# soedinglab/prosstt

Hardware: AMD Instinct MI355X
Metric: simulated cells*genes per second (count sampling: sample_density -> draw_counts) (higher is better)
Workload: dtype f32

## Files before the change

### prosstt_amd/_native.py

```python
import ctypes
import os
import threading
from collections import namedtuple

_HERE = os.path.dirname(os.path.abspath(__file__))

OK, EINVAL, EDOMAIN, EHIP, ENOMEM, ENODEV, ERCCL = 0, -1, -2, -3, -4, -5, -6
HOST_INPUTS, HOST_OUTPUT, CHECK_DOMAIN, TIME_KERNEL, CHECK_DEFERRED, MEANS_CACHED, PARAMS_NONNEG = 1, 2, 4, 8, 16, 32, 64
STATS_ACCUMULATE = 1

_Library = namedtuple("_Library", "path header hip symbols last_error")


def _path(env, filename):
    return os.environ.get(env) or os.path.join(_HERE, "lib", filename)


def _int(*argtypes):
    return ctypes.c_int, list(argtypes)


_ptr_to = ctypes.POINTER
_text = (ctypes.c_char_p, None)
vp, i32, i64, u32, u64, f64 = ctypes.c_void_p, ctypes.c_int32, ctypes.c_int64, ctypes.c_uint32, ctypes.c_uint64, ctypes.c_double
# ... 16 lines not shown
        "prosstt_amd_nb_params": _int(vp, vp, i64, i32, vp, vp, vp, vp, i64, vp, vp, vp, vp, u32),
        "prosstt_amd_hw_math": _int(vp, i32, u32, u64, vp, u32),
        "prosstt_amd_hw_math_at": _int(vp, i32, vp, u64, vp, u32),
        "prosstt_amd_comm_unique_id": _int(vp),
        "prosstt_amd_comm_init": _int(vp, vp, i32, i32, _ptr_to(vp)),
        "prosstt_amd_comm_destroy": _int(vp),
        "prosstt_amd_gather_counts": _int(vp, vp, vp, vp, i32, i32, vp),
        "prosstt_amd_comm_selftest": _int(vp, vp, u64),
        "prosstt_amd_domain_status": _int(vp, _ptr_to(i32)),
        "prosstt_amd_numpy_programs": _int(vp, vp, vp, vp, i32, i32, i32, vp, vp, vp, vp, vp, vp, vp, vp),
        "prosstt_amd_lineage_attempt": _int(vp, vp, i32, i32, vp, i64, i32, vp, vp, vp, vp),
        "prosstt_amd_lineage_attempt_batch": _int(vp, vp, i32, i32, i32, vp, i64, i32, vp, vp, vp, vp),
        "prosstt_amd_lineage_walk": _int(vp, u64, u64, i32, i32, vp),
        "prosstt_amd_lineage_walk_batch": _int(vp, u64, u64, i32, i32, i32, vp),
        "prosstt_amd_lineage_commit": _int(vp, vp, i32, i32, vp, i64, vp, vp),
        "prosstt_amd_gene_max": _int(vp, vp, i64, i64, vp),
        "prosstt_amd_means_from_rel": _int(vp, vp, vp, i64, i64, vp),
    }, "prosstt_amd_last_error"),
    "host": _Library(_path("PROSSTT_AMD_HOST_LIB", "libprosstt_amd_host.so"), "prosstt_amd_host.h", False, {
        "prosstt_amd_host_widen_i32_i64": _widen,
        "prosstt_amd_host_widen_u16_i64": _widen,
        "prosstt_amd_host_widen_u16_i32": _widen,
        "prosstt_amd_host_widen_u8_i64": _widen,
        "prosstt_amd_host_widen_u8_i32": _widen,
        "prosstt_amd_host_scatter_i32": _int(vp, i32, vp, vp, u64, i32),
        "prosstt_amd_host_has_avx2": (ctypes.c_int, None),
    }, None),
    "stats": _Library(_path("PROSSTT_AMD_STATS_LIB", "libprosstt_amd_stats.so"), "prosstt_amd_stats.h", True, {
        "prosstt_amd_stats_last_error": _text,
        "prosstt_amd_stats_workspace_bytes": _int(i64, i64, _ptr_to(u64)),
        "prosstt_amd_stats_count_summary": _int(vp, vp, i64, i64, i64, vp, u64, vp, vp, vp, vp, vp, vp, u32),
    }, "prosstt_amd_stats_last_error"),
    "embed": _Library(_path("PROSSTT_AMD_EMBED_LIB", "libprosstt_amd_embed.so"), "prosstt_amd_embed.h", True, {
        "prosstt_amd_embed_last_error": _text,
        "prosstt_amd_embed_workspace_bytes": _int(i64, i64, i64, _ptr_to(u64)),
        "prosstt_amd_embed_gene_moments": _int(vp, vp, i64, i64, i64, vp, vp, u64, vp, vp, vp),
        "prosstt_amd_embed_matmul": _int(vp, vp, i64, i64, i64, vp, vp, i64, vp, vp, u64, vp),
        "prosstt_amd_embed_rmatmul": _int(vp, vp, i64, i64, i64, vp, vp, i64, vp, vp, u64, vp),
    }, "prosstt_amd_embed_last_error"),
    "knn": _Library(_path("PROSSTT_AMD_KNN_LIB", "libprosstt_amd_knn.so"), "prosstt_amd_knn.h", True, {
        "prosstt_amd_knn_last_error": _text,
        "prosstt_amd_knn_workspace_bytes": _int(i64, i64, i64, i64, _ptr_to(u64)),
        "prosstt_amd_knn_search": _int(vp, vp, i64, i64, i64, i64, i64, vp, vp, vp, u64),
    }, "prosstt_amd_knn_last_error"),
    "graph": _Library(_path("PROSSTT_AMD_GRAPH_LIB", "libprosstt_amd_graph.so"), "prosstt_amd_graph.h", True, {
        "prosstt_amd_graph_last_error": _text,
        "prosstt_amd_graph_workspace_bytes": _int(i64, i64, _ptr_to(u64)),
        "prosstt_amd_graph_memberships": _int(vp, vp, vp, i64, i64, vp, vp, vp, vp),
        "prosstt_amd_graph_symmetrize_emit": _int(vp, vp, vp, i64, i64, vp, u64),
        "prosstt_amd_graph_symmetrize_fold": _int(vp, vp, vp, vp, i64, i64, i64, vp, u64, vp, vp, vp),
        "prosstt_amd_graph_normalize": _int(vp, vp, vp, vp, i64, i64, vp, vp, vp, vp),
        "prosstt_amd_graph_spmv": _int(vp, vp, vp, vp, i64, i64, vp, vp, i32),
    }, "prosstt_amd_graph_last_error"),
    "layout": _Library(_path("PROSSTT_AMD_LAYOUT_LIB", "libprosstt_amd_layout.so"), "prosstt_amd_layout.h", True, {
        "prosstt_amd_layout_last_error": _text,
        "prosstt_amd_layout_epochs": _int(vp, vp, vp, vp, i64, i64, i32, vp, vp, i32, i32, i32, f64, f64, f64, f64, i32, u64, i32),
        "prosstt_amd_layout_negatives": _int(vp, u64, i32, i64, i64, i32, i64, vp),
    }, "prosstt_amd_layout_last_error"),
}

ADDED_LIBRARIES = {
    "tsne": _Library(_path("PROSSTT_AMD_TSNE_LIB", "libprosstt_amd_tsne.so"), "prosstt_amd_tsne.h", True, {
        "prosstt_amd_tsne_last_error": _text,
        "prosstt_amd_tsne_workspace_bytes": _int(i64, i32, i32, _ptr_to(u64)),
        "prosstt_amd_tsne_affinities": _int(vp, vp, vp, i64, i64, f64, vp, vp, vp),
        "prosstt_amd_tsne_symmetrize_fold": _int(vp, vp, vp, vp, i64, i64, i64, vp, u64, vp, vp, vp),
        "prosstt_amd_tsne_gradient": _int(vp, vp, vp, vp, i64, i64, i32, vp, f64, i32, vp, u64, vp, vp, vp),
        "prosstt_amd_tsne_iterations": _int(vp, vp, vp, vp, i64, i64, i32, vp, vp, vp, vp, i32, i32, i32, f64, f64, i32, vp, u64),
        "prosstt_amd_tsne_objective": _int(vp, vp, vp, vp, i64, i64, i32, vp, vp),
    }, "prosstt_amd_tsne_last_error"),
}

LATER_LIBRARIES = {
    "dpt": _Library(_path("PROSSTT_AMD_DPT_LIB", "libprosstt_amd_dpt.so"), "prosstt_amd_dpt.h", True, {
        "prosstt_amd_dpt_last_error": _text,
        "prosstt_amd_dpt_workspace_bytes": _int(i64, i32, i32, _ptr_to(u64)),
        "prosstt_amd_dpt_rows": _int(vp, vp, i64, vp, i64, i64, vp, i64, vp),
        "prosstt_amd_dpt_concordance": _int(vp, vp, vp, i64, i32, i32, vp, u64, vp, vp),
    }, "prosstt_amd_dpt_last_error"),
    "markers": _Library(_path("PROSSTT_AMD_MARKERS_LIB", "libprosstt_amd_markers.so"), "prosstt_amd_markers.h", True, {
        "prosstt_amd_markers_last_error": _text,
        "prosstt_amd_markers_workspace_bytes": _int(i64, i64, i64, i64, _ptr_to(u64)),
        "prosstt_amd_markers_group_moments": _int(vp, vp, i64, i64, i64, vp, vp, i64, vp, i64, i64, vp, u64, vp, vp, vp, vp, vp),
    }, "prosstt_amd_markers_last_error"),
    "cluster": _Library(_path("PROSSTT_AMD_CLUSTER_LIB", "libprosstt_amd_cluster.so"), "prosstt_amd_cluster.h", True, {
        "prosstt_amd_cluster_last_error": _text,
        "prosstt_amd_cluster_workspace_bytes": _int(i64, i64, _ptr_to(u64)),
        "prosstt_amd_cluster_quantize": _int(vp, vp, vp, vp, i64, i64, vp, vp, vp),
        "prosstt_amd_cluster_sweep": _int(vp, vp, vp, vp, vp, i64, i64, vp, i64, i64, i64, vp, vp, i64, f64, i32, i32, vp, vp, vp),
        "prosstt_amd_cluster_totals": _int(vp, vp, vp, vp, vp, i64, i64, vp, vp, vp, vp),
        "prosstt_amd_cluster_aggregate_emit": _int(vp, vp, vp, i64, i64, vp, i64, vp, u64, vp),
        "prosstt_amd_cluster_aggregate_fold": _int(vp, vp, vp, vp, vp, i64, i64, i64, vp, vp, vp, vp),
    }, "prosstt_amd_cluster_last_error"),
    "ranks": _Library(_path("PROSSTT_AMD_RANKS_LIB", "libprosstt_amd_ranks.so"), "prosstt_amd_ranks.h", True, {
        "prosstt_amd_ranks_last_error": _text,
        "prosstt_amd_ranks_workspace_bytes": _int(i64, i64, i64, _ptr_to(u64)),
        "prosstt_amd_ranks_rank_sums": _int(vp, vp, i64, i64, i64, vp, vp, i64, vp, i64, i64, i64, vp, u64, vp, vp, vp),
    }, "prosstt_amd_ranks_last_error"),
    "hvg": _Library(_path("PROSSTT_AMD_HVG_LIB", "libprosstt_amd_hvg.so"), "prosstt_amd_hvg.h", True, {
        "prosstt_amd_hvg_last_error": _text,
        "prosstt_amd_hvg_workspace_bytes": _int(i64, i64, _ptr_to(u64)),
        "prosstt_amd_hvg_clipped_sums": _int(vp, vp, i64, i64, i64, vp, vp, u64, vp, vp, vp, vp),
        "prosstt_amd_hvg_normalized_moments": _int(vp, vp, i64, i64, i64, vp, vp, u64, vp, vp, vp),
        "prosstt_amd_hvg_gather_columns": _int(vp, vp, i64, i64, i64, vp, i64, vp, i64, vp),
    }, "prosstt_amd_hvg_last_error"),
    "autocorr": _Library(_path("PROSSTT_AMD_AUTOCORR_LIB", "libprosstt_amd_autocorr.so"), "prosstt_amd_autocorr.h", True, {
        "prosstt_amd_autocorr_last_error": _text,
        "prosstt_amd_autocorr_workspace_bytes": _int(i64, i64, i64, _ptr_to(u64)),
        "prosstt_amd_autocorr_gene_sums": _int(vp, vp, i64, i64, i64, vp, vp, vp, vp, vp, i64, vp, i64, i32, vp, u64, vp, vp, vp, vp, vp),
        "prosstt_amd_autocorr_smooth": _int(vp, vp, i64, i64, i64, vp, vp, vp, vp, vp, i64, i32, i32, vp, i64, vp),
    }, "prosstt_amd_autocorr_last_error"),
    "fit": _Library(_path("PROSSTT_AMD_FIT_LIB", "libprosstt_amd_fit.so"), "prosstt_amd_fit.h", True, {
        "prosstt_amd_fit_last_error": _text,
        "prosstt_amd_fit_workspace_bytes": _int(i64, i64, i64, _ptr_to(u64)),
        "prosstt_amd_fit_loglik": _int(vp, vp, i64, i64, i64, vp, vp, i64, vp, i64, vp, vp, i64, vp, u64, vp, vp, vp, vp),
    }, "prosstt_amd_fit_last_error"),
    "trends": _Library(_path("PROSSTT_AMD_TRENDS_LIB", "libprosstt_amd_trends.so"), "prosstt_amd_trends.h", True, {
        "prosstt_amd_trends_last_error": _text,
        "prosstt_amd_trends_workspace_bytes": _int(i64, i64, i64, i64, _ptr_to(u64)),
        "prosstt_amd_trends_node_sums": _int(vp, vp, i64, i64, i64, vp, vp, vp, i64, i64, i64, vp, u64, vp, vp, vp),
    }, "prosstt_amd_trends_last_error"),
    "mapping": _Library(_path("PROSSTT_AMD_MAPPING_LIB", "libprosstt_amd_mapping.so"), "prosstt_amd_mapping.h", True, {
        "prosstt_amd_mapping_last_error": _text,
        "prosstt_amd_mapping_workspace_bytes": _int(i64, i64, i64, i64, _ptr_to(u64)),
        "prosstt_amd_mapping_node_scores": _int(vp, vp, i64, i64, i64, vp, vp, i64, i64, vp, vp, vp, i64, i64, vp, u64, vp, vp,
                                                vp, vp, vp, vp),
        "prosstt_amd_mapping_node_scores_tiled": _int(vp, vp, i64, i64, i64, vp, vp, i64, i64, vp, vp, vp, i64, i64, i32, vp, u64,
                                                      vp, vp, vp, vp, vp, vp),
    }, "prosstt_amd_mapping_last_error"),
    "ptree": _Library(_path("PROSSTT_AMD_PTREE_LIB", "libprosstt_amd_ptree.so"), "prosstt_amd_ptree.h", True, {
        "prosstt_amd_ptree_last_error": _text,
        "prosstt_amd_ptree_workspace_bytes": _int(i64, i64, i64, i32, _ptr_to(u64)),
        "prosstt_amd_ptree_assign": _int(vp, vp, i64, i64, i64, vp, i64, i64, f64, vp, u64, vp, vp, vp, vp, vp, vp, vp),
        "prosstt_amd_ptree_project": _int(vp, vp, i64, i64, i64, vp, i64, i64, vp, i64, vp, vp, vp, vp),
    }, "prosstt_amd_ptree_last_error"),
}

NEWER_LIBRARIES = {
    "regress": _Library(_path("PROSSTT_AMD_REGRESS_LIB", "libprosstt_amd_regress.so"), "prosstt_amd_regress.h", True, {
        "prosstt_amd_regress_last_error": _text,
        "prosstt_amd_regress_workspace_bytes": _int(i64, i64, i64, _ptr_to(u64)),
        "prosstt_amd_regress_normal_equations": _int(vp, vp, i64, i64, i64, vp, vp, i64, vp, i64, i64, vp, vp, vp, i32, i32, vp,
                                                     u64, vp, vp, vp, vp, vp),
    }, "prosstt_amd_regress_last_error"),
}


SAMPLER_LATER = ("prosstt_amd_plan.h", {
    "prosstt_amd_strip_plan": _int(i64, i32, i32, i32, i32, vp, _ptr_to(i32), _ptr_to(i32), _ptr_to(i32)),
    "prosstt_amd_last_strip_plan": _int(vp, vp, _ptr_to(i32), _ptr_to(i32), _ptr_to(i32)),
})


def _library(name):
    for table in (LIBRARIES, ADDED_LIBRARIES, LATER_LIBRARIES):
        if name in table:
            return table[name]
    return NEWER_LIBRARIES[name]


class NativeError(RuntimeError):
    def __init__(self, code, message):
        super().__init__("prosstt_amd error %d: %s" % (code, message))
        self.code = code


_loaded = {}
_lock = threading.Lock()


def load(name="sampler"):
    lib = _library(name)
    with _lock:
        if name not in _loaded:
            if not os.path.exists(lib.path):
                raise RuntimeError("%s not found: build it with `make -C prosstt_amd/csrc %s` (or "
                                   "`python -c 'import __graft_entry__ as g; g.build()'`)%s"
                                   % (lib.path, name, ". prosstt_amd has no CPU fallback." if lib.hip else ""))
            if lib.hip:
                import torch
            L = ctypes.CDLL(lib.path)
            symbols = dict(lib.symbols, **SAMPLER_LATER[1]) if name == "sampler" else lib.symbols
            for symbol, (restype, argtypes) in symbols.items():
                fn = getattr(L, symbol)
                fn.restype = restype
                if argtypes is not None:
                    fn.argtypes = argtypes
            _loaded[name] = L
        return _loaded[name]


def check(code, name="sampler"):
    if code != OK:
        msg = getattr(load(name), _library(name).last_error)().decode("utf-8", "replace")
        if code == EDOMAIN:
            raise ValueError(msg)
        raise NativeError(code, msg)


def device_count():
    n = ctypes.c_int(0)
    rc = load().prosstt_amd_device_count(ctypes.byref(n))
    return n.value if rc == OK else 0
```

### prosstt_amd/csrc/k3_heavy.h

```cpp
#pragma once
#include "prnb_device.h"
#include "k3_stream.h"

namespace k3 {

constexpr int kHeavyBlock = 256;
constexpr int kHCap = 128;
constexpr uint32_t kWalkerBlocks = 6u;
constexpr int kWCap = 96;

struct HGEntry { int32_t n, g, attempt; float m; };
struct HPEntry { int32_t n, g; float lam; int32_t attempt; };
struct HWId { int32_t n, g; };

struct HeavyLds {
    HGEntry hg[kHCap];
    HPEntry hp[kHCap];
    f32x4_t wst[kWCap];
    HWId wid[kWCap];
    uint16_t wk[kWCap];
};

__global__ __launch_bounds__(kHeavyBlock) void sample_counts_heavy_kernel(
    const HeavyList* __restrict__ heavy_ptr, uint32_t regions, StripPlan plan,
    const float* __restrict__ means, int64_t rows,
    int32_t G, const int32_t* __restrict__ row_of_cell, const float* __restrict__ scal,
    const float* __restrict__ ga, const float* __restrict__ gbm1, int64_t N, uint32_t k0, uint32_t k1,
    uint64_t cell_offset, const int64_t* __restrict__ cell_index, int32_t* __restrict__ out, int64_t ld,
    int64_t* __restrict__ check_words, uint32_t check_request, uint32_t check_bad_row, uint32_t check_verdict)
{
    __shared__ __attribute__((aligned(16))) float inv_k_store[prnb::kTabShift + prnb::kKTab];
    float* const inv_k = inv_k_store + prnb::kTabShift;
    __shared__ HeavyLds lds_all[kHeavyBlock / 64];
    const HeavyList heavy = *heavy_ptr;
    const int tid = threadIdx.x, lane = tid & 63, wv = __builtin_amdgcn_readfirstlane(tid >> 6);
    HeavyLds& L = lds_all[wv];
    for (int k = tid - prnb::kTabShift; k < prnb::kKTab; k += kHeavyBlock) inv_k[k] = k > 0 ? 1.0f / (float)k : 0.0f;
    __shared__ uint32_t seg_n[kSegs], seg_first[kSegs + 1];
    if (wv == 0) {
        uint32_t n = heavy.seg_cnt[lane];
        n = n < heavy.ent_cap ? n : heavy.ent_cap;
        uint32_t x = (n + 63u) >> 6;
        const uint32_t mine = x;
#pragma unroll
        for (int d = 1; d < 64; d <<= 1) {
            const uint32_t t = (uint32_t)__shfl_up((int)x, d, 64);
            if (lane >= d) x += t;
        }
        seg_n[lane] = n;
        seg_first[lane] = x - mine;
        if (lane == 63) seg_first[kSegs] = x;
    }
    struct ClassRec { int32_t first_cell, end_cell; uint32_t first_block, groups, groups_rcp, log2_len, pad[2]; };
    __shared__ __attribute__((aligned(16))) ClassRec cls_tab[kPlanClasses];
    if (tid < kPlanClasses) {
        static_assert(kPlanClasses == 4, "spelled out below");
        const StripClass c0 = plan.c[0], c1 = plan.c[1], c2 = plan.c[2], c3 = plan.c[3];
        const int32_t end_all = plan.c[4].first_cell;
        const int32_t first = tid == 0 ? c0.first_cell : (tid == 1 ? c1.first_cell : (tid == 2 ? c2.first_cell : c3.first_cell));
        const int32_t end = tid == 0 ? c1.first_cell : (tid == 1 ? c2.first_cell : (tid == 2 ? c3.first_cell : end_all));
        const int32_t len = tid == 0 ? c0.strip_cells : (tid == 1 ? c1.strip_cells : (tid == 2 ? c2.strip_cells : c3.strip_cells));
        const int32_t fb = tid == 0 ? c0.first_block : (tid == 1 ? c1.first_block : (tid == 2 ? c2.first_block : c3.first_block));
        const uint32_t sh = (uint32_t)__builtin_ctz((uint32_t)len);
        const int32_t strips = (end - first + len - 1) >> sh;
        const uint32_t g = strips > 4 ? (uint32_t)(strips + 3) / 4u : 1u;
        ClassRec c;
        c.first_cell = first; c.end_cell = end; c.first_block = (uint32_t)fb;
        c.groups = g;
        c.groups_rcp = 0xffffffffu / g + ((g & (g - 1u)) == 0u ? 1u : 0u);
        c.log2_len = sh; c.pad[0] = c.pad[1] = 0u;
        cls_tab[tid] = c;
    }
    __syncthreads();
    const uint32_t waves = gridDim.x * (kHeavyBlock / 64);
    auto locate = [&](uint32_t chunk, uint32_t& seg, uint32_t& first) __attribute__((always_inline)) {
        uint32_t lo = 0u;
#pragma unroll
        for (uint32_t step = kSegs / 2; step != 0u; step >>= 1)
            if (seg_first[lo + step] <= chunk) lo += step;
        seg = lo;
        first = (chunk - seg_first[lo]) << 6;
    };
    const uint32_t fb1 = (uint32_t)plan.c[1].first_block, fb2 = (uint32_t)plan.c[2].first_block, fb3 = (uint32_t)plan.c[3].first_block;
    struct Origin { int32_t tile_g, n0, cells; };
    auto region_origin = [&](uint32_t r) __attribute__((always_inline)) -> Origin {
        const uint32_t blk = r >> 2;
        const uint32_t cls = (blk >= fb1 ? 1u : 0u) + (blk >= fb2 ? 1u : 0u) + (blk >= fb3 ? 1u : 0u);
        const ClassRec c = cls_tab[cls];
        const uint32_t local = blk - c.first_block;
        uint32_t q = __umulhi(local, c.groups_rcp);
        q += (local - q * c.groups >= c.groups) ? 1u : 0u;
        q = c.groups > 1u ? q : local;
        Origin o;
        o.tile_g = (int32_t)q;
        o.n0 = c.first_cell + (int32_t)(((local - q * c.groups) * 4u + (r & 3u)) << c.log2_len);
        o.cells = c.end_cell - o.n0 < (1 << c.log2_len) ? c.end_cell - o.n0 : (1 << c.log2_len);
        return o;
    };

    int hg_top = 0, hp_top = 0, hw_top = 0;

    auto cell_id = [&](int32_t n) __attribute__((always_inline)) -> uint64_t {
        return cell_index ? (uint64_t)cell_index[n] : cell_offset + (uint64_t)n;
    };

    auto poisson_pass = [&]() __attribute__((always_inline)) {
        const int cnt = hp_top < 64 ? hp_top : 64;
        bool again = false, small = false;
        HPEntry e;
        e.n = 0; e.g = 0; e.lam = 0.0f; e.attempt = 0;
        int32_t x = 0;
        if (lane < cnt) {
            e = L.hp[hp_top - 1 - lane];
            const uint64_t cell = cell_id(e.n);
            const uint32_t c0 = (uint32_t)cell, c1 = (uint32_t)(cell >> 32);
            const float lam = e.lam;
            if (!(lam > 0.0f)) {
                x = 0;
            } else if (lam < prnb::kPoisInv) {
                small = true;
            } else if (!(lam < prnb::kLamBig)) {
                const prnb::Words w = prnb::philox_count<0>(c0, c1, (uint32_t)e.g, 0x80000000u, k0, k1);
                const float z = prnb::hw_normal(w.w[0], w.w[1]);
                const float kf = __builtin_floorf(PRNB_FMA(prnb::hw_sqrt(lam), z, lam) + 0.5f);
                x = (int32_t)__builtin_fminf(__builtin_fmaxf(kf, 0.0f), 2147483520.0f);
            } else {
                const int j = e.attempt;
                const prnb::Words w =
                    prnb::philox_count<0>(c0, c1, (uint32_t)e.g, 0x80000000u + (uint32_t)(j >> 1), k0, k1);
                const float slam = prnb::hw_sqrt(lam);
                const float bb = PRNB_FMA(2.53f, slam, 0.931f);
                const float aa = PRNB_FMA(0.02483f, bb, -0.059f);
                const float U = prnb::unif((j & 1) ? w.w[2] : w.w[0]) - 0.5f;
                const float V = prnb::unif((j & 1) ? w.w[3] : w.w[1]);
                const float us = __builtin_fmaxf(0.5f - __builtin_fabsf(U), 5.8207661e-11f);
                const float rus = prnb::hw_rcp(us);
                float kf = __builtin_floorf(PRNB_FMA(PRNB_FMA(2.0f * aa, rus, bb), U, lam + 0.43f));
                const float vr = PRNB_FMA(-3.6224f, prnb::hw_rcp(bb - 2.0f), 0.9277f);
                bool accept = (us >= 0.07f) && (V <= vr);
                if (!accept && !(kf < 0.0f || (us < 0.013f && V > us))) {
                    const float invalpha = PRNB_FMA(1.1328f, prnb::hw_rcp(bb - 3.4f), 1.1239f);
                    const float lhs = prnb::kLn2 * prnb::hw_log2((V * invalpha) * prnb::hw_rcp(PRNB_FMA(aa * rus, rus, bb)));
                    float rhs;
                    if (kf < 10.0f) {
                        rhs = PRNB_FMA(kf, prnb::kLn2 * prnb::hw_log2(lam), -lam) - prnb::logfact_small((int)kf);
                    } else {
                        const float rk = prnb::hw_rcp(kf);
                        const float d = (lam - kf) * rk;
                        const float lp = prnb::hw_log1pmx(d, lam * rk);
                        const float st = rk * PRNB_FMA(-0.0027777778f, rk * rk, 0.083333336f);
                        rhs = PRNB_FMA(kf, lp, PRNB_FMA(-0.5f, prnb::kLn2 * prnb::hw_log2(6.2831855f * kf), -st));
                    }
                    accept = lhs <= rhs;
                }
                if (!accept) {
                    kf = __builtin_floorf(lam);
                    again = j + 1 < 2 * prnb::kMaxTries;
                }
                x = (int32_t)__builtin_fminf(__builtin_fmaxf(kf, 0.0f), 2147483520.0f);
            }
        }
        if (__builtin_amdgcn_ballot_w64(small) != 0ull) {
            const uint64_t cell = cell_id(e.n);
            const prnb::Words w = prnb::philox_count<0>((uint32_t)cell, (uint32_t)(cell >> 32), (uint32_t)e.g, 0x80000000u, k0, k1);
            const float lam = small ? e.lam : 1.0f;
            const int32_t xs = prnb::chop_down_wave(small, w.w[0], prnb::hw_exp2(-(lam * prnb::kLog2e)), lam, 0.0f, inv_k);
            if (small) x = xs;
        }
        if (lane < cnt && !again && x != 0) out[(int64_t)e.n * ld + e.g] = x;
        hp_top -= cnt;
        const unsigned long long m = __builtin_amdgcn_ballot_w64(again);
        if (again) {
            e.attempt += 1;
            L.hp[hp_top + lane_rank(m)] = e;
        }
        hp_top += __popcll(m);
    };

    auto gamma_pass = [&]() __attribute__((always_inline)) {
        const int cnt = hg_top < 64 ? hg_top : 64;
        bool again = false, accepted = false;
        HGEntry e;
        e.n = 0; e.g = 0; e.attempt = 0; e.m = 0.0f;
        float lam = 0.0f;
        if (lane < cnt) {
            e = L.hg[hg_top - 1 - lane];
            const prnb::Params P = prnb::make_params_m(e.m, ga[e.g], gbm1[e.g]);
            const float r = P.m * P.inv_th;
            if (P.valid && r >= prnb::kRMin) {
                const uint64_t cell = cell_id(e.n);
                const bool boost = r < 1.0f;
                const float rr = boost ? r + 1.0f : r;
                const float dd = rr - 0.33333334f;
                const float cc = prnb::hw_rsq(9.0f * dd);
                const int i = e.attempt;
                const bool last = (i == prnb::kMaxTries - 1);
                const prnb::Words w = prnb::philox_count<0>((uint32_t)cell, (uint32_t)(cell >> 32), (uint32_t)e.g,
                                                          1u + (uint32_t)i, k0, k1);
                const float x = prnb::hw_normal(w.w[0], w.w[1]);
                const float t = cc * x;
                const float v1 = 1.0f + t;
                float v = 1.0f;
                bool ok;
                if (!(v1 > 0.0f)) {
                    ok = last;
                } else {
                    v = (v1 * v1) * v1;
                    ok = last;
                    if (!ok) {
                        const float u = prnb::unif(w.w[2]);
                        const float x2 = x * x;
                        ok = u < PRNB_FMA(-0.0331f, x2 * x2, 1.0f);
                        if (!ok) {
                            const float t2 = t * t;
                            const float h = PRNB_FMA(3.0f, prnb::hw_log1pmx(t, v1), PRNB_FMA(-t2, t, -3.0f * t2));
                            ok = prnb::kLn2 * prnb::hw_log2(u) < PRNB_FMA(dd, h, 0.5f * x2);
                        }
                    }
                }
                if (ok) {
                    float g = dd * v;
                    if (boost) g = g * prnb::hw_exp2(prnb::hw_log2(prnb::unif(w.w[3])) * prnb::hw_rcp(r));
                    lam = P.theta * g;
                    accepted = true;
                } else {
                    again = true;
                }
            }
        }
        hg_top -= cnt;
        const unsigned long long ma = __builtin_amdgcn_ballot_w64(again);
        if (again) {
            e.attempt += 1;
            L.hg[hg_top + lane_rank(ma)] = e;
        }
        hg_top += __popcll(ma);
        const unsigned long long mp = __builtin_amdgcn_ballot_w64(accepted);
        if (accepted) {
            HPEntry p;
            p.n = e.n; p.g = e.g; p.lam = lam; p.attempt = 0;
            L.hp[hp_top + lane_rank(mp)] = p;
        }
        hp_top += __popcll(mp);
        while (hp_top >= 64) poisson_pass();
    };

    int32_t wk = -1;
    float wps = 0.0f, wrem = 0.0f, wd = 0.0f, wq = 0.0f;
    int32_t wn = 0, wg = 0;
    auto walk_take = [&]() __attribute__((always_inline)) {
        const unsigned long long idle_m = __builtin_amdgcn_ballot_w64(wk < 0);
        const int rank = lane_rank(idle_m);
        if (wk < 0 && rank < hw_top) {
            const int at = hw_top - 1 - rank;
            const f32x4_t s = L.wst[at];
            const HWId id = L.wid[at];
            wk = (int32_t)L.wk[at];
            wps = s.x; wd = s.y; wq = s.z; wrem = s.w;
            wn = id.n; wg = id.g;
        }
        const int idle = __popcll(idle_m);
        hw_top -= idle < hw_top ? idle : hw_top;
    };
    auto walk_pass = [&]() __attribute__((always_inline)) {
        const bool busy = wk >= 0;
        const float* tab = &inv_k[busy ? wk + 1 : 6];
        float4 iv[4];
#pragma unroll
        for (int j = 0; j < 4; ++j) iv[j] = *reinterpret_cast<const float4*>(__builtin_assume_aligned(tab + 4 * j, 16));
        float t = wps, r = wrem;
        float rg[4][4], tl[4];
#pragma unroll
        for (int j = 0; j < 4; ++j) {
            rg[j][0] = r - t;
            t = t * PRNB_FMA(wd, iv[j].x, wq);
            rg[j][1] = rg[j][0] - t;
            t = t * PRNB_FMA(wd, iv[j].y, wq);
            rg[j][2] = rg[j][1] - t;
            t = t * PRNB_FMA(wd, iv[j].z, wq);
            rg[j][3] = rg[j][2] - t;
            tl[j] = t;
            r = rg[j][3];
            t = t * PRNB_FMA(wd, iv[j].w, wq);
        }
        bool end[4];
#pragma unroll
        for (int j = 0; j < 4; ++j) end[j] = (rg[j][3] < 0.0f) || (tl[j] < 1.0f) || (wk + 4 * j + 3 >= prnb::kWalkEnd);
        const bool ended = busy && (end[0] || end[1] || end[2] || end[3]);
        if (__builtin_amdgcn_ballot_w64(ended) != 0ull) {
            int32_t at[4];
#pragma unroll
            for (int j = 0; j < 4; ++j)
                at[j] = ((wk + 4 * j + 3) + ((int32_t)prnb::f2u(rg[j][0]) >> 31)) + (((int32_t)prnb::f2u(rg[j][1]) >> 31) + ((int32_t)prnb::f2u(rg[j][2]) >> 31));
            if (ended) {
                out[(int64_t)wn * ld + wg] = end[0] ? at[0] : (end[1] ? at[1] : (end[2] ? at[2] : at[3]));
                wk = -1;
                wps = 0.0f;
            }
        }
        if (wk >= 0) {
            wps = t;
            wk += 16;
            wrem = r;
        }
    };
    auto walk_service = [&](bool drain) __attribute__((always_inline)) {
        for (;;) {
            const int busy = __popcll(__builtin_amdgcn_ballot_w64(wk >= 0));
            if (busy <= 32 && (drain ? hw_top > 0 : hw_top >= 32)) walk_take();
            else if (drain ? busy > 0 : busy > 32) walk_pass();
            else break;
        }
    };
    auto walk_push = [&](bool push, int32_t n, int32_t g, int32_t k, f32x4_t s) __attribute__((always_inline)) {
        const unsigned long long mw = __builtin_amdgcn_ballot_w64(push);
        if (push) {
            const int at = hw_top + lane_rank(mw);
            L.wst[at] = s;
            HWId id;
            id.n = n; id.g = g;
            L.wid[at] = id;
            L.wk[at] = (uint16_t)k;
        }
        hw_top += __popcll(mw);
        if (hw_top >= 32) walk_service(false);
    };

    auto from_start = [&](bool has, int32_t n, int32_t g) __attribute__((always_inline)) {
        bool heavy_c = false, light = false;
        prnb::Params P;
        P.m = 1.0f; P.theta = 1.0f; P.iu = 0.5f; P.t2 = 1.0f; P.inv_th = 1.0f; P.valid = false; P.light = false;
        if (has) {
            int32_t row = row_of_cell[n];
            row = row < 0 ? 0 : (row >= rows ? (int32_t)(rows - 1) : row);
            P = prnb::make_params(means[(int64_t)row * G + g], scal[n], ga[g], gbm1[g]);
            light = P.valid && P.light;
            heavy_c = P.valid && !P.light;
        }
        const unsigned long long mh = __builtin_amdgcn_ballot_w64(heavy_c);
        if (heavy_c) {
            HGEntry e;
            e.n = n; e.g = g; e.attempt = 0; e.m = P.m;
            L.hg[hg_top + lane_rank(mh)] = e;
        }
        hg_top += __popcll(mh);
        bool push = false;
        f32x4_t s = {0.0f, 0.0f, 0.0f, 0.0f};
        if (__builtin_amdgcn_ballot_w64(light) != 0ull) {
            const uint64_t cell = cell_id(has ? n : 0);
            const prnb::Words w = prnb::philox_count<0>((uint32_t)cell, (uint32_t)(cell >> 32), (uint32_t)g >> 2, 0u, k0, k1);
            const uint32_t sel = (uint32_t)g & 3u;
            const uint32_t wj = sel == 0u ? w.w[0] : (sel == 1u ? w.w[1] : (sel == 2u ? w.w[2] : w.w[3]));
            const float mp = P.m * P.iu, q = P.theta * P.iu, d = mp - q;
            const float ps = prnb::hw_exp2(-P.t2) * 4294967296.0f;
            const float r0 = (float)wj - ps;
            const float p1 = ps * mp;
            const float r1 = r0 - p1;
            const float p2 = p1 * PRNB_FMA(d, inv_k[2], q);
            const float r2 = r1 - p2;
            const float p3 = p2 * PRNB_FMA(d, inv_k[3], q);
            const float r3 = r2 - p3;
            const float p4 = p3 * PRNB_FMA(d, inv_k[4], q);
            const float r4 = r3 - p4;
            const bool done = (r0 < 0.0f) || (r1 < 0.0f) || (r2 < 0.0f) || (r3 < 0.0f) || (r4 < 0.0f) || (p4 < 1.0f);
            const int32_t x = (r0 < 0.0f) ? 0 : ((r1 < 0.0f) ? 1 : ((r2 < 0.0f) ? 2 : ((r3 < 0.0f) ? 3 : 4)));
            if (light && done && x != 0) out[(int64_t)n * ld + g] = x;
            push = light && !done;
            s.x = p4 * PRNB_FMA(d, inv_k[5], q);
            s.y = d; s.z = q; s.w = r4;
        }
        walk_push(push, n, g, 5, s);
        while (hg_top >= 64) gamma_pass();
    };

    const uint32_t wave_id = blockIdx.x * (kHeavyBlock / 64) + (uint32_t)wv;
    const bool walker = (blockIdx.x & 15u) < kWalkerBlocks;
    const uint32_t walker_blocks = (gridDim.x >> 4) * kWalkerBlocks + ((gridDim.x & 15u) < kWalkerBlocks ? (gridDim.x & 15u) : kWalkerBlocks);
    const uint32_t n_redo = heavy.seg_cnt[kSegs + 1] < (uint32_t)kRedoCap ? heavy.seg_cnt[kSegs + 1] : (uint32_t)kRedoCap;
    auto push_entries = [&](bool has, int32_t n, int32_t g, float m) __attribute__((always_inline)) {
        const unsigned long long mh = __builtin_amdgcn_ballot_w64(has);
        if (has) {
            HGEntry h;
            h.n = n; h.g = g; h.attempt = 0; h.m = m;
            L.hg[hg_top + lane_rank(mh)] = h;
        }
        hg_top += __popcll(mh);
        while (hg_top >= 64) gamma_pass();
    };
    if (!walker) {
        const uint32_t blk_rank = blockIdx.x - ((blockIdx.x >> 4) * kWalkerBlocks + ((blockIdx.x & 15u) < kWalkerBlocks ? (blockIdx.x & 15u) : kWalkerBlocks));
        const uint32_t rank = blk_rank * (kHeavyBlock / 64) + (uint32_t)wv;
        const uint32_t drawers = (gridDim.x - walker_blocks) * (kHeavyBlock / 64);
        {
            const int sub = lane >> 4, sl = lane & 15;
            const uint4* const dense4 = reinterpret_cast<const uint4*>(heavy.dense);
            struct Step { uint32_t cnt; uint4 d4; Origin o; };
            auto load_step = [&](uint64_t r0) __attribute__((always_inline)) -> Step {
                Step S;
                S.cnt = 0u; S.d4 = make_uint4(0u, 0u, 0u, 0u);
                const uint64_t r = r0 + (uint64_t)sub * drawers;
                S.o = region_origin((uint32_t)r);
                if (r < (uint64_t)regions) {
                    S.cnt = heavy.count[r] & 0xffffu;
                    S.d4 = dense4[r * (kDense / 2) + (uint32_t)sl];
                }
                return S;
            };
            Step nxt = load_step(rank);
            for (uint64_t r0 = rank; r0 < (uint64_t)regions; r0 += 4ull * drawers) {
                const Step cur = nxt;
                nxt = load_step(r0 + 4ull * drawers);
                const uint32_t cnt = cur.cnt > heavy.cap ? 0u : cur.cnt;
                const int32_t tile_g = cur.o.tile_g, n0 = cur.o.n0;
                push_entries(2u * (uint32_t)sl < cnt, n0 + (int32_t)(cur.d4.x >> 8), tile_g * kTileG + (int32_t)(cur.d4.x & 255u), __uint_as_float(cur.d4.y));
                push_entries(2u * (uint32_t)sl + 1u < cnt, n0 + (int32_t)(cur.d4.z >> 8), tile_g * kTileG + (int32_t)(cur.d4.z & 255u), __uint_as_float(cur.d4.w));
            }
        }
        {
            const uint32_t chunks = seg_first[kSegs];
            HeavyEntry nx;
            nx.n = 0; nx.g = 0; nx.m = 0.0f; nx.pad = 0u;
            bool nx_has = false;
            auto request = [&](uint32_t chunk) __attribute__((always_inline)) {
                uint32_t sg, first;
                locate(chunk, sg, first);
                nx_has = first + (uint32_t)lane < seg_n[sg];
                if (nx_has) nx = heavy.ent[(uint64_t)sg * heavy.ent_cap + first + (uint32_t)lane];
            };
            if (rank < chunks) request(rank);
            for (uint32_t chunk = rank; chunk < chunks; chunk += drawers) {
                const HeavyEntry e = nx;
                const bool has = nx_has;
                if (chunk + drawers < chunks) request(chunk + drawers);
                push_entries(has, e.n, e.g, e.m);
            }
        }
    } else {
        const uint32_t wrank = ((blockIdx.x >> 4) * kWalkerBlocks + (blockIdx.x & 15u)) * (kHeavyBlock / 64) + (uint32_t)wv;
        const uint32_t walkers = walker_blocks * (kHeavyBlock / 64);
        for (uint32_t i = wrank * 64u; i < n_redo; i += walkers * 64u) {
            const bool has = i + (uint32_t)lane < n_redo;
            const int2 ng = has ? heavy.redo[i + (uint32_t)lane] : make_int2(0, 0);
            from_start(has, ng.x, ng.y);
        }
        const uint32_t per_walker = ((regions + walkers - 1u) / walkers + 15u) & ~15u;
        const uint32_t r_end = (wrank + 1u) * per_walker < regions ? (wrank + 1u) * per_walker : regions;
        const uint32_t rl = (uint32_t)lane >> 2, s0 = (uint32_t)lane & 3u;
        static_assert(kWalkSlots <= 12, "three slots per lane");
        struct WStep { uint32_t n_walks; f32x4_t st[3]; uint32_t id[3]; Origin o; };
        auto load_wstep = [&](uint32_t rb) __attribute__((always_inline)) -> WStep {
            WStep S;
            S.n_walks = 0u;
            const uint32_t r = rb + rl;
            S.o = region_origin(r);
#pragma unroll
            for (int j = 0; j < 3; ++j) { S.st[j] = f32x4_t{0.0f, 0.0f, 0.0f, 0.0f}; S.id[j] = 0u; }
            if (r < r_end) {
                S.n_walks = heavy.count[r] >> 16;
#pragma unroll
                for (int j = 0; j < 3; ++j) {
                    const uint32_t slot = s0 + 4u * (uint32_t)j;
                    if (slot < (uint32_t)kWalkSlots) {
                        S.st[j] = heavy.wst[(uint64_t)r * kWalkSlots + slot];
                        S.id[j] = heavy.wid[(uint64_t)r * kWalkSlots + slot];
                    }
                }
            }
            return S;
        };
        WStep wn = load_wstep(wrank * per_walker);
        for (uint32_t rb = wrank * per_walker; rb < r_end; rb += 16u) {
            const WStep cur = wn;
            wn = load_wstep(rb + 16u);
            const int32_t tile_g = cur.o.tile_g, n0 = cur.o.n0;
#pragma unroll
            for (int j = 0; j < 3; ++j) {
                const uint32_t slot = s0 + 4u * (uint32_t)j;
                walk_push(slot < cur.n_walks, n0 + (int32_t)((cur.id[j] & 0xffffu) >> 8), tile_g * kTileG + (int32_t)(cur.id[j] & 255u),
                          (int32_t)(cur.id[j] >> 16) - 3, cur.st[j]);
            }
        }
    }
    {
        const uint32_t n_ovf = heavy.seg_cnt[kSegs];
        for (uint32_t i = wave_id; i < n_ovf; i += waves) {
            const uint32_t r = heavy.ovf_regions[i];
            const Origin o = region_origin(r);
            const int32_t tg = o.tile_g;
            const int64_t nb = o.n0;
            for (int32_t c = 0; c < o.cells; ++c)
                for (int j = 0; j < 4; ++j) {
                    const int32_t g = tg * kTileG + j * 64 + lane;
                    from_start(g < G, (int32_t)(nb + c), g);
                }
        }
    }
    walk_service(true);
    while (hg_top > 0) gamma_pass();
    while (hp_top > 0) poisson_pass();

    if (check_words && check_words[check_request] != 0 && check_words[check_bad_row] == 0) {
        bool bad = false;
        for (int64_t n = blockIdx.x; n < N; n += gridDim.x) {
            const float s = scal[n];
            const float* mrow = means + (int64_t)row_of_cell[n] * G;
            for (int32_t g = tid; g < G; g += kHeavyBlock) {
                const float M = mrow[g];
                const float m = M * s;
                bad = bad || !(M > 0.0f && M < __builtin_inff()) || (PRNB_FMA(ga[g], m, gbm1[g]) < 0.0f);
            }
        }
        if (bad) check_words[check_verdict] = 1;
    }
}

}
```

### prosstt_amd/csrc/k3_stream.h

```cpp
#pragma once
#include <type_traits>
#include "prnb_device.h"

namespace k3 {

constexpr int kBlock = 256;
constexpr int kTileG = 256;
constexpr int kStripCells = 128;
constexpr int kS1Cap = 192;
constexpr int kS2Cap = 104;
constexpr int kS2Run = 40;
static_assert(kS2Cap >= kS2Run - 1 + 64 && kS1Cap >= 63 + 128, "a stack must take one more round of pushes");
constexpr int kRing = 8;
constexpr int kBail = 6;

constexpr int kLateCap = 64;
constexpr int kRingMaxK3 = 248;
constexpr int kLongSlots = 4;
constexpr int kListTail = 16;
constexpr int kInvTab = 272;

struct CellInfo { uint64_t row_bytes; float s; uint32_t runs; uint32_t ph[4]; };
static_assert(sizeof(CellInfo) == 32, "one s_load_dwordx8");

constexpr int kRunMinCells = 8;

__host__ __device__ inline uint32_t run_word(const int32_t* row_of_cell, int64_t i, int64_t N, int64_t rows, int32_t strip_cells)
{
    if (i >= N) return 1u;
    auto row = [&](int64_t n) -> int64_t { const int64_t r = row_of_cell[n]; return r < 0 ? 0 : (r >= rows ? rows - 1 : r); };
    const int64_t first = i - i % strip_cells;
    const int64_t end = first + strip_cells < N ? first + strip_cells : N;
    const int64_t mine = row(i);
    if (i != first && row(i - 1) == mine) return 0u;
    int64_t j = i + 1;
    while (j < end && row(j) == mine) ++j;
    const uint32_t len = (uint32_t)(j - i);
    if (i != first) return len;
    uint32_t runs = 1u;
    for (int64_t prev = mine; j < end; ++j) {
        const int64_t r = row(j);
        runs += r != prev;
        prev = r;
    }
    return len | (runs << 16);
}

constexpr int kPlanClasses = 4;
constexpr int kPlanAlign = 64;
constexpr int kPlanMinStrip = 8;
struct StripClass { int32_t first_cell, strip_cells, first_block; };
struct StripPlan {
    int32_t classes, tiles_g;
    StripClass c[kPlanClasses + 1];
};

__host__ __device__ inline StripPlan strip_plan(int64_t N, int32_t G, int32_t resident, int32_t forced_cells, int32_t taper, int32_t max_classes)
{
    const int64_t n = N > 0 ? N : 0;
    const int64_t tiles = ((int64_t)(G > 0 ? G : 0) + kTileG - 1) / kTileG;
    int64_t L = 64;
    while (L > 8 && ((n + L - 1) / L) * tiles < 4 * 5 * 1024) L /= 2;
    if (forced_cells == 8 || forced_cells == 16 || forced_cells == 32 || forced_cells == 64) L = forced_cells;
    if (forced_cells == kStripCells) L = 64;
    const int64_t uniform_blocks = (((n + L - 1) / L + 3) / 4) * tiles;
    const int64_t R = taper > 0 ? taper : resident;
    const int most = max_classes >= 1 && max_classes <= kPlanClasses ? max_classes : kPlanClasses;
    int64_t size[kPlanClasses] = {n, 0, 0, 0};
    int K = 1;
    if (taper > 0 || (resident > 0 && uniform_blocks >= 4 * (int64_t)resident)) {
        const int64_t uniform_len = L;
        if (L == 64 && forced_cells != 64) L = kStripCells;
        const int64_t align = L > kPlanAlign ? L : kPlanAlign;
        int64_t shorts = 0;
        while (K < most && (L >> K) >= kPlanMinStrip) {
            int64_t s = ((R * 4 * (L >> K) / (tiles > 0 ? tiles : 1) + kPlanAlign / 2) / kPlanAlign) * kPlanAlign;
            if (s < kPlanAlign) s = kPlanAlign;
            if (n - (shorts + s) < align) break;
            size[K++] = s;
            shorts += s;
        }
        if (K > 1) size[0] = ((n - shorts) / align) * align;
        else L = uniform_len;
    }
    StripPlan p;
    p.classes = K;
    p.tiles_g = (int32_t)tiles;
    int64_t cell = 0, block = 0;
    for (int k = 0; k <= kPlanClasses; ++k) {
        const int64_t len = k < K ? L >> k : 1;
        const int64_t cells = k + 1 < K ? size[k] : n - cell;
        p.c[k].first_cell = (int32_t)cell;
        p.c[k].strip_cells = (int32_t)len;
        p.c[k].first_block = (int32_t)(block < 0x7fffffff ? block : 0x7fffffff);
        cell += cells;
        block += (((cells + len - 1) / len + 3) / 4) * tiles;
    }
    return p;
}

struct StripAt { int32_t tile_g, cells, strip_cells; int64_t n0; };
__host__ __device__ inline StripAt strip_of_region(const StripPlan& p, uint32_t region)
{
    const int32_t blk = (int32_t)(region >> 2);
    static_assert(kPlanClasses == 4, "spelled out below");
    const StripClass c0 = p.c[0], c1 = p.c[1], c2 = p.c[2], c3 = p.c[3];
    const int32_t end_all = p.c[4].first_cell;
    StripClass c = c0;
    int32_t end = c1.first_cell;
    if (blk >= c1.first_block) { c = c1; end = c2.first_cell; }
    if (blk >= c2.first_block) { c = c2; end = c3.first_cell; }
    if (blk >= c3.first_block) { c = c3; end = end_all; }
    const int32_t first = c.first_cell, len = c.strip_cells, fb = c.first_block;
    const int32_t strips = (end - first + len - 1) >> __builtin_ctz((uint32_t)len);
    const int32_t groups = strips > 4 ? (strips + 3) / 4 : 1;
    const int32_t local = blk - fb;
    StripAt at;
    at.tile_g = local / groups;
    at.strip_cells = len;
    const int32_t strip = (local - at.tile_g * groups) * 4 + (int32_t)(region & 3u);
    at.n0 = (int64_t)first + (int64_t)strip * len;
    at.cells = strip < strips ? (end - at.n0 < len ? (int32_t)(end - at.n0) : len) : 0;
    return at;
}

constexpr uint32_t kPhiloxM0 = 0xD2511F53u, kPhiloxM1 = 0xCD9E8D57u, kPhiloxW0 = 0x9E3779B9u, kPhiloxW1 = 0xBB67AE85u;

__host__ __device__ inline void philox_cell_part(uint32_t cell_lo, uint32_t cell_hi, uint32_t k0, uint32_t k1, uint32_t ph[4])
{
    const uint64_t p0 = (uint64_t)kPhiloxM0 * cell_lo;
    const uint64_t p1 = (uint64_t)kPhiloxM1 * ((uint32_t)(p0 >> 32) ^ k1);
    ph[0] = cell_hi ^ k0;
    ph[1] = (uint32_t)(p1 >> 32) ^ (k0 + kPhiloxW0);
    ph[2] = (uint32_t)p0 ^ (k1 + kPhiloxW1);
    ph[3] = (uint32_t)p1;
}

__device__ __forceinline__ prnb::Words philox_count_row(const uint32_t ph[4], uint32_t hi1, uint32_t lo1, uint32_t k0, uint32_t k1)
{
    static_assert(prnb::kCountRounds >= 3, "two rounds are spelled out here");
    const uint32_t c0a = hi1 ^ ph[0];
    const uint64_t p0 = (uint64_t)kPhiloxM0 * c0a;
    const uint32_t c0b = lo1 ^ ph[1];
    const uint32_t c1b = ph[3];
    const uint32_t c2b = (uint32_t)(p0 >> 32) ^ ph[2];
    const uint32_t c3b = (uint32_t)p0;
    return prnb::philox4x32<prnb::kCountRounds - 2, 0>(c0b, c1b, c2b, c3b, k0 + 2u * kPhiloxW0, k1 + 2u * kPhiloxW1);
}

struct S1Entry { float m, theta, wf; uint32_t pos; };
struct S2Entry { float ps, d, q, rem; };

struct WaveLds {
    S1Entry s1_null;
    S1Entry s1[kS1Cap];
    S2Entry s2[kS2Cap];
    uint32_t s2p[kS2Cap];
    uint32_t late[kLateCap];
};

static_assert(offsetof(WaveLds, s1) == offsetof(WaveLds, s1_null) + sizeof(S1Entry), "s1[-1] must be the null entry");

typedef float f32x4_t __attribute__((ext_vector_type(4)));
constexpr int kSegs = 64;
constexpr int kDense = 32;
constexpr int kWalkSlots = kBail + kLongSlots;
struct HeavyEntry { int32_t n, g; float m; uint32_t pad; };
struct HeavyList {
    uint2* list; uint32_t cap;
    uint2* dense;
    uint32_t* count;
    f32x4_t* wst; uint32_t* wid;
    uint32_t* overflow;
    uint32_t* seg_cnt;
    HeavyEntry* ent; uint32_t ent_cap;
    uint32_t* ovf_regions;
    int2* redo;
};
constexpr int kRedoCap = 65536;

__device__ __forceinline__ uint32_t umin(uint32_t a, uint32_t b) { return a < b ? a : b; }

__device__ __forceinline__ int lane_rank(unsigned long long mask)
{
    return (int)__builtin_amdgcn_mbcnt_hi((uint32_t)(mask >> 32),
                                          __builtin_amdgcn_mbcnt_lo((uint32_t)mask, 0u));
}

#define K3_GLOBAL(T) __attribute__((address_space(1))) T*
typedef uint32_t u32x4_t __attribute__((ext_vector_type(4)));
typedef int32_t i32x2_t __attribute__((ext_vector_type(2)));
static_assert(sizeof(HeavyEntry) == sizeof(u32x4_t) && sizeof(int2) == sizeof(i32x2_t), "stored as plain vectors");
template <bool VEC, bool BIG>
__global__ __launch_bounds__(kBlock, 5) void sample_counts_stream_kernel(
    const float* __restrict__ means, int32_t G, const CellInfo* __restrict__ cellinfo,
    const float* __restrict__ ga, const float* __restrict__ gbm1, const float* __restrict__ gphi,
    int64_t N, uint32_t k0, uint32_t k1, int32_t* __restrict__ out, int64_t ld, StripPlan plan,
    uint2* __restrict__ heavy_list, uint32_t heavy_cap, uint2* __restrict__ heavy_dense,
    const HeavyList* __restrict__ heavy_ptr)
{
    struct HeavyGlobal {
        K3_GLOBAL(uint32_t) count; K3_GLOBAL(f32x4_t) wst; K3_GLOBAL(uint32_t) wid; K3_GLOBAL(uint32_t) overflow;
        K3_GLOBAL(uint32_t) seg_cnt; K3_GLOBAL(u32x4_t) ent; uint32_t ent_cap; K3_GLOBAL(uint32_t) ovf_regions; K3_GLOBAL(i32x2_t) redo;
    };
    auto heavy_late = [&]() -> HeavyGlobal {
        const HeavyList* p = heavy_ptr;
        asm volatile("" : "+s"(p));
        const __attribute__((address_space(4))) HeavyList* h = (const __attribute__((address_space(4))) HeavyList*)p;
        HeavyGlobal g;
        g.count = (K3_GLOBAL(uint32_t))h->count; g.wst = (K3_GLOBAL(f32x4_t))h->wst; g.wid = (K3_GLOBAL(uint32_t))h->wid;
        g.overflow = (K3_GLOBAL(uint32_t))h->overflow; g.seg_cnt = (K3_GLOBAL(uint32_t))h->seg_cnt; g.ent = (K3_GLOBAL(u32x4_t))h->ent;
        g.ent_cap = h->ent_cap; g.ovf_regions = (K3_GLOBAL(uint32_t))h->ovf_regions; g.redo = (K3_GLOBAL(i32x2_t))h->redo;
        return g;
    };
    __shared__ __attribute__((aligned(16))) float inv_k_store[prnb::kTabShift + kInvTab + 2];
    float* const inv_k = inv_k_store + prnb::kTabShift;
    __shared__ WaveLds lds_all[kBlock / 64];
    __shared__ __attribute__((aligned(kRing * 256))) uint8_t ring_all[kBlock / 64][kRing * 256];

    const int tid = threadIdx.x;
    const int lane = tid & 63, wv = __builtin_amdgcn_readfirstlane(tid >> 6);
    WaveLds& L = lds_all[wv];

    for (int k = tid - prnb::kTabShift; k < kInvTab + 2; k += kBlock) inv_k[k] = k > 0 ? 1.0f / (float)k : 0.0f;
    __syncthreads();

    const uint32_t region = blockIdx.x * 4u + (uint32_t)wv;
    const StripAt at = strip_of_region(plan, region);
    const int32_t gbase = __builtin_amdgcn_readfirstlane(at.tile_g) * kTileG;
    const int32_t g0 = gbase + lane * 4;
    const int64_t n0 = (int64_t)__builtin_amdgcn_readfirstlane((int32_t)at.n0);
    const int cells = __builtin_amdgcn_readfirstlane(at.cells);
    if (cells <= 0) {
        if (lane == 0) heavy_late().count[region] = 0u;
        return;
    }

    float a[4], bm1[4], phi[4];
#pragma unroll
    for (int j = 0; j < 4; ++j) {
        const bool in = g0 + j < G;
        a[j] = in ? ga[g0 + j] : 0.0f;
        bm1[j] = in ? gbm1[g0 + j] : 0.0f;
        phi[j] = in ? gphi[g0 + j] : 1.0f;
    }

    const uint32_t s1_lds = (uint32_t)(uintptr_t)&L.s1[0];
    uint32_t s1_at = s1_lds;
    int s2_top = 0;
    constexpr uint32_t kNoHeavy = 0xffffffffu;
    uint32_t hpend = kNoHeavy;
    float hpend_m = 0.0f;
    typedef float f32x4 __attribute__((ext_vector_type(4)));
    f32x4 st = {0.0f, 0.0f, 0.0f, 0.0f};
    uint32_t pos = 0u;
    int k3 = 8;
    f32x4 inv = *reinterpret_cast<const f32x4*>(__builtin_assume_aligned(&inv_k[6], 16));
    f32x4 inv2 = *reinterpret_cast<const f32x4*>(__builtin_assume_aligned(&inv_k[10], 16));
    unsigned long long idle_s = ~0ull;

    constexpr uint32_t kPosMagic = 0x4B000000u;
    int32_t* const strip_out = out + n0 * ld + gbase;
    const uint32_t ld32 = (uint32_t)ld;
    int32_t flushed_pos = -1;
    uint8_t* const ring = ring_all[wv];
    for (int i = lane; i < kRing * 64; i += 64) reinterpret_cast<uint32_t*>(ring)[i] = 0u;
    if (lane < 4) reinterpret_cast<uint32_t*>(&L.s1_null)[lane] = 0u;

    const __amdgpu_buffer_rsrc_t out_rsrc = __builtin_amdgcn_make_buffer_rsrc(strip_out, 0, 0x80000000u, 0x00020000);
    const uint32_t store_voff = g0 < G ? (uint32_t)lane * 16u : 0x80000000u;
    uint32_t flush_off = 0u;

    auto flush_row = [&](int cl) {
        uint32_t* slot = reinterpret_cast<uint32_t*>(ring + (cl & (kRing - 1)) * 256) + lane;
        const uint32_t packed = __hip_atomic_exchange(slot, 0u, __ATOMIC_RELAXED, __HIP_MEMORY_SCOPE_WAVEFRONT);
        const int32_t v[4] = {(int32_t)(packed & 0xffu), (int32_t)((packed >> 8) & 0xffu),
                              (int32_t)((packed >> 16) & 0xffu), (int32_t)(packed >> 24)};
        if (VEC) {
            typedef uint32_t u32x4_ __attribute__((ext_vector_type(4)));
            const u32x4_ row4 = {(uint32_t)v[0], (uint32_t)v[1], (uint32_t)v[2], (uint32_t)v[3]};
            if (BIG) __builtin_amdgcn_raw_buffer_store_b128(row4, out_rsrc, store_voff, flush_off, 18 );
            else __builtin_amdgcn_raw_buffer_store_b128(row4, out_rsrc, store_voff, flush_off, 2 );
        } else {
            int32_t* dst = strip_out + (int64_t)cl * ld + lane * 4;
#pragma unroll
            for (int j = 0; j < 4; ++j)
                if (g0 + j < G) dst[j] = v[j];
        }
        flush_off += ld32 * 4u;
        flushed_pos = (int32_t)kPosMagic | (cl << 8) | 255;
    };

    int late_top = 0;
    auto flush_late = [&]() {
        for (int i = lane; i < late_top; i += 64) {
            const uint32_t e = L.late[i];
            const uint32_t p = e >> 16;
            strip_out[(p >> 8) * ld32 + (p & 255u)] = (int32_t)(e & 0xffffu);
        }
        late_top = 0;
    };
#define K3_MASK(x) __builtin_amdgcn_ballot_w64(x)
    const uint32_t ring_lds = (uint32_t)(uintptr_t)&ring[0];
    uint32_t ring_mask = (uint32_t)(kRing * 256 - 1);
    asm volatile("" : "+v"(ring_mask));
    const uint32_t late_lds = (uint32_t)(uintptr_t)&L.late[0];
    uint2* const my_list = heavy_list + (uint64_t)region * (heavy_cap + (uint32_t)kListTail);
    uint2* const my_long = my_list + heavy_cap;
    int n_long = 0;
    uint32_t h_cnt = 0u;
    auto flush_heavy = [&]() {
        const unsigned long long mp_ = K3_MASK(hpend != kNoHeavy);
        if (hpend != kNoHeavy) {
            const uint32_t slot = h_cnt + (uint32_t)lane_rank(mp_);
            if (slot < heavy_cap) {
                uint2* const dst = slot < (uint32_t)kDense ? heavy_dense + ((uint64_t)region * kDense + slot) : my_list + slot;
                *dst = make_uint2(hpend & 0xffffu, __float_as_uint(hpend_m));
            }
        }
        h_cnt += (uint32_t)__popcll(mp_);
        hpend = kNoHeavy;
    };
    auto deliver = [&](unsigned long long ok_m, unsigned long long give_m, uint32_t p, uint32_t res, float gm) {
        const unsigned long long late_m = K3_MASK((int32_t)p <= flushed_pos);
        uint32_t ring_at;
        asm volatile("v_and_or_b32 %0, %2, %3, %4\n\ts_mov_b64 exec, %1\n\tds_write_b8 %0, %5\n\ts_mov_b64 exec, -1"
                     : "=&v"(ring_at) : "s"(ok_m & ~late_m), "v"(p), "v"(ring_mask), "s"(ring_lds), "v"(res) : "memory");
        const unsigned long long ml = ok_m & late_m;
        if ((ml | give_m) != 0ull) {
            if (ml != 0ull) {
                const int cnt = __popcll(ml);
                if (late_top + cnt > kLateCap) flush_late();
                asm volatile("s_mov_b64 exec, %0\n\tds_write_b32 %1, %2\n\ts_mov_b64 exec, -1"
                             :: "s"(ml), "v"(late_lds + (uint32_t)((late_top + lane_rank(ml)) << 2)), "v"((p << 16) | res) : "memory");
                late_top += cnt;
            }
            if (give_m != 0ull) {
                if ((give_m & K3_MASK(hpend != kNoHeavy)) != 0ull) flush_heavy();
                asm volatile("s_mov_b64 exec, %2\n\tv_mov_b32 %0, %3\n\tv_mov_b32 %1, %4\n\ts_mov_b64 exec, -1"
                             : "+v"(hpend), "+v"(hpend_m) : "s"(give_m), "v"(p), "v"(gm));
            }
        }
    };
    const uint32_t s2_lds = (uint32_t)(uintptr_t)&L.s2[0];
    const uint32_t s2p_lds = (uint32_t)(uintptr_t)&L.s2p[0];
    auto stage3_pass = [&]() {
        if (BIG) __builtin_amdgcn_s_setprio(2);
        if (idle_s != 0ull && s2_top > 0) {
            const int left_ = s2_top - __popcll(idle_s);
            const int left = left_ > 0 ? left_ : 0;
            const int rank = lane_rank(idle_s);
            const unsigned long long take_m = idle_s & K3_MASK(rank < s2_top - left);
            asm volatile("s_mov_b64 exec, %[tm]\n\t"
                         "ds_read_b128 %[st], %[ea]\n\t"
                         "ds_read_b32 %[pos], %[pa]\n\t"
                         "s_mov_b64 exec, -1\n\t"
                         "s_waitcnt lgkmcnt(0)"
                         : [st] "+v"(st), [pos] "+v"(pos)
                         : [tm] "s"(take_m), [ea] "v"(((uint32_t)rank << 4) + (s2_lds + ((uint32_t)left << 4))),
                           [pa] "v"(((uint32_t)rank << 2) + (s2p_lds + ((uint32_t)left << 2)))
                         : "memory");
            s2_top = left;
            idle_s &= ~take_m;
        }
        const float d = st.y, q = st.z;
        const float r1 = st.w - st.x;
        const float ps1 = st.x * PRNB_FMA(d, inv.x, q);
        const float r2 = r1 - ps1;
        const float ps2 = ps1 * PRNB_FMA(d, inv.y, q);
        const float r3 = r2 - ps2;
        const float ps3 = ps2 * PRNB_FMA(d, inv.z, q);
        const float r4 = r3 - ps3;
        const float ps4 = ps3 * PRNB_FMA(d, inv.w, q);
        const float r5 = r4 - ps4;
        const float ps5 = ps4 * PRNB_FMA(d, inv2.x, q);
        const float r6 = r5 - ps5;
        const float ps6 = ps5 * PRNB_FMA(d, inv2.y, q);
        const float r7 = r6 - ps6;
        const float ps7 = ps6 * PRNB_FMA(d, inv2.z, q);
        const float r8 = r7 - ps7;
        const unsigned long long hit_a = K3_MASK(r4 < 0.0f), tail_a = K3_MASK(ps3 < 1.0f);
        const unsigned long long hit_b = K3_MASK(r8 < 0.0f), tail_b = K3_MASK(ps7 < 1.0f);
        const int32_t res_a = (k3 + ((int32_t)prnb::f2u(r1) >> 31) + ((int32_t)prnb::f2u(r2) >> 31)) + ((int32_t)prnb::f2u(r3) >> 31);
        const int32_t res_b = ((k3 + 4) + ((int32_t)prnb::f2u(r5) >> 31) + ((int32_t)prnb::f2u(r6) >> 31)) + ((int32_t)prnb::f2u(r7) >> 31);
        const unsigned long long end_a = (hit_a | tail_a) & ~idle_s;
        const unsigned long long big_m = K3_MASK(k3 >= kRingMaxK3) & ~idle_s;
        const unsigned long long end_b = (hit_b | tail_b) & ~(idle_s | end_a);
        const unsigned long long long_m = big_m & ~(end_a | end_b);
        int32_t res_k;
        asm("v_cndmask_b32 %0, %1, %2, %3" : "=v"(res_k) : "v"(res_b), "v"(res_a), "s"(end_a));
        deliver(end_a | end_b, 0ull, pos, (uint32_t)res_k, 0.0f);
        idle_s |= end_a | end_b | big_m;
        st.x = ps7 * PRNB_FMA(d, inv2.w, q);
        const int k3n = k3 + 8;
        st.w = r8;
        if (long_m != 0ull) {
            const int n_have = n_long < 0 ? kLongSlots : n_long;
            const int slot = n_have + lane_rank(long_m);
            const bool mine = (long_m >> lane) & 1ull;
            bool full = false;
            if (mine && slot < kLongSlots) {
                my_long[3 * slot] = make_uint2(__float_as_uint(st.x), __float_as_uint(st.y));
                my_long[3 * slot + 1] = make_uint2(__float_as_uint(st.z), __float_as_uint(st.w));
                my_long[3 * slot + 2] = make_uint2((pos & 0xffffu) | ((uint32_t)k3n << 16), 0u);
            }
            if (mine && slot >= kLongSlots) {
                const HeavyGlobal heavy = heavy_late();
                const uint32_t at = __hip_atomic_fetch_add(heavy.seg_cnt + kSegs + 1, 1u, __ATOMIC_RELAXED, __HIP_MEMORY_SCOPE_AGENT);
                if (at < (uint32_t)kRedoCap) heavy.redo[at] = i32x2_t{(int32_t)(n0 + ((pos & 0xffffu) >> 8)), gbase + (int32_t)(pos & 255u)};
                else full = true;
            }
            const bool any_full = __builtin_amdgcn_ballot_w64(full) != 0ull;
            const int n_new = n_have + __popcll(long_m);
            n_long = (n_long < 0 || any_full) ? -1 : (n_new < kLongSlots ? n_new : kLongSlots);
        }
        asm("v_cndmask_b32 %0, %1, 8, %2" : "=v"(k3) : "v"(k3n), "s"(idle_s));
        inv = *reinterpret_cast<const f32x4*>(__builtin_assume_aligned(&inv_k[k3 - 2], 16));
        inv2 = *reinterpret_cast<const f32x4*>(__builtin_assume_aligned(&inv_k[k3 + 2], 16));
// ... 66 lines not shown
        Seg r;
        const float* rowp = reinterpret_cast<const float*>(reinterpret_cast<const char*>(mcol) + row_bytes);
        if (VEC) {
            typedef uint32_t u32x4_ __attribute__((ext_vector_type(4)));
            const __amdgpu_buffer_rsrc_t rs = __builtin_amdgcn_make_buffer_rsrc(const_cast<float*>(rowp), 0, 0x7fffffff, 0x00020000);
            const u32x4_ raw = __builtin_amdgcn_raw_buffer_load_b128(rs, gload_b, 0, 0);
            r.x = __uint_as_float(raw.x); r.y = __uint_as_float(raw.y); r.z = __uint_as_float(raw.z); r.w = __uint_as_float(raw.w);
        } else {
            r.x = (g0 + 0 < G) ? rowp[lane4 + 0] : 0.0f;
            r.y = (g0 + 1 < G) ? rowp[lane4 + 1] : 0.0f;
            r.z = (g0 + 2 < G) ? rowp[lane4 + 2] : 0.0f;
            r.w = (g0 + 3 < G) ? rowp[lane4 + 3] : 0.0f;
        }
        return r;
    };
    const uint32_t runs_word = cinfo[0].runs;
    const bool by_runs = (runs_word >> 16) * (uint32_t)kRunMinCells <= (uint32_t)cells;
    Seg cur = load_seg(cinfo[0].row_bytes), nxt;
    uint64_t row2 = 0u;
    if (!by_runs) {
        nxt = load_seg(cinfo[1].row_bytes);
        row2 = cinfo[2].row_bytes;
    }
    float s = cinfo[0].s;
    uint32_t ph[4] = {cinfo[0].ph[0], cinfo[0].ph[1], cinfo[0].ph[2], cinfo[0].ph[3]};
    const uint64_t quad_p1 = (uint64_t)kPhiloxM1 * ((uint32_t)g0 >> 2);
    const uint32_t quad_hi = (uint32_t)(quad_p1 >> 32), quad_lo = (uint32_t)quad_p1;
    __builtin_amdgcn_s_waitcnt(0x0F70);
    float posf = __uint_as_float(kPosMagic | lane4);
    int cl = 0;
    auto stage1_pass = [&](auto load_tag) {
        constexpr bool kLoad = decltype(load_tag)::value;
        const float m4[4] = {cur.x * s, cur.y * s, cur.z * s, cur.w * s};
        if (cl >= kRing) flush_row(cl - kRing);
        __builtin_amdgcn_sched_barrier(0);
        Seg nn;
        uint64_t row3 = 0u;
        if constexpr (kLoad) {
            nn = load_seg(row2);
            row3 = cinfo[3].row_bytes;
        }
        const float s_next = cinfo[1].s;
        const uint32_t ph_next[4] = {cinfo[1].ph[0], cinfo[1].ph[1], cinfo[1].ph[2], cinfo[1].ph[3]};
        ++cinfo;
        __builtin_amdgcn_sched_barrier(0);
        const prnb::Words W = philox_count_row(ph, quad_hi, quad_lo, k0, k1);
        u32x4 e[4];
        unsigned long long push_m[4];
#pragma unroll
        for (int j = 0; j < 4; ++j) {
            const float m = m4[j];
            const float x = m * phi[j];
            const float bound32 = PRNB_FMA(PRNB_FMA(PRNB_FMA(-715827882.7f, x, 2147483648.0f), x, -4294967296.0f),
                                           x, 4294924346.0f);
            const float wf = (float)W.w[j];
            asm("v_cmp_nlt_f32 %0, %1, %2" : "=s"(push_m[j]) : "v"(wf), "v"(bound32));
            e[j].x = __float_as_uint(m);
            e[j].y = __float_as_uint(PRNB_FMA(a[j], m, bm1[j]));
            e[j].z = __float_as_uint(wf);
            e[j].w = __float_as_uint(posf + (float)j);
        }
#pragma unroll
        for (int h = 0; h < 2; ++h) {
            uint32_t t0, t1, c_;
            asm volatile(
                "s_mov_b64 exec, %[m0]\n\t"
                "v_mbcnt_lo_u32_b32 %[t0], exec_lo, 0\n\t"
                "v_mbcnt_hi_u32_b32 %[t0], exec_hi, %[t0]\n\t"
                "v_lshl_add_u32 %[t0], %[t0], 4, %[at]\n\t"
                "ds_write_b128 %[t0], %[e0]\n\t"
                "s_bcnt1_i32_b64 %[c], exec\n\t"
                "s_lshl4_add_u32 %[at], %[c], %[at]\n\t"
                "s_mov_b64 exec, %[m1]\n\t"
                "v_mbcnt_lo_u32_b32 %[t1], exec_lo, 0\n\t"
                "v_mbcnt_hi_u32_b32 %[t1], exec_hi, %[t1]\n\t"
                "v_lshl_add_u32 %[t1], %[t1], 4, %[at]\n\t"
                "ds_write_b128 %[t1], %[e1]\n\t"
                "s_bcnt1_i32_b64 %[c], exec\n\t"
                "s_lshl4_add_u32 %[at], %[c], %[at]\n\t"
                "s_mov_b64 exec, -1"
                : [at] "+s"(s1_at), [t0] "=&v"(t0), [t1] "=&v"(t1), [c] "=&s"(c_)
                : [m0] "s"(push_m[2 * h]), [m1] "s"(push_m[2 * h + 1]), [e0] "v"(e[2 * h]), [e1] "v"(e[2 * h + 1])
                : "memory", "scc");
            while (s1_at - s1_lds >= 64u * 16u) {
                stage2_pass(std::true_type{});
                while (s2_top >= kS2Run) stage3_pass();
            }
        }
        if constexpr (kLoad) {
            cur = nxt;
            nxt = nn;
            row2 = row3;
        }
        s = s_next;
        ph[0] = ph_next[0]; ph[1] = ph_next[1]; ph[2] = ph_next[2]; ph[3] = ph_next[3];
        posf += 256.0f;
    };
    if (!by_runs) {
#pragma unroll 1
        for (; cl < cells; ++cl) stage1_pass(std::true_type{});
    } else {
        int run = (int)(runs_word & 0xffffu);
#pragma unroll 1
        while (cl < cells) {
            const int run_end = run > 0 && cl + run < cells ? cl + run : cells;
            const int len = run_end - cl;
            nxt = load_seg(cinfo[len].row_bytes);
            run = (int)(cinfo[len].runs & 0xffffu);
#pragma unroll 1
            for (; cl < run_end; ++cl) stage1_pass(std::false_type{});
            __builtin_amdgcn_s_waitcnt(0x0F70);
            cur = nxt;
        }
    }

    while (s1_at != s1_lds) {
        stage2_pass(std::false_type{});
        while (s2_top >= kS2Run) stage3_pass();
    }
    unsigned long long bail_m = 0ull;
    for (;;) {
        const unsigned long long busy_m = ~idle_s;
        if (s2_top == 0) {
            if (busy_m == 0ull) break;
            if (__popcll(busy_m) <= kBail) { bail_m = busy_m; break; }
        }
        stage3_pass();
    }
    if (__builtin_amdgcn_ballot_w64(hpend != kNoHeavy) != 0ull) flush_heavy();
    for (int cl = (cells > kRing ? cells - kRing : 0); cl < cells; ++cl) flush_row(cl);
    flush_late();
    const HeavyGlobal heavy = heavy_late();
    auto staged = [&](uint32_t i) -> unsigned long long {
        return __hip_atomic_load(reinterpret_cast<unsigned long long*>(my_list + i), __ATOMIC_RELAXED, __HIP_MEMORY_SCOPE_AGENT);
    };
    const int n_kept = n_long < 0 ? kLongSlots : n_long;
    const uint32_t n_still = (uint32_t)__popcll(bail_m);
    if ((bail_m >> lane) & 1ull) {
        const uint64_t at = (uint64_t)region * kWalkSlots + (uint32_t)lane_rank(bail_m);
        heavy.wst[at] = st;
        heavy.wid[at] = (pos & 0xffffu) | ((uint32_t)k3 << 16);
    }
    if (n_kept != 0) {
        __builtin_amdgcn_s_waitcnt(0x0F70);
        if (lane < n_kept) {
            const uint64_t at = (uint64_t)region * kWalkSlots + n_still + (uint32_t)lane;
            const unsigned long long w0 = staged(heavy_cap + 3u * (uint32_t)lane), w1 = staged(heavy_cap + 3u * (uint32_t)lane + 1u);
            const f32x4_t stl = {__uint_as_float((uint32_t)w0), __uint_as_float((uint32_t)(w0 >> 32)), __uint_as_float((uint32_t)w1), __uint_as_float((uint32_t)(w1 >> 32))};
            heavy.wst[at] = stl;
            heavy.wid[at] = (uint32_t)staged(heavy_cap + 3u * (uint32_t)lane + 2u);
        }
    }
    const bool too_many = h_cnt > heavy_cap || n_long < 0;
    if (lane == 0) heavy.count[region] = (h_cnt < 0xffffu ? h_cnt : 0xffffu) | ((n_still + (uint32_t)n_kept) << 16);
    bool spills = too_many;
    if (!too_many && h_cnt > (uint32_t)kDense) {
        const uint32_t n_over = h_cnt - (uint32_t)kDense;
        const uint32_t seg = region & (uint32_t)(kSegs - 1);
        uint32_t base_e = 0u;
        if (lane == 0) base_e = __hip_atomic_fetch_add(heavy.seg_cnt + seg, n_over, __ATOMIC_RELAXED, __HIP_MEMORY_SCOPE_AGENT);
        __builtin_amdgcn_s_waitcnt(0x0F70);
        base_e = (uint32_t)__builtin_amdgcn_readfirstlane((int32_t)base_e);
        spills = base_e + n_over > heavy.ent_cap;
        for (uint32_t i = (uint32_t)lane; i < n_over; i += 64u) {
            if (base_e + i < heavy.ent_cap) {
                const unsigned long long raw = staged((uint32_t)kDense + i);
                const uint32_t px = (uint32_t)raw;
                const u32x4_t e = {(uint32_t)(n0 + (px >> 8)), (uint32_t)(gbase + (int32_t)(px & 255u)), (uint32_t)(raw >> 32), 0u};
                heavy.ent[(uint64_t)seg * heavy.ent_cap + base_e + i] = e;
            }
        }
    }
    if (spills && lane == 0) {
        const uint32_t at = __hip_atomic_fetch_add(heavy.seg_cnt + kSegs, 1u, __ATOMIC_RELAXED, __HIP_MEMORY_SCOPE_AGENT);
        heavy.ovf_regions[at] = region;
        heavy.overflow[0] = 1u;
    }
}

}
```

### prosstt_amd/csrc/prosstt_amd.hip

```cpp
#include <hip/hip_runtime.h>

#include <cmath>
#include <cstdarg>
#include <cstdio>
#include <cstring>
#include <cstdlib>
#include <limits>
#include <new>
#include <vector>

#include <hip/hip_ext.h>
#include "../../include/prosstt_amd.h"
#include "prnb_device.h"
#include "k3_stream.h"
#include "k3_heavy.h"
#include "numpy_stream.h"

#define PA_EXPORT extern "C" __attribute__((visibility("default")))
#define PA_CATCH                                                                                       \
    catch (const std::bad_alloc&) { return fail(PROSSTT_AMD_ENOMEM, "out of host memory"); }          \
    catch (const std::exception& e) { return fail(PROSSTT_AMD_EINVAL, "unexpected exception: %s", e.what()); } \
    catch (...) { return fail(PROSSTT_AMD_EINVAL, "unexpected exception"); }

static thread_local char g_err[512] = "";

static int fail(int code, const char* fmt, ...)
{
    va_list ap;
    va_start(ap, fmt);
    vsnprintf(g_err, sizeof(g_err), fmt, ap);
    va_end(ap);
    return code;
}

#define HIP_TRY(expr)                                                                          \
    do {                                                                                       \
        hipError_t e_ = (expr);                                                                \
        if (e_ != hipSuccess)                                                                  \
            return fail(e_ == hipErrorOutOfMemory ? PROSSTT_AMD_ENOMEM : PROSSTT_AMD_EHIP,     \
                        "%s: %s (%s:%d)", #expr, hipGetErrorString(e_), __FILE__, __LINE__);   \
    } while (0)

struct prosstt_amd_ctx {
    int device = 0;
    hipStream_t stream = nullptr;
    void* ws = nullptr;
    size_t ws_bytes = 0;
    int64_t* scratch = nullptr;
    int64_t* h_scratch = nullptr;
    std::vector<hipEvent_t> events;
    size_t events_used = 0;
    k3::HeavyList list{};
    uint64_t list_regions = 0;
    k3::StripPlan list_plan{};
    const k3::CellInfo* list_info = nullptr;
    int64_t list_cells = 0;
    int heavy_grid = 1280;
    int stream_resident = 1280;
    uint8_t* row_bad = nullptr;
    size_t row_bad_cap = 0;
    const float* row_bad_means = nullptr;
    int64_t row_bad_rows = 0;
    int32_t row_bad_G = 0;
    uint32_t call_parity = 0;
};

static int next_event_pair(prosstt_amd_ctx* c, hipEvent_t* a, hipEvent_t* b)
{
    if (c->events_used + 2 > c->events.size()) {
        hipEvent_t e0, e1;
        HIP_TRY(hipEventCreate(&e0));
        HIP_TRY(hipEventCreate(&e1));
        c->events.push_back(e0);
        c->events.push_back(e1);
    }
    *a = c->events[c->events_used];
    *b = c->events[c->events_used + 1];
    c->events_used += 2;
    return 0;
}
enum ScratchWord : int {
    kListOverflow = 3,
    kStickyDomain = 4,
    kStickyRow = 5,
    kFullReq = 6,
    kScratchWords = 8
};
static_assert(kStickyRow == kStickyDomain + 1, "domain_verdict copies and clears the two sticky words as one 16-byte range");

static int ws_reserve(prosstt_amd_ctx* c, size_t bytes)
{
    c->list = k3::HeavyList{};
    if (bytes <= c->ws_bytes) return 0;
    if (c->ws) {
        HIP_TRY(hipStreamSynchronize(c->stream));
        HIP_TRY(hipFree(c->ws));
        c->ws = nullptr;
        c->ws_bytes = 0;
    }
    bytes = (bytes + (1u << 20)) & ~((size_t)(1u << 20) - 1);
    HIP_TRY(hipMalloc(&c->ws, bytes));
    c->ws_bytes = bytes;
    return 0;
}

struct Staging {
    const bool host_in, host_out;
    std::vector<void*> bufs;
    explicit Staging(uint32_t flags = 0) : host_in(flags & PROSSTT_AMD_HOST_INPUTS), host_out(flags & PROSSTT_AMD_HOST_OUTPUT) {}
    ~Staging() { for (void* p : bufs) (void)hipFree(p); }
    int alloc(void** p, size_t bytes)
    {
        HIP_TRY(hipMalloc(p, bytes ? bytes : 1));
        bufs.push_back(*p);
        return 0;
    }
    template <class T> int in(const T*& p, size_t count, hipStream_t s)
    {
        if (!host_in || !p) return 0;
        void* d = nullptr;
        int rc = alloc(&d, count * sizeof(T));
        if (rc) return rc;
        HIP_TRY(hipMemcpyAsync(d, p, count * sizeof(T), hipMemcpyHostToDevice, s));
        p = (const T*)d;
        return 0;
    }
    template <class T> int out(T*& p, size_t count)
    {
        if (!host_out || !p) return 0;
        void* d = nullptr;
        int rc = alloc(&d, count * sizeof(T));
        if (rc) return rc;
        p = (T*)d;
        return 0;
    }
    template <class T> int back(T* host, const T* dev, size_t count, hipStream_t s)
    {
        if (host_out && host) HIP_TRY(hipMemcpyAsync(host, dev, count * sizeof(T), hipMemcpyDeviceToHost, s));
        return 0;
    }
};


__global__ void prep_kernel(const double* __restrict__ scaling, int64_t N,
                            const double* __restrict__ alpha, const double* __restrict__ beta, int32_t G,
                            float* __restrict__ scal_f, float* __restrict__ a_f,
                            float* __restrict__ bm1_f, float* __restrict__ phi_f,
                            const int32_t* __restrict__ row_of_cell, int64_t rows, uint64_t cell_offset,
                            const int64_t* __restrict__ cell_index,
                            uint32_t k0, uint32_t k1, k3::CellInfo* __restrict__ info, int64_t* __restrict__ flags,
                            const uint8_t* __restrict__ row_bad, uint32_t parity, k3::HeavyList heavy,
                            k3::HeavyList* __restrict__ heavy_rec, k3::StripPlan plan)
{
    const int64_t i = (int64_t)blockIdx.x * blockDim.x + threadIdx.x;
    if (heavy_rec && i < k3::kSegs + 2) heavy.seg_cnt[i] = 0u;
    if (heavy_rec && i == 0) *heavy_rec = heavy;
    if (flags && i == 0) {
        flags[kListOverflow] = 0;
        flags[kFullReq + (parity ^ 1u)] = 0;
    }
    if (i < N) {
        const double sd = scaling[i];
        scal_f[i] = (float)sd;
        if (row_bad) {
            const int64_t r = row_of_cell[i];
            if (r < 0 || r >= rows) flags[kStickyRow] = 1;
            else if (row_bad[r] || !(sd > 0.0 && sd < __builtin_inf())) flags[kStickyDomain] = 1;
        }
    }
    if (i < G) {
        const float a = (float)alpha[i];
        const float bm1 = (float)(beta[i] - 1.0);
        a_f[i] = a;
        bm1_f[i] = bm1;
        phi_f[i] = prnb::zero_test_factor(a, bm1);
        if (row_bad && (!(a >= 0.0f) || !(bm1 >= 0.0f))) flags[kFullReq + parity] = 1;
    }
    if (info) {
        const int64_t n = i < N ? i : N - 1;
        auto clamped = [&](int32_t r) -> int64_t { return r < 0 ? 0 : (r >= rows ? rows - 1 : (int64_t)r); };
        int32_t row_here = row_of_cell[n], row_before = row_of_cell[n > 0 ? n - 1 : 0];
        const uint64_t cell = cell_index ? (uint64_t)cell_index[n] : cell_offset + (uint64_t)n;
        const float s_n = (float)scaling[n];
        asm volatile("" : "+v"(row_here), "+v"(row_before));
        const int64_t row = clamped(row_here);
        int32_t strip_cells = plan.c[0].strip_cells;
#pragma unroll
        for (int k = 1; k < k3::kPlanClasses; ++k)
            if (k < plan.classes && n >= plan.c[k].first_cell) strip_cells = plan.c[k].strip_cells;
        uint32_t word = 0u;
        if (strip_cells > 0 && 64 % strip_cells == 0) {
            const uint32_t lane = threadIdx.x & 63u, pos = lane & (uint32_t)(strip_cells - 1), first = lane - pos;
            const bool cell_here = i < N;
            const bool starts_run = cell_here && (pos == 0u || clamped(row_before) != row);
            const unsigned long long strip_m = (strip_cells == 64 ? ~0ull : (1ull << strip_cells) - 1ull) << first;
            const unsigned long long starts_m = __builtin_amdgcn_ballot_w64(starts_run) & strip_m;
            const unsigned long long cells_m = __builtin_amdgcn_ballot_w64(cell_here) & strip_m;
            const unsigned long long behind = starts_m & ~((2ull << lane) - 1ull);
            const uint32_t end = behind ? (uint32_t)__ffsll((long long)behind) - 1u : first + (uint32_t)__popcll(cells_m);
            word = !cell_here ? 1u : (!starts_run ? 0u : ((end - lane) | (pos == 0u ? (uint32_t)__popcll(starts_m) << 16 : 0u)));
        } else if (strip_cells != 2 * 64) {
            word = i < N + 4 ? k3::run_word(row_of_cell, i, N, rows, strip_cells) : 0u;
        }
        if (plan.c[0].strip_cells == 2 * 64) {
            __shared__ unsigned long long masks[4][2];
            const uint32_t lane = threadIdx.x & 63u, wave = threadIdx.x >> 6, half = wave & 1u;
            const bool cell_here = i < N;
            const bool starts_run = cell_here && ((lane == 0u && half == 0u) || clamped(row_before) != row);
            const unsigned long long starts_m = __builtin_amdgcn_ballot_w64(starts_run), cells_m = __builtin_amdgcn_ballot_w64(cell_here);
            if (lane == 0u) { masks[wave][0] = starts_m; masks[wave][1] = cells_m; }
            __syncthreads();
            if (strip_cells == 2 * 64) {
                const unsigned long long other_starts = masks[wave ^ 1u][0], other_cells = masks[wave ^ 1u][1];
                const uint32_t pos = half * 64u + lane;
                const uint32_t strip_end = (uint32_t)__popcll(cells_m) + (uint32_t)__popcll(other_cells);
                const unsigned long long behind = starts_m & ~((2ull << lane) - 1ull);
                const uint32_t end = behind ? half * 64u + (uint32_t)__ffsll((long long)behind) - 1u
                                            : (half == 0u && other_starts ? 64u + (uint32_t)__ffsll((long long)other_starts) - 1u : strip_end);
                const uint32_t runs = (uint32_t)__popcll(starts_m) + (uint32_t)__popcll(other_starts);
                word = !cell_here ? 1u : (!starts_run ? 0u : ((end - pos) | (pos == 0u ? runs << 16 : 0u)));
            }
        }
        if (i < N + 4) {
            k3::CellInfo c;
            c.row_bytes = (uint64_t)row * (uint64_t)G * 4u;
            c.s = s_n;
            c.runs = word;
            k3::philox_cell_part((uint32_t)cell, (uint32_t)(cell >> 32), k0, k1, c.ph);
            info[i] = c;
        }
    }
}

constexpr int kTileG = 256;

__global__ void nb_params_kernel(const float* __restrict__ means, int32_t G,
                                 const int32_t* __restrict__ row_of_cell,
                                 const float* __restrict__ scal, const float* __restrict__ ga,
                                 const float* __restrict__ gbm1, int64_t N, int64_t rows, float* __restrict__ mu,
                                 float* __restrict__ p, float* __restrict__ r,
                                 int32_t* __restrict__ path)
{
    const int64_t i = (int64_t)blockIdx.x * blockDim.x + threadIdx.x;
    if (i >= N * G) return;
    const int64_t n = i / G;
    const int32_t g = (int32_t)(i - n * G);
    int64_t row = row_of_cell[n];
    row = row < 0 ? 0 : (row >= rows ? rows - 1 : row);
    const prnb::Params P = prnb::make_params(means[row * G + g], scal[n], ga[g], gbm1[g]);
    if (mu) mu[i] = P.m;
    if (p) p[i] = P.valid ? P.theta * P.iu : 0.0f;
    if (r) r[i] = P.valid ? P.m * P.inv_th : 0.0f;
    if (path) path[i] = !P.valid ? 0 : (P.light ? 1 : 2);
}

__global__ void hw_math_kernel(int32_t op, uint32_t first_bits, uint64_t count, float* __restrict__ y)
{
    for (uint64_t i = (uint64_t)blockIdx.x * blockDim.x + threadIdx.x; i < count; i += (uint64_t)gridDim.x * blockDim.x) {
        const float x = __uint_as_float(first_bits + (uint32_t)i);
        y[i] = op == 0 ? prnb::hw_rcp(x) : (op == 1 ? prnb::hw_log2(x) : prnb::hw_exp2(-x));
    }
}

__global__ void hw_math_at_kernel(int32_t op, const float* __restrict__ x, uint64_t count, float* __restrict__ y)
{
    for (uint64_t i = (uint64_t)blockIdx.x * blockDim.x + threadIdx.x; i < count; i += (uint64_t)gridDim.x * blockDim.x) {
        const float v = x[i];
        float r;
        switch (op) {
        case 0: r = prnb::hw_rcp(v); break;
        case 1: r = prnb::hw_log2(v); break;
        case 2: r = prnb::hw_exp2(-v); break;
        case 3: r = prnb::hw_sqrt(v); break;
        case 4: r = prnb::hw_rsq(v); break;
        default: r = prnb::hw_cos(v); break;
        }
        y[i] = r;
    }
}

__device__ __forceinline__ unsigned long long ordered_bits(double x)
{
    const unsigned long long b = (unsigned long long)__double_as_longlong(x);
    return (b >> 63) ? ~b : (b | 0x8000000000000000ull);
}
static double from_ordered_bits(unsigned long long o)
{
    const unsigned long long b = (o >> 63) ? (o & 0x7fffffffffffffffull) : ~o;
    double d;
    memcpy(&d, &b, 8);
    return d;
}

constexpr int kLinChunks = 4;

template <bool HREG>
struct GeneColumn {
    const double* h;
    int64_t G;
    int32_t K;
    double reg[HREG ? 32 : 1];
    __device__ __forceinline__ GeneColumn(const double* H, int64_t g, bool live, int64_t G_, int32_t K_) : h(H + (live ? g : 0)), G(G_), K(K_)
    {
        if (HREG) {
#pragma unroll
            for (int k = 0; k < 32; ++k) reg[k] = k < K ? h[(int64_t)k * G] : 0.0;
        }
    }
// ... 208 lines not shown
}

__global__ __launch_bounds__(256) void gene_max_kernel(const double* __restrict__ rel, int64_t rows,
                                                       int64_t G, double* __restrict__ gene_max)
{
    const int c = threadIdx.x >> 6;
    const int64_t g = (int64_t)blockIdx.x * 64 + (threadIdx.x & 63);
    const int64_t r0 = ((int64_t)blockIdx.y * rows) / gridDim.y, r1 = ((int64_t)(blockIdx.y + 1) * rows) / gridDim.y;
    double mx = -std::numeric_limits<double>::infinity();
    if (g < G)
        for (int64_t t = r0 + c; t < r1; t += 4) mx = fmax(mx, rel[t * G + g]);
    fold_gene_max(mx, g < G, gene_max, g);
}

__global__ __launch_bounds__(256) void means_from_rel_kernel(const double* __restrict__ rel,
                                                             const double* __restrict__ base,
                                                             int64_t rows, int64_t G,
                                                             float* __restrict__ out)
{
    const int64_t total = rows * G;
    for (int64_t i = (int64_t)blockIdx.x * blockDim.x + threadIdx.x; i < total;
         i += (int64_t)gridDim.x * blockDim.x) {
        const int64_t g = i % G;
        const double v = exp(rel[i]) * base[g];
        out[i] = (v > 0.0 && v < 1.17549435e-38) ? 1.17549435e-38f : (float)v;
    }
}

__global__ __launch_bounds__(256) void row_flags_kernel(const float* __restrict__ means, int64_t rows, int64_t G,
                                                        uint8_t* __restrict__ row_bad)
{
    for (int64_t r = blockIdx.x; r < rows; r += gridDim.x) {
        const float* row = means + r * G;
        int bad = 0;
        for (int64_t g = threadIdx.x; g < G; g += blockDim.x) {
            const float v = row[g];
            bad |= !(v > 0.0f && v < __builtin_inff());
        }
        bad = __syncthreads_or(bad);
        if (threadIdx.x == 0) row_bad[r] = (uint8_t)(bad != 0);
    }
}


PA_EXPORT int prosstt_amd_version(void) { return PROSSTT_AMD_VERSION; }
PA_EXPORT const char* prosstt_amd_last_error(void) { return g_err; }

PA_EXPORT int prosstt_amd_device_count(int* count) try
{
    if (!count) return fail(PROSSTT_AMD_EINVAL, "count is NULL");
    *count = 0;
    hipError_t e = hipGetDeviceCount(count);
    if (e != hipSuccess) {
        *count = 0;
        return fail(PROSSTT_AMD_ENODEV, "hipGetDeviceCount: %s", hipGetErrorString(e));
    }
    return 0;
}
PA_CATCH

PA_EXPORT int prosstt_amd_ctx_create(int device, void* stream, prosstt_amd_ctx** out) try
{
    if (!out) return fail(PROSSTT_AMD_EINVAL, "out is NULL");
    *out = nullptr;
    int n = 0;
    if (hipGetDeviceCount(&n) != hipSuccess || n <= 0)
        return fail(PROSSTT_AMD_ENODEV, "no HIP device visible: the prosstt_amd path has no CPU fallback");
    if (device < 0 || device >= n) return fail(PROSSTT_AMD_EINVAL, "device %d out of range [0,%d)", device, n);
    hipDeviceProp_t prop;
    HIP_TRY(hipGetDeviceProperties(&prop, device));
    if (strncmp(prop.gcnArchName, "gfx950", 6) != 0)
        return fail(PROSSTT_AMD_ENODEV, "device %d is %s; this library is built for gfx950 only", device,
                    prop.gcnArchName);
    HIP_TRY(hipSetDevice(device));
    prosstt_amd_ctx* c = new (std::nothrow) prosstt_amd_ctx();
    if (!c) return fail(PROSSTT_AMD_ENOMEM, "out of host memory");
    c->device = device;
    c->stream = (hipStream_t)stream;
    if (hipMalloc((void**)&c->scratch, kScratchWords * 8) != hipSuccess ||
        hipHostMalloc((void**)&c->h_scratch, kScratchWords * 8) != hipSuccess) {
        prosstt_amd_ctx_destroy(c);
        return fail(PROSSTT_AMD_EHIP, "ctx allocation failed");
    }
    if (hipMemset(c->scratch, 0, kScratchWords * 8) != hipSuccess) {
        prosstt_amd_ctx_destroy(c);
        return fail(PROSSTT_AMD_EHIP, "ctx initialisation failed");
    }
    int per_cu = 0;
    if (hipOccupancyMaxActiveBlocksPerMultiprocessor(&per_cu, k3::sample_counts_heavy_kernel, k3::kHeavyBlock, 0) == hipSuccess &&
        per_cu > 0 && prop.multiProcessorCount > 0)
        c->heavy_grid = per_cu * prop.multiProcessorCount;
    if (prop.multiProcessorCount > 0) c->stream_resident = 5 * prop.multiProcessorCount;
    *out = c;
    return 0;
}
PA_CATCH

PA_EXPORT int prosstt_amd_ctx_destroy(prosstt_amd_ctx* c) try
{
    if (!c) return 0;
    (void)hipSetDevice(c->device);
    (void)hipStreamSynchronize(c->stream);
    if (c->ws) (void)hipFree(c->ws);
    if (c->scratch) (void)hipFree(c->scratch);
    if (c->row_bad) (void)hipFree(c->row_bad);
    if (c->h_scratch) (void)hipHostFree(c->h_scratch);
    for (hipEvent_t e : c->events) (void)hipEventDestroy(e);
    delete c;
    return 0;
}
PA_CATCH

PA_EXPORT int prosstt_amd_ctx_synchronize(prosstt_amd_ctx* c) try
{
    if (!c) return fail(PROSSTT_AMD_EINVAL, "ctx is NULL");
    HIP_TRY(hipStreamSynchronize(c->stream));
    return 0;
}
PA_CATCH

PA_EXPORT int prosstt_amd_last_kernel_ms(prosstt_amd_ctx* c, float* ms) try
{
    if (!c || !ms) return fail(PROSSTT_AMD_EINVAL, "NULL argument");
    if (c->events_used == 0)
        return fail(PROSSTT_AMD_EINVAL, "no kernel was launched with PROSSTT_AMD_TIME_KERNEL since the last call");
    HIP_TRY(hipEventSynchronize(c->events[c->events_used - 1]));
    double total = 0.0;
    for (size_t i = 0; i < c->events_used; i += 2) {
        float one = 0.0f;
        HIP_TRY(hipEventElapsedTime(&one, c->events[i], c->events[i + 1]));
        total += one;
    }
    *ms = (float)(total / (double)(c->events_used / 2));
    c->events_used = 0;
    return 0;
}
PA_CATCH

struct SamplerArgs {
    const float* means; const int32_t* row_of_cell;
    const int64_t* cell_index;
    float *scal, *ga, *gbm1, *gphi;
    k3::HeavyList heavy;
    k3::HeavyList* heavy_rec;
    k3::CellInfo* cellinfo;
};

struct StreamGeometry {
    k3::StripPlan plan;
    int64_t tiles_g, strip_cells, blocks;
    uint64_t regions;
    uint32_t region_cap;
    uint32_t ent_cap;
};

static long env_number(const char* name)
{
    const char* v = getenv(name);
    return v ? strtol(v, nullptr, 10) : 0;
}

static StreamGeometry stream_geometry(int64_t N, int32_t G, int resident)
{
    StreamGeometry g;
    const long forced = env_number("PROSSTT_AMD_STRIP_CELLS"), taper = env_number("PROSSTT_AMD_STRIP_TAPER");
    const long most = env_number("PROSSTT_AMD_STRIP_CLASSES");
    const bool uniform = taper <= 0 && (forced == 8 || forced == 16 || forced == 32 || forced == 64);
    g.plan = k3::strip_plan(N, G, uniform ? 0 : resident, (int32_t)(forced > 0 && forced <= k3::kStripCells ? forced : 0),
                            (int32_t)(taper > 0 && taper <= 0x7fffffffl ? taper : 0), (int32_t)(most > 0 && most <= k3::kPlanClasses ? most : 0));
    const int64_t n = N > 0 ? N : 0;
    g.tiles_g = g.plan.tiles_g;
    g.strip_cells = g.plan.c[0].strip_cells;
    g.blocks = 0;
    for (int k = 0; k < g.plan.classes; ++k) {
        const int64_t len = g.plan.c[k].strip_cells, cells = g.plan.c[k + 1].first_cell - g.plan.c[k].first_cell;
        g.blocks += (((cells + len - 1) / len + 3) / 4) * g.tiles_g;
    }
    g.regions = (uint64_t)g.blocks * 4u;
    g.region_cap = (uint32_t)g.strip_cells * (kTileG / 16);
    if (g.region_cap > 1024u) g.region_cap = 1024u;
    const uint64_t per_seg = ((uint64_t)n * (uint64_t)(G > 0 ? G : 0) / 64u + k3::kSegs - 1) / k3::kSegs;
    g.ent_cap = (uint32_t)(per_seg < 4u * g.region_cap ? 4u * g.region_cap : (per_seg > 0x7fffffffull ? 0x7fffffffull : per_seg));
    return g;
}

struct StreamWorkspace {
    k3::HeavyList heavy;
    k3::HeavyList* heavy_rec;
    k3::CellInfo* info;
    size_t bytes;
};

static StreamWorkspace stream_workspace(const StreamGeometry& g, int64_t N, char* base)
{
    size_t at = 0;
    auto take = [&](size_t bytes) {
        char* p = base ? base + at : nullptr;
        at += (bytes + 255) & ~(size_t)255;
        return p;
    };
    StreamWorkspace w{};
    w.heavy.list = (uint2*)take(g.regions * ((size_t)g.region_cap + k3::kListTail) * sizeof(uint2));
    char* counters = take(768 + sizeof(k3::HeavyList));
    static_assert((k3::kSegs + 2) * 4 <= 768, "the counters end where the record starts");
    w.heavy.seg_cnt = (uint32_t*)counters;
    w.heavy_rec = (k3::HeavyList*)(counters ? counters + 768 : nullptr);
    w.heavy.dense = (uint2*)take(g.regions * (size_t)k3::kDense * sizeof(uint2));
    w.heavy.count = (uint32_t*)take(g.regions * 4u);
    w.heavy.ent = (k3::HeavyEntry*)take((size_t)k3::kSegs * g.ent_cap * sizeof(k3::HeavyEntry));
    w.heavy.wst = (k3::f32x4_t*)take(g.regions * (size_t)k3::kWalkSlots * 16u);
    w.heavy.wid = (uint32_t*)take(g.regions * (size_t)k3::kWalkSlots * 4u);
    w.heavy.ovf_regions = (uint32_t*)take(g.regions * 4u);
    w.heavy.redo = (int2*)take((size_t)k3::kRedoCap * sizeof(int2));
    w.info = (k3::CellInfo*)take(0);
    w.bytes = at + ((size_t)N + 4) * sizeof(k3::CellInfo) + 256;
    return w;
}

static int sampler_setup(prosstt_amd_ctx* c, Staging& st, const float* means, int64_t rows, int32_t G,
                         const int32_t* row_of_cell, const double* scaling, const double* alpha,
                         const double* beta, int64_t N, uint32_t flags, SamplerArgs* A,
                         const StreamGeometry* geo, uint64_t cell_offset, const int64_t* cell_index, uint64_t seed)
{
    if (!c) return fail(PROSSTT_AMD_EINVAL, "ctx is NULL");
    if (N < 0 || G < 0 || rows < 0) return fail(PROSSTT_AMD_EINVAL, "negative size");
    if (N > 0 && G > 0 && (!means || !row_of_cell || !scaling || !alpha || !beta))
        return fail(PROSSTT_AMD_EINVAL, "NULL input array");
    if (N > 0 && G > 0 && rows == 0) return fail(PROSSTT_AMD_EINVAL, "the mean tensor has no rows");
    if ((int64_t)G * 4 > (int64_t)1 << 33) return fail(PROSSTT_AMD_EINVAL, "G too large");
    HIP_TRY(hipSetDevice(c->device));
    if (N == 0 || G == 0) return 0;
    if (st.host_in)
        for (int64_t n = 0; n < N; ++n)
            if (row_of_cell[n] < 0 || row_of_cell[n] >= rows)
                return fail(PROSSTT_AMD_EINVAL, "row_of_cell[%lld] = %d outside [0,%lld)", (long long)n,
                            row_of_cell[n], (long long)rows);
    int rc;
    if ((rc = st.in(means, (size_t)rows * G, c->stream)) || (rc = st.in(row_of_cell, (size_t)N, c->stream)) ||
        (rc = st.in(scaling, (size_t)N, c->stream)) || (rc = st.in(alpha, (size_t)G, c->stream)) ||
        (rc = st.in(beta, (size_t)G, c->stream)) || (rc = st.in(cell_index, (size_t)N, c->stream)))
        return rc;
    const int64_t n_pad = (N + 15) & ~(int64_t)15;
    const size_t vec_bytes = ((((size_t)n_pad + 3 * (size_t)G) * sizeof(float)) + 255) & ~(size_t)255;
    if ((rc = ws_reserve(c, vec_bytes + (geo ? stream_workspace(*geo, N, nullptr).bytes : 0)))) return rc;
    A->means = means;
    A->row_of_cell = row_of_cell;
    A->cell_index = cell_index;
    A->scal = (float*)c->ws;
    A->ga = A->scal + n_pad;
    A->gbm1 = A->ga + G;
    A->gphi = A->gbm1 + G;
    if (geo) {
        const StreamWorkspace w = stream_workspace(*geo, N, (char*)c->ws + vec_bytes);
        A->heavy = w.heavy;
        A->heavy.cap = geo->region_cap;
        A->heavy.ent_cap = geo->ent_cap;
        A->heavy.overflow = (uint32_t*)(c->scratch + kListOverflow);
        A->heavy_rec = w.heavy_rec;
        A->cellinfo = w.info;
    }
    const uint8_t* row_bad = nullptr;
    if (geo && (flags & (PROSSTT_AMD_CHECK_DOMAIN | PROSSTT_AMD_CHECK_DEFERRED))) {
        const bool cached = (flags & PROSSTT_AMD_MEANS_CACHED) && !(flags & PROSSTT_AMD_HOST_INPUTS) && c->row_bad &&
                            c->row_bad_means == means && c->row_bad_rows == rows && c->row_bad_G == G;
        if (!cached) {
            if ((size_t)rows > c->row_bad_cap) {
                HIP_TRY(hipStreamSynchronize(c->stream));
                if (c->row_bad) HIP_TRY(hipFree(c->row_bad));
                c->row_bad = nullptr;
                c->row_bad_cap = 0;
                c->row_bad_means = nullptr;
                HIP_TRY(hipMalloc((void**)&c->row_bad, ((size_t)rows + 4095) & ~(size_t)4095));
                c->row_bad_cap = ((size_t)rows + 4095) & ~(size_t)4095;
            }
            row_flags_kernel<<<dim3((unsigned)(rows < 65536 ? rows : 65536)), dim3(256), 0, c->stream>>>(means, rows, G, c->row_bad);
            HIP_TRY(hipGetLastError());
            c->row_bad_means = (flags & PROSSTT_AMD_HOST_INPUTS) ? nullptr : means;
            c->row_bad_rows = rows;
            c->row_bad_G = G;
        }
        row_bad = c->row_bad;
    }
    const int64_t span = (N + 4 > G ? N + 4 : G);
    prep_kernel<<<dim3((unsigned)((span + 255) / 256)), dim3(256), 0, c->stream>>>(
        scaling, N, alpha, beta, G, A->scal, A->ga, A->gbm1, A->gphi, row_of_cell, rows, cell_offset, cell_index,
        (uint32_t)seed, (uint32_t)(seed >> 32), A->cellinfo, geo ? c->scratch : nullptr,
        row_bad, c->call_parity, A->heavy, A->heavy_rec, geo ? geo->plan : k3::strip_plan(N, G, 0, 0, 0, 0));
    HIP_TRY(hipGetLastError());
    return 0;
}

static int domain_verdict(prosstt_amd_ctx* c, int64_t rows, int* verdict)
{
    HIP_TRY(hipMemcpyAsync(c->h_scratch + kStickyDomain, c->scratch + kStickyDomain, 16, hipMemcpyDeviceToHost, c->stream));
    HIP_TRY(hipMemsetAsync(c->scratch + kStickyDomain, 0, 16, c->stream));
    HIP_TRY(hipStreamSynchronize(c->stream));
    *verdict = 0;
    if (c->h_scratch[kStickyRow]) {
        *verdict = PROSSTT_AMD_EINVAL;
        if (rows >= 0) return fail(PROSSTT_AMD_EINVAL, "row_of_cell holds an index outside [0,%lld)", (long long)rows);
        return fail(PROSSTT_AMD_EINVAL, "row_of_cell of a checked call held an index outside the mean tensor");
    }
    if (c->h_scratch[kStickyDomain]) {
        *verdict = PROSSTT_AMD_EDOMAIN;
        return fail(PROSSTT_AMD_EDOMAIN, "Domain error in arguments: a mean that is not positive and finite, or alpha*m + beta < 1");
    }
    return 0;
}

PA_EXPORT int prosstt_amd_domain_status(prosstt_amd_ctx* c, int32_t* status) try
{
    if (!c) return fail(PROSSTT_AMD_EINVAL, "ctx is NULL");
    HIP_TRY(hipSetDevice(c->device));
    int verdict = 0;
    const int rc = domain_verdict(c, -1, &verdict);
    if (status) *status = verdict;
    return (rc == PROSSTT_AMD_EHIP) ? rc : 0;
}
PA_CATCH

PA_EXPORT int prosstt_amd_plan_order(const int32_t* row_of_cell, int64_t N, int64_t rows, int32_t* order) try
{
    if (N < 0 || rows < 0 || N > 0x7fffffffll) return fail(PROSSTT_AMD_EINVAL, "bad size");
    if (N > 0 && (!row_of_cell || !order)) return fail(PROSSTT_AMD_EINVAL, "NULL argument");
    std::vector<int64_t> first((size_t)rows + 1, 0);
    for (int64_t n = 0; n < N; ++n) {
        if (row_of_cell[n] < 0 || row_of_cell[n] >= rows)
            return fail(PROSSTT_AMD_EINVAL, "row_of_cell[%lld] = %d outside [0,%lld)", (long long)n, row_of_cell[n], (long long)rows);
        first[(size_t)row_of_cell[n] + 1] += 1;
    }
    for (int64_t r = 0; r < rows; ++r) first[(size_t)r + 1] += first[(size_t)r];
    for (int64_t n = 0; n < N; ++n) order[first[(size_t)row_of_cell[n]]++] = (int32_t)n;
    return 0;
}
PA_CATCH

PA_EXPORT int prosstt_amd_run_plan(const int32_t* row_of_cell, int64_t N, int64_t rows, int32_t strip_cells, uint32_t* words) try
{
    if (N < 0 || rows < 1 || N > 0x7fffffffll) return fail(PROSSTT_AMD_EINVAL, "bad size");
    if (strip_cells < 1 || strip_cells > k3::kStripCells) return fail(PROSSTT_AMD_EINVAL, "strip_cells outside [1,%d]", k3::kStripCells);
    if (!words || (N > 0 && !row_of_cell)) return fail(PROSSTT_AMD_EINVAL, "NULL argument");
    for (int64_t i = 0; i < N + 4; ++i) words[i] = k3::run_word(row_of_cell, i, N, rows, strip_cells);
    return 0;
}
PA_CATCH

PA_EXPORT int prosstt_amd_last_run_plan(prosstt_amd_ctx* c, uint32_t* words, int64_t cap, int64_t* total, int32_t* strip_cells) try
{
    if (!c || !total) return fail(PROSSTT_AMD_EINVAL, "NULL argument");
    if (cap > 0 && !words) return fail(PROSSTT_AMD_EINVAL, "NULL output array");
    *total = 0;
    if (strip_cells) *strip_cells = 0;
    if (!c->list.seg_cnt || !c->list_info) return 0;
    HIP_TRY(hipSetDevice(c->device));
    HIP_TRY(hipStreamSynchronize(c->stream));
    *total = c->list_cells + 4;
    if (strip_cells) *strip_cells = c->list_plan.c[0].strip_cells;
    const int64_t n = cap < *total ? cap : *total;
    if (n > 0)
        HIP_TRY(hipMemcpy2D(words, 4, (const char*)c->list_info + offsetof(k3::CellInfo, runs), sizeof(k3::CellInfo), 4, (size_t)n,
                            hipMemcpyDeviceToHost));
    return 0;
}
PA_CATCH

static void plan_out(const k3::StripPlan& p, int32_t* classes, int32_t* n_classes, int32_t* tiles_g, int32_t* blocks)
{
    for (int k = 0; k < p.classes; ++k) {
        classes[3 * k] = p.c[k].first_cell;
        classes[3 * k + 1] = p.c[k].strip_cells;
        classes[3 * k + 2] = p.c[k].first_block;
    }
    *n_classes = p.classes;
    if (tiles_g) *tiles_g = p.tiles_g;
    if (blocks) *blocks = p.c[p.classes].first_block;
}

PA_EXPORT int prosstt_amd_strip_plan(int64_t N, int32_t G, int32_t resident_blocks, int32_t strip_cells, int32_t taper,
                                     int32_t* classes, int32_t* n_classes, int32_t* tiles_g, int32_t* blocks) try
{
    if (N < 0 || G < 0 || N > 0x7fffffffll || resident_blocks < 0 || taper < 0) return fail(PROSSTT_AMD_EINVAL, "bad size");
    if (strip_cells != 0 && strip_cells != 8 && strip_cells != 16 && strip_cells != 32 && strip_cells != 64 && strip_cells != 128)
        return fail(PROSSTT_AMD_EINVAL, "strip_cells is not 0, 8, 16, 32, 64 or 128");
    if (!classes || !n_classes) return fail(PROSSTT_AMD_EINVAL, "NULL argument");
    plan_out(k3::strip_plan(N, G, resident_blocks, strip_cells, taper, 0), classes, n_classes, tiles_g, blocks);
    return 0;
}
PA_CATCH

PA_EXPORT int prosstt_amd_last_strip_plan(prosstt_amd_ctx* c, int32_t* classes, int32_t* n_classes, int32_t* tiles_g, int32_t* blocks) try
{
    if (!c || !classes || !n_classes) return fail(PROSSTT_AMD_EINVAL, "NULL argument");
    *n_classes = 0;
    if (tiles_g) *tiles_g = 0;
    if (blocks) *blocks = 0;
    if (!c->list.seg_cnt) return 0;
    plan_out(c->list_plan, classes, n_classes, tiles_g, blocks);
    return 0;
}
PA_CATCH

PA_EXPORT int prosstt_amd_sample_counts(prosstt_amd_ctx* c, const float* means, int64_t rows, int32_t G,
                                        const int32_t* row_of_cell, const double* scaling,
                                        const double* alpha, const double* beta, int64_t N,
                                        uint64_t seed, uint64_t cell_offset, const int64_t* cell_index,
                                        int32_t* out, int64_t ld_out, uint32_t flags) try
{
    Staging st(flags);
    SamplerArgs A{};
    if (N > 0 && G > 0) {
        if (!out) return fail(PROSSTT_AMD_EINVAL, "out is NULL");
        if (ld_out < G) return fail(PROSSTT_AMD_EINVAL, "ld_out %lld < G %d", (long long)ld_out, G);
        if (ld_out * k3::kStripCells >= ((int64_t)1 << 29))
            return fail(PROSSTT_AMD_EINVAL, "ld_out too large: a strip's rows must span less than 2 GiB");
        if (N > 0x7fffffffll) return fail(PROSSTT_AMD_EINVAL, "too many cells; chunk them");
        if ((uint64_t)(rows > 0 ? rows : 0) * (uint64_t)G >= ((uint64_t)1 << 61)) return fail(PROSSTT_AMD_EINVAL, "mean tensor too large");
    }
    const StreamGeometry geo = stream_geometry(N, G, c ? c->stream_resident : 0);
    if (geo.blocks > 0x1fffffffll) return fail(PROSSTT_AMD_EINVAL, "too many tiles; chunk the cells");
    int rc = sampler_setup(c, st, means, rows, G, row_of_cell, scaling, alpha, beta, N, flags, &A, &geo, cell_offset,
                           cell_index, seed);
    if (rc) return rc;
    if (N == 0 || G == 0) return 0;
    const k3::HeavyList heavy = A.heavy;
    k3::CellInfo* cellinfo = A.cellinfo;
    const int64_t* d_cell_index = A.cell_index;
    int32_t* d_out = out;
    if ((rc = st.out(d_out, (size_t)N * ld_out))) return rc;

    const bool vec = (G % 4 == 0) && (ld_out % 4 == 0) && (((uintptr_t)A.means & 15) == 0) &&
                     (((uintptr_t)d_out & 15) == 0);
    const uint32_t k0 = (uint32_t)seed, k1 = (uint32_t)(seed >> 32);
    const bool checked = (flags & (PROSSTT_AMD_CHECK_DOMAIN | PROSSTT_AMD_CHECK_DEFERRED)) != 0;
    hipEvent_t ev_start = nullptr, ev_stop = nullptr;
    if (flags & PROSSTT_AMD_TIME_KERNEL) {
        if ((rc = next_event_pair(c, &ev_start, &ev_stop))) return rc;
    }
    const dim3 grid((unsigned)geo.blocks), block(k3::kBlock);
    const bool big = geo.strip_cells >= k3::kStripCells / 2 && (double)N * (double)ld_out * 4.0 >= 1073741824.0;
#define K3_LAUNCH(V, B)                                                                                          \
    hipExtLaunchKernelGGL((k3::sample_counts_stream_kernel<V, B>), grid, block, 0, c->stream, ev_start, ev_stop, 0,  \
        A.means, G, (const k3::CellInfo*)cellinfo, (const float*)A.ga, (const float*)A.gbm1, (const float*)A.gphi, N, k0, k1, \
        d_out, ld_out, geo.plan, heavy.list, heavy.cap, heavy.dense, (const k3::HeavyList*)A.heavy_rec)
    if (vec && big) K3_LAUNCH(true, true);
    else if (vec) K3_LAUNCH(true, false);
    else if (big) K3_LAUNCH(false, true);
    else K3_LAUNCH(false, false);
#undef K3_LAUNCH
    HIP_TRY(hipGetLastError());
    const uint64_t region_blocks = (geo.regions + 15u) / 16u;
    const unsigned heavy_blocks = (unsigned)(region_blocks < 256u ? 256u : (region_blocks < (uint64_t)c->heavy_grid ? region_blocks : (uint64_t)c->heavy_grid));
    k3::sample_counts_heavy_kernel<<<dim3(heavy_blocks), dim3(k3::kHeavyBlock), 0, c->stream>>>(
        (const k3::HeavyList*)A.heavy_rec, (uint32_t)geo.regions, geo.plan, A.means, rows, G, A.row_of_cell,
        A.scal, A.ga, A.gbm1, N, k0, k1, cell_offset, d_cell_index, d_out, ld_out,
        (checked && !(flags & PROSSTT_AMD_PARAMS_NONNEG)) ? c->scratch : nullptr, (uint32_t)kFullReq + c->call_parity,
        (uint32_t)kStickyRow, (uint32_t)kStickyDomain);
    HIP_TRY(hipGetLastError());
    c->list = heavy;
    c->list_regions = geo.regions;
    c->list_plan = geo.plan;
    c->list_info = cellinfo;
    c->list_cells = N;
    c->call_parity ^= 1u;
    if (st.host_out)
        HIP_TRY(hipMemcpy2DAsync(out, (size_t)ld_out * 4, d_out, (size_t)ld_out * 4, (size_t)G * 4, (size_t)N,
                                 hipMemcpyDeviceToHost, c->stream));
    if (flags & PROSSTT_AMD_CHECK_DOMAIN) {
        int verdict = 0;
        rc = domain_verdict(c, rows, &verdict);
        if (rc) return rc;
    } else if (st.host_in || st.host_out) {
        HIP_TRY(hipStreamSynchronize(c->stream));
    }
    return 0;
}
PA_CATCH

PA_EXPORT int prosstt_amd_last_list(prosstt_amd_ctx* c, int64_t* cells, int32_t* genes, int64_t cap,
                                    int64_t* total, int32_t* overflowed) try
{
    if (!c || !total) return fail(PROSSTT_AMD_EINVAL, "NULL argument");
    if (cap > 0 && (!cells || !genes)) return fail(PROSSTT_AMD_EINVAL, "NULL output array");
    *total = 0;
    if (overflowed) *overflowed = 0;
    if (!c->list.seg_cnt) return 0;
    HIP_TRY(hipSetDevice(c->device));
    HIP_TRY(hipStreamSynchronize(c->stream));
    int64_t overflow = 0;
    HIP_TRY(hipMemcpy(&overflow, c->scratch + kListOverflow, 8, hipMemcpyDeviceToHost));
    if (overflowed) *overflowed = (int32_t)((uint32_t)overflow != 0u);
    int64_t written = 0;
    std::vector<uint32_t> counts(c->list_regions);
    HIP_TRY(hipMemcpy(counts.data(), c->list.count, counts.size() * 4, hipMemcpyDeviceToHost));
    uint2 dense[k3::kDense];
    uint32_t wid[k3::kWalkSlots];
    for (uint64_t r = 0; r < c->list_regions; ++r) {
        const uint32_t listed = counts[r] & 0xffffu, walks = counts[r] >> 16;
        const uint32_t nd = listed > c->list.cap ? 0u : (listed < (uint32_t)k3::kDense ? listed : (uint32_t)k3::kDense);
        *total += nd + walks;
        if (nd + walks == 0 || written >= cap) continue;
        if (nd) HIP_TRY(hipMemcpy(dense, c->list.dense + r * k3::kDense, (size_t)nd * sizeof(uint2), hipMemcpyDeviceToHost));
        if (walks) HIP_TRY(hipMemcpy(wid, c->list.wid + r * k3::kWalkSlots, (size_t)walks * 4, hipMemcpyDeviceToHost));
        const k3::StripAt at = k3::strip_of_region(c->list_plan, (uint32_t)r);
        const int64_t tile_g = at.tile_g, n0 = at.n0;
        for (uint32_t i = 0; i < nd + walks && written < cap; ++i, ++written) {
            const uint32_t pos = i < nd ? dense[i].x : (wid[i - nd] & 0xffffu);
            cells[written] = n0 + (pos >> 8);
            genes[written] = (int32_t)(tile_g * kTileG + (pos & 255u));
        }
    }
    uint32_t fill[k3::kSegs];
    HIP_TRY(hipMemcpy(fill, c->list.seg_cnt, sizeof(fill), hipMemcpyDeviceToHost));
    std::vector<k3::HeavyEntry> ent;
    for (int sg = 0; sg < k3::kSegs; ++sg) {
        const uint32_t ne = fill[sg] < c->list.ent_cap ? fill[sg] : c->list.ent_cap;
        *total += (int64_t)ne;
        if (written >= cap || ne == 0) continue;
        ent.resize(ne);
        HIP_TRY(hipMemcpy(ent.data(), c->list.ent + (size_t)sg * c->list.ent_cap, (size_t)ne * sizeof(k3::HeavyEntry), hipMemcpyDeviceToHost));
        for (uint32_t i = 0; i < ne && written < cap; ++i, ++written) {
            cells[written] = ent[i].n;
            genes[written] = ent[i].g;
        }
    }
    return 0;
}
PA_CATCH

PA_EXPORT int prosstt_amd_nb_params(prosstt_amd_ctx* c, const float* means, int64_t rows, int32_t G,
                                    const int32_t* row_of_cell, const double* scaling,
                                    const double* alpha, const double* beta, int64_t N, float* mu,
                                    float* p, float* r, int32_t* path, uint32_t flags) try
{
    Staging st(flags);
    SamplerArgs A{};
    int rc = sampler_setup(c, st, means, rows, G, row_of_cell, scaling, alpha, beta, N, flags, &A, nullptr, 0, nullptr, 0);
    if (rc) return rc;
    if (N == 0 || G == 0) return 0;
    const int64_t total = N * (int64_t)G;
    float *d_mu = mu, *d_p = p, *d_r = r;
    int32_t* d_path = path;
    if ((rc = st.out(d_mu, total)) || (rc = st.out(d_p, total)) || (rc = st.out(d_r, total)) || (rc = st.out(d_path, total))) return rc;
    nb_params_kernel<<<dim3((unsigned)((total + 255) / 256)), dim3(256), 0, c->stream>>>(
        A.means, G, A.row_of_cell, A.scal, A.ga, A.gbm1, N, rows, d_mu, d_p, d_r, d_path);
    HIP_TRY(hipGetLastError());
    if ((rc = st.back(mu, d_mu, total, c->stream)) || (rc = st.back(p, d_p, total, c->stream)) ||
        (rc = st.back(r, d_r, total, c->stream)) || (rc = st.back(path, d_path, total, c->stream)))
        return rc;
    if (st.host_in || st.host_out) HIP_TRY(hipStreamSynchronize(c->stream));
    return 0;
}
PA_CATCH

PA_EXPORT int prosstt_amd_hw_math(prosstt_amd_ctx* c, int32_t op, uint32_t first_bits, uint64_t count, float* out,
                                  uint32_t flags) try
{
    if (!c || !out) return fail(PROSSTT_AMD_EINVAL, "NULL argument");
    if (op < 0 || op > 2) return fail(PROSSTT_AMD_EINVAL, "op must be 0 (rcp), 1 (log2) or 2 (exp2 of -x)");
    if ((uint64_t)first_bits + count > ((uint64_t)1 << 32)) return fail(PROSSTT_AMD_EINVAL, "the range leaves the 32-bit patterns");
    if (count == 0) return 0;
    HIP_TRY(hipSetDevice(c->device));
    Staging st(flags);
    float* d = out;
    int rc;
    if ((rc = st.out(d, count))) return rc;
    const uint64_t blocks = (count + 255) / 256;
    hw_math_kernel<<<dim3((unsigned)(blocks < 65536 ? blocks : 65536)), dim3(256), 0, c->stream>>>(op, first_bits, count, d);
    HIP_TRY(hipGetLastError());
    if ((rc = st.back(out, d, count, c->stream))) return rc;
    if (st.host_out) HIP_TRY(hipStreamSynchronize(c->stream));
    return 0;
}
PA_CATCH

PA_EXPORT int prosstt_amd_hw_math_at(prosstt_amd_ctx* c, int32_t op, const float* x, uint64_t count, float* out,
                                     uint32_t flags) try
{
    if (!c || !out || !x) return fail(PROSSTT_AMD_EINVAL, "NULL argument");
    if (op < 0 || op > 5) return fail(PROSSTT_AMD_EINVAL, "op must be 0 (rcp), 1 (log2), 2 (exp2 of -x), 3 (sqrt), 4 (rsq) or 5 (cos of x revolutions)");
    if (count == 0) return 0;
    HIP_TRY(hipSetDevice(c->device));
    Staging st(flags);
    const float* dx = x;
    float* dy = out;
    int rc;
    if ((rc = st.in(dx, count, c->stream)) || (rc = st.out(dy, count))) return rc;
    const uint64_t blocks = (count + 255) / 256;
    hw_math_at_kernel<<<dim3((unsigned)(blocks < 65536 ? blocks : 65536)), dim3(256), 0, c->stream>>>(op, dx, count, dy);
    HIP_TRY(hipGetLastError());
    if ((rc = st.back(out, dy, count, c->stream))) return rc;
    if (st.host_in || st.host_out) HIP_TRY(hipStreamSynchronize(c->stream));
    return 0;
}
PA_CATCH

#include <dlfcn.h>
namespace rccl {
typedef struct { char internal[128]; } UniqueId;
typedef void* Comm;
enum { kInt32 = 2, kUint8 = 1 };
static int (*GetUniqueId)(UniqueId*) = nullptr;
static int (*CommInitRank)(Comm*, int, UniqueId, int) = nullptr;
static int (*CommDestroy)(Comm) = nullptr;
static int (*Send)(const void*, size_t, int, int, Comm, hipStream_t) = nullptr;
static int (*Recv)(void*, size_t, int, int, Comm, hipStream_t) = nullptr;
static int (*GroupStart)() = nullptr;
static int (*GroupEnd)() = nullptr;
static const char* (*GetErrorString)(int) = nullptr;
static bool open()
{
    if (GroupEnd) return true;
    void* h = nullptr;
    for (const char* name : {"librccl.so.1", "librccl.so", "/opt/rocm/lib/librccl.so.1"})
        if ((h = dlopen(name, RTLD_NOW | RTLD_GLOBAL))) break;
    if (!h) return false;
    auto sym = [&](const char* n) { return dlsym(h, n); };
    GetUniqueId = (int (*)(UniqueId*))sym("ncclGetUniqueId");
    CommInitRank = (int (*)(Comm*, int, UniqueId, int))sym("ncclCommInitRank");
    CommDestroy = (int (*)(Comm))sym("ncclCommDestroy");
    Send = (int (*)(const void*, size_t, int, int, Comm, hipStream_t))sym("ncclSend");
    Recv = (int (*)(void*, size_t, int, int, Comm, hipStream_t))sym("ncclRecv");
    GroupStart = (int (*)())sym("ncclGroupStart");
    GetErrorString = (const char* (*)(int))sym("ncclGetErrorString");
    auto ge = (int (*)())sym("ncclGroupEnd");
    if (!GetUniqueId || !CommInitRank || !CommDestroy || !Send || !Recv || !GroupStart || !ge) return false;
    GroupEnd = ge;
    return true;
}
}

struct prosstt_amd_comm { rccl::Comm comm = nullptr; int32_t rank = 0, world = 1; };

#define RCCL_TRY(expr)                                                                                   \
    do {                                                                                                 \
        int r_ = (expr);                                                                                 \
        if (r_ != 0) return fail(PROSSTT_AMD_ERCCL, "%s: %s", #expr, rccl::GetErrorString ? rccl::GetErrorString(r_) : "RCCL error"); \
    } while (0)

PA_EXPORT int prosstt_amd_comm_unique_id(void* id_out) try
{
    if (!id_out) return fail(PROSSTT_AMD_EINVAL, "NULL argument");
    if (!rccl::open()) return fail(PROSSTT_AMD_ERCCL, "librccl.so.1 could not be opened: %s", dlerror());
    rccl::UniqueId id;
    RCCL_TRY(rccl::GetUniqueId(&id));
    memcpy(id_out, &id, sizeof(id));
    return 0;
}
PA_CATCH

PA_EXPORT int prosstt_amd_comm_init(prosstt_amd_ctx* c, const void* id, int32_t rank, int32_t world, prosstt_amd_comm** out) try
{
    if (!c || !id || !out) return fail(PROSSTT_AMD_EINVAL, "NULL argument");
    if (world < 1 || rank < 0 || rank >= world) return fail(PROSSTT_AMD_EINVAL, "rank %d of %d", rank, world);
    if (!rccl::open()) return fail(PROSSTT_AMD_ERCCL, "librccl.so.1 could not be opened: %s", dlerror());
    HIP_TRY(hipSetDevice(c->device));
    rccl::UniqueId uid;
    memcpy(&uid, id, sizeof(uid));
    prosstt_amd_comm* k = new prosstt_amd_comm;
    k->rank = rank;
// ... 278 lines not shown
```

### prosstt_amd/device.py

```python
import ctypes
import os
import threading
import warnings
import weakref

import numpy as np

from . import _native


def _torch():
    import torch
    return torch


def require_gpu():
    _native.load()
    torch = _torch()
    if not torch.cuda.is_available() or _native.device_count() == 0:
        raise RuntimeError("prosstt_amd needs an AMD MI355X (gfx950) device: there is no CPU fallback")


def _ptr(t):
    return ctypes.c_void_p(t.data_ptr()) if t is not None else None


def need_device(name):
    L = _native.load(name)
    if not _torch().cuda.is_available():
        raise RuntimeError("prosstt_amd needs an AMD MI355X (gfx950) device: there is no CPU fallback")
    return L


def current_stream(dev):
    return ctypes.c_void_p(_torch().cuda.current_stream(dev).cuda_stream)


def workspace(name, query_symbol, dev, *sizes):
    need = ctypes.c_uint64(0)
    _native.check(getattr(_native.load(name), query_symbol)(*sizes, ctypes.byref(need)), name)
    return _torch().empty(max(int(need.value), 1), dtype=_torch().uint8, device=dev)


class Context:

    def __init__(self, device=None):
        require_gpu()
        torch = _torch()
        self.device = torch.cuda.current_device() if device is None else int(device)
        self.torch_device = torch.device("cuda", self.device)
        self.stream = torch.cuda.current_stream(self.device)
        self._lib = _native.load()
        handle = ctypes.c_void_p()
        _native.check(self._lib.prosstt_amd_ctx_create(
            self.device, ctypes.c_void_p(self.stream.cuda_stream), ctypes.byref(handle)))
        self._h = handle
        self._checked_means = None

    def close(self):
        if getattr(self, "_h", None):
            self._lib.prosstt_amd_ctx_destroy(self._h)
            self._h = None

    def __del__(self):
        try:
            self.close()
        except Exception:
            pass

    def tensor(self, array, dtype):
        torch = _torch()
        if isinstance(array, torch.Tensor):
            return array.to(device=self.torch_device, dtype=dtype).contiguous()
        host = np.ascontiguousarray(array)
        if not host.flags.writeable:
            host = host.copy()
        return torch.as_tensor(host, dtype=dtype).to(self.torch_device)

    def synchronize(self):
        _native.check(self._lib.prosstt_amd_ctx_synchronize(self._h))

    def last_kernel_ms(self):
        ms = ctypes.c_float(0)
        _native.check(self._lib.prosstt_amd_last_kernel_ms(self._h, ctypes.byref(ms)))
        return ms.value

    def sample_counts(self, means, row_of_cell, scaling, alpha, beta, seed, cell_offset=0,
                      out=None, check_domain=True, time_kernel=False, cell_index=None, means_token=None):
        torch = _torch()
        means = self.tensor(means, torch.float32)
        rows, G = means.shape
        row_of_cell = self.tensor(row_of_cell, torch.int32)
        N = row_of_cell.numel()
        scaling = self.tensor(scaling, torch.float64)
        nonneg = bool(check_domain) and self._params_nonneg(alpha, beta)
        alpha = self.tensor(alpha, torch.float64)
        beta = self.tensor(beta, torch.float64)
        if scaling.numel() != N or alpha.numel() != G or beta.numel() != G:
            raise ValueError("scaling must have one entry per cell, alpha/beta one per gene")
        if out is None:
            out = torch.empty((N, G), dtype=torch.int32, device=self.torch_device)
        elif out.dtype != torch.int32 or out.shape != (N, G) or out.stride(1) != 1:
            raise ValueError("out must be an int32 (N, G) tensor with unit column stride")
        if cell_index is not None:
            cell_index = self.tensor(cell_index, torch.int64)
            if cell_index.numel() != N:
                raise ValueError("cell_index must have one entry per cell")
        if check_domain not in (True, False, "deferred"):
            raise ValueError("check_domain must be True, False or 'deferred'")
        flags = _native.TIME_KERNEL if time_kernel else 0
        if check_domain:
            flags |= _native.CHECK_DEFERRED if check_domain == "deferred" else _native.CHECK_DOMAIN
            if nonneg:
                flags |= _native.PARAMS_NONNEG
            key = (means.data_ptr(), rows, G, means_token)
            if means_token is not None and key == self._checked_means:
                flags |= _native.MEANS_CACHED
            self._checked_means = None
        _native.check(self._lib.prosstt_amd_sample_counts(
            self._h, _ptr(means), rows, G, _ptr(row_of_cell), _ptr(scaling), _ptr(alpha), _ptr(beta),
            N, ctypes.c_uint64(seed & (2 ** 64 - 1)), ctypes.c_uint64(cell_offset), _ptr(cell_index),
            _ptr(out), out.stride(0) if N else G, flags))
        if check_domain and N and G and means_token is not None:
            self._checked_means = key
        return out

    def _params_nonneg(self, alpha, beta):
        torch = _torch()
        for arr, floor in ((alpha, 0.0), (beta, 1.0)):
            if isinstance(arr, torch.Tensor) or not bool(np.all(np.asarray(arr) >= floor)):
                return False
        return True

    def domain_status(self):
        status = ctypes.c_int32(0)
        _native.check(self._lib.prosstt_amd_domain_status(self._h, ctypes.byref(status)))
        _native.check(status.value)

    def last_list(self, cap=1 << 22):
        cells = np.empty(cap, np.int64)
        genes = np.empty(cap, np.int32)
        total = ctypes.c_int64(0)
        over = ctypes.c_int32(0)
        _native.check(self._lib.prosstt_amd_last_list(
            self._h, cells.ctypes.data_as(ctypes.c_void_p), genes.ctypes.data_as(ctypes.c_void_p), cap,
            ctypes.byref(total), ctypes.byref(over)))
        n = min(cap, total.value)
        return cells[:n], genes[:n], total.value, bool(over.value)

    def last_run_plan(self):
        total = ctypes.c_int64(0)
        strip = ctypes.c_int32(0)
        _native.check(self._lib.prosstt_amd_last_run_plan(self._h, None, 0, ctypes.byref(total), ctypes.byref(strip)))
        words = np.empty(total.value, np.uint32)
        _native.check(self._lib.prosstt_amd_last_run_plan(
            self._h, words.ctypes.data_as(ctypes.c_void_p), words.size, ctypes.byref(total), ctypes.byref(strip)))
        return words, strip.value

    def last_strip_plan(self):
        classes = np.zeros((4, 3), np.int32)
        n, tiles, blocks = ctypes.c_int32(0), ctypes.c_int32(0), ctypes.c_int32(0)
        _native.check(self._lib.prosstt_amd_last_strip_plan(
            self._h, classes.ctypes.data_as(ctypes.c_void_p), ctypes.byref(n), ctypes.byref(tiles), ctypes.byref(blocks)))
        return classes[:n.value].copy(), tiles.value, blocks.value

    HW_OPS = dict(rcp=0, log2=1, exp2neg=2)

    def hw_math(self, op, first_bits, count):
        out = np.empty(int(count), np.float32)
        _native.check(self._lib.prosstt_amd_hw_math(
            self._h, self.HW_OPS[op], ctypes.c_uint32(first_bits), ctypes.c_uint64(int(count)),
            out.ctypes.data_as(ctypes.c_void_p), _native.HOST_OUTPUT))
        return out

    HW_OPS_AT = dict(rcp=0, log2=1, exp2neg=2, sqrt=3, rsq=4, cos=5)

    def hw_math_at(self, op, x):
        x = np.ascontiguousarray(x, np.float32)
        out = np.empty(x.size, np.float32)
        code = self.HW_OPS_AT[op] if isinstance(op, str) else int(op)
        _native.check(self._lib.prosstt_amd_hw_math_at(
            self._h, code, x.ctypes.data_as(ctypes.c_void_p), ctypes.c_uint64(x.size),
            out.ctypes.data_as(ctypes.c_void_p), _native.HOST_OUTPUT | _native.HOST_INPUTS))
        return out

    def nb_params(self, means, row_of_cell, scaling, alpha, beta):
        torch = _torch()
        means = self.tensor(means, torch.float32)
        rows, G = means.shape
        row_of_cell = self.tensor(row_of_cell, torch.int32)
        N = row_of_cell.numel()
        scaling = self.tensor(scaling, torch.float64)
        alpha = self.tensor(alpha, torch.float64)
        beta = self.tensor(beta, torch.float64)
        mu = torch.empty((N, G), dtype=torch.float32, device=self.torch_device)
        p = torch.empty_like(mu)
        r = torch.empty_like(mu)
        path = torch.empty((N, G), dtype=torch.int32, device=self.torch_device)
        _native.check(self._lib.prosstt_amd_nb_params(
            self._h, _ptr(means), rows, G, _ptr(row_of_cell), _ptr(scaling), _ptr(alpha), _ptr(beta),
            N, _ptr(mu), _ptr(p), _ptr(r), _ptr(path), 0))
        return mu, p, r, path

    def lineage_attempt_batch(self, programs, H, sib_programs=()):
        programs = np.ascontiguousarray(programs, np.float64)
        if programs.ndim != 3:
            raise ValueError("programs must be (B, T, K)")
        B, T, K = programs.shape
        H = self._coefficients(H, K)
        sibs = [np.ascontiguousarray(s, np.float64) for s in sib_programs]
        n = len(sibs)
        for s in sibs:
            if s.ndim != 2 or s.shape[1] != K:
                raise ValueError("sibling programs must have %d columns" % K)
        ptrs = (ctypes.c_void_p * max(n, 1))(*[s.ctypes.data for s in sibs])
        lens = (ctypes.c_int32 * max(n, 1))(*[s.shape[0] for s in sibs])
        top = np.empty(B, np.float64)
        counts = np.zeros((B, max(n, 1)), np.int64)
        _native.check(self._lib.prosstt_amd_lineage_attempt_batch(
            self._h, programs.ctypes.data_as(ctypes.c_void_p), B, T, K, _ptr(H), H.shape[1], n,
            ctypes.cast(ptrs, ctypes.c_void_p), ctypes.cast(lens, ctypes.c_void_p),
            top.ctypes.data_as(ctypes.c_void_p), counts.ctypes.data_as(ctypes.c_void_p)))
        return top, counts[:, :n]

    def lineage_attempt(self, programs, H, sib_programs=()):
        top, counts = self.lineage_attempt_batch(np.asarray(programs, np.float64)[None], H, sib_programs)
        return float(top[0]), [int(c) for c in counts[0]]

    def lineage_walk(self, seed, stream_id, T, K):
        out = np.empty((T, K), np.float64)
        _native.check(self._lib.prosstt_amd_lineage_walk(
            self._h, ctypes.c_uint64(seed & (2 ** 64 - 1)), ctypes.c_uint64(stream_id), T, K,
            out.ctypes.data_as(ctypes.c_void_p)))
        return out

    def lineage_walks(self, seed, stream_ids, T, K):
        ids = [int(i) for i in stream_ids]
        if not ids:
            return np.empty((0, T, K), np.float64)
        if ids != list(range(ids[0], ids[0] + len(ids))):
            return np.stack([self.lineage_walk(seed, i, T, K) for i in ids])
        out = np.empty((len(ids), T, K), np.float64)
        _native.check(self._lib.prosstt_amd_lineage_walk_batch(
            self._h, ctypes.c_uint64(seed & (2 ** 64 - 1)), ctypes.c_uint64(ids[0]), len(ids), T, K,
            out.ctypes.data_as(ctypes.c_void_p)))
        return out

    def lineage_commit(self, programs, H, rel_out=None, gene_max=None):
        torch = _torch()
        programs = np.ascontiguousarray(programs, np.float64)
        if programs.ndim != 2:
            raise ValueError("programs must be (T, K)")
        T, K = programs.shape
        H = self._coefficients(H, K)
        G = H.shape[1]
        self._output(rel_out, "rel_out", torch.float64, (T, G))
        self._output(gene_max, "gene_max", torch.float64, (G,))
        _native.check(self._lib.prosstt_amd_lineage_commit(
            self._h, programs.ctypes.data_as(ctypes.c_void_p), T, K, _ptr(H), H.shape[1],
            _ptr(rel_out), _ptr(gene_max)))

    def gene_max(self, rel, gene_max):
        torch = _torch()
        rel = self.tensor(rel, torch.float64)
        if rel.dim() != 2:
            raise ValueError("rel must be (rows, G)")
        self._output(gene_max, "gene_max", torch.float64, (rel.shape[1],))
        if rel.numel():
            _native.check(self._lib.prosstt_amd_gene_max(self._h, _ptr(rel), rel.shape[0], rel.shape[1], _ptr(gene_max)))
        return gene_max

    def means_from_rel(self, rel, base, out=None):
        torch = _torch()
        rel = self.tensor(rel, torch.float64)
        if rel.dim() != 2:
            raise ValueError("rel must be (rows, G)")
        rows, G = rel.shape
        base = self.tensor(base, torch.float64)
        if base.shape != (G,):
            raise ValueError("base must have one entry per gene")
        if out is None:
            out = torch.empty((rows, G), dtype=torch.float32, device=self.torch_device)
        self._output(out, "out", torch.float32, (rows, G))
        if out.numel():
            _native.check(self._lib.prosstt_amd_means_from_rel(self._h, _ptr(rel), _ptr(base), rows, G, _ptr(out)))
        return out

    def _coefficients(self, H, K):
        H = self.tensor(H, _torch().float64)
        if H.dim() != 2 or H.shape[0] != K or H.shape[1] == 0:
            raise ValueError("H must be (%d, G >= 1), not %s" % (K, tuple(H.shape)))
        return H

    def _output(self, t, name, dtype, shape):
        if t is None:
            return
        torch = _torch()
        if not isinstance(t, torch.Tensor):
            raise TypeError("%s must be a torch tensor on %s" % (name, self.torch_device))
        if t.device != self.torch_device:
            raise ValueError("%s is on %s, not on %s" % (name, t.device, self.torch_device))
        if t.dtype != dtype:
            raise TypeError("%s must be %s, not %s" % (name, dtype, t.dtype))
        if tuple(t.shape) != tuple(shape):
            raise ValueError("%s must have shape %s, not %s" % (name, tuple(shape), tuple(t.shape)))
        if not t.is_contiguous():
            raise ValueError("%s must be contiguous" % name)


def plan_order(row_of_cell, rows=None):
    roc = np.ascontiguousarray(row_of_cell, dtype=np.int32)
    order = np.empty(roc.size, dtype=np.int32)
    if roc.size:
        n_rows = int(roc.max()) + 1 if rows is None else int(rows)
        _native.check(_native.load().prosstt_amd_plan_order(
            roc.ctypes.data_as(ctypes.c_void_p), roc.size, n_rows, order.ctypes.data_as(ctypes.c_void_p)))
    return order

# ... 503 lines not shown
```

Before: 850.0 billion.

## Fuse heavy-entry sampling into the stream kernel via per-group tail processing

Splits the heavy sampling kernel body into a reusable device routine (heavy_work) and runs it inside the main stream kernel. Groups of blocks handle the heavy list, staged overflow entries, redo entries and walks for their own regions once those regions are done, so the separate heavy kernel launch is skipped unless full domain checking is requested. The aim is to remove a kernel launch and the serialized tail phase, and to overlap heavy work with light sampling. In exchange it adds group counters and workspace, changes how staged list entries are read, and puts more register and LDS pressure on the fused kernel.

Measured after the change: 847.1 billion. About the same (-0.3%).

```diff
diff --git a/include/prosstt_amd_heavy.h b/include/prosstt_amd_heavy.h
--- /dev/null
+++ b/include/prosstt_amd_heavy.h
@@ -0,0 +1,21 @@
+#ifndef PROSSTT_AMD_HEAVY_H
+#define PROSSTT_AMD_HEAVY_H
+
+#include "prosstt_amd.h"
+
+#ifdef __cplusplus
+extern "C" {
+#endif
+
+int prosstt_amd_heavy_groups(int64_t blocks, int32_t* group, int64_t* groups, int32_t* last);
+
+int prosstt_amd_heavy_workspace(int64_t N, int32_t G, int32_t resident_blocks, int64_t* counters_offset,
+                                int64_t* counters_bytes, int64_t* total_bytes);
+
+int prosstt_amd_last_heavy_mode(prosstt_amd_ctx* ctx, int32_t* fused, int32_t* heavy_launches, int64_t* groups);
+
+#ifdef __cplusplus
+}
+#endif
+
+#endif
diff --git a/prosstt_amd/_native.py b/prosstt_amd/_native.py
--- a/prosstt_amd/_native.py
+++ b/prosstt_amd/_native.py
@@ -192,6 +192,13 @@
 })
 
 
+SAMPLER_HEAVY = ("prosstt_amd_heavy.h", {
+    "prosstt_amd_heavy_groups": _int(i64, _ptr_to(i32), _ptr_to(i64), _ptr_to(i32)),
+    "prosstt_amd_heavy_workspace": _int(i64, i32, i32, _ptr_to(i64), _ptr_to(i64), _ptr_to(i64)),
+    "prosstt_amd_last_heavy_mode": _int(vp, _ptr_to(i32), _ptr_to(i32), _ptr_to(i64)),
+})
+
+
 def _library(name):
     for table in (LIBRARIES, ADDED_LIBRARIES, LATER_LIBRARIES):
         if name in table:
@@ -220,7 +227,7 @@
             if lib.hip:
                 import torch
             L = ctypes.CDLL(lib.path)
-            symbols = dict(lib.symbols, **SAMPLER_LATER[1]) if name == "sampler" else lib.symbols
+            symbols = dict(lib.symbols, **SAMPLER_LATER[1], **SAMPLER_HEAVY[1]) if name == "sampler" else lib.symbols
             for symbol, (restype, argtypes) in symbols.items():
                 fn = getattr(L, symbol)
                 fn.restype = restype
diff --git a/prosstt_amd/csrc/k3_heavy.h b/prosstt_amd/csrc/k3_heavy.h
--- a/prosstt_amd/csrc/k3_heavy.h
+++ b/prosstt_amd/csrc/k3_heavy.h
@@ -21,38 +21,10 @@
     uint16_t wk[kWCap];
 };
 
-__global__ __launch_bounds__(kHeavyBlock) void sample_counts_heavy_kernel(
-    const HeavyList* __restrict__ heavy_ptr, uint32_t regions, StripPlan plan,
-    const float* __restrict__ means, int64_t rows,
-    int32_t G, const int32_t* __restrict__ row_of_cell, const float* __restrict__ scal,
-    const float* __restrict__ ga, const float* __restrict__ gbm1, int64_t N, uint32_t k0, uint32_t k1,
-    uint64_t cell_offset, const int64_t* __restrict__ cell_index, int32_t* __restrict__ out, int64_t ld,
-    int64_t* __restrict__ check_words, uint32_t check_request, uint32_t check_bad_row, uint32_t check_verdict)
+struct ClassRec { int32_t first_cell, end_cell; uint32_t first_block, groups, groups_rcp, log2_len, pad[2]; };
+
+__device__ __forceinline__ void class_table(ClassRec* cls_tab, const StripPlan& plan, int tid)
 {
-    __shared__ __attribute__((aligned(16))) float inv_k_store[prnb::kTabShift + prnb::kKTab];
-    float* const inv_k = inv_k_store + prnb::kTabShift;
-    __shared__ HeavyLds lds_all[kHeavyBlock / 64];
-    const HeavyList heavy = *heavy_ptr;
-    const int tid = threadIdx.x, lane = tid & 63, wv = __builtin_amdgcn_readfirstlane(tid >> 6);
-    HeavyLds& L = lds_all[wv];
-    for (int k = tid - prnb::kTabShift; k < prnb::kKTab; k += kHeavyBlock) inv_k[k] = k > 0 ? 1.0f / (float)k : 0.0f;
-    __shared__ uint32_t seg_n[kSegs], seg_first[kSegs + 1];
-    if (wv == 0) {
-        uint32_t n = heavy.seg_cnt[lane];
-        n = n < heavy.ent_cap ? n : heavy.ent_cap;
-        uint32_t x = (n + 63u) >> 6;
-        const uint32_t mine = x;
-#pragma unroll
-        for (int d = 1; d < 64; d <<= 1) {
-            const uint32_t t = (uint32_t)__shfl_up((int)x, d, 64);
-            if (lane >= d) x += t;
-        }
-        seg_n[lane] = n;
-        seg_first[lane] = x - mine;
-        if (lane == 63) seg_first[kSegs] = x;
-    }
-    struct ClassRec { int32_t first_cell, end_cell; uint32_t first_block, groups, groups_rcp, log2_len, pad[2]; };
-    __shared__ __attribute__((aligned(16))) ClassRec cls_tab[kPlanClasses];
     if (tid < kPlanClasses) {
         static_assert(kPlanClasses == 4, "spelled out below");
         const StripClass c0 = plan.c[0], c1 = plan.c[1], c2 = plan.c[2], c3 = plan.c[3];
@@ -71,17 +43,50 @@
         c.log2_len = sh; c.pad[0] = c.pad[1] = 0u;
         cls_tab[tid] = c;
     }
-    __syncthreads();
-    const uint32_t waves = gridDim.x * (kHeavyBlock / 64);
+}
+
+typedef uint32_t u32x2_t __attribute__((ext_vector_type(2)));
+static_assert(sizeof(uint2) == sizeof(u32x2_t) && sizeof(uint4) == sizeof(u32x4_t), "read as plain vectors");
+struct HeavyRec {
+    K3_GLOBAL(const u32x2_t) list; uint32_t cap; K3_GLOBAL(const u32x4_t) dense4; K3_GLOBAL(const uint32_t) count;
+    K3_GLOBAL(const f32x4_t) wst; K3_GLOBAL(const uint32_t) wid; K3_GLOBAL(const uint32_t) seg_cnt;
+    K3_GLOBAL(const u32x4_t) ent; uint32_t ent_cap; K3_GLOBAL(const uint32_t) ovf_regions; K3_GLOBAL(const i32x2_t) redo;
+    K3_GLOBAL(const float) means; int64_t rows; int32_t G; K3_GLOBAL(const int32_t) row_of_cell;
+    K3_GLOBAL(const float) scal; K3_GLOBAL(const float) ga; K3_GLOBAL(const float) gbm1; uint32_t k0, k1;
+    uint64_t cell_offset; K3_GLOBAL(const int64_t) cell_index; K3_GLOBAL(int32_t) out; int64_t ld;
+    uint32_t fb1, fb2, fb3;
+};
+__device__ __forceinline__ void heavy_rec_lists(HeavyRec& R, const HeavyList& h)
+{
+    R.list = (K3_GLOBAL(const u32x2_t))h.list; R.cap = h.cap; R.dense4 = (K3_GLOBAL(const u32x4_t))h.dense;
+    R.count = (K3_GLOBAL(const uint32_t))h.count; R.wst = (K3_GLOBAL(const f32x4_t))h.wst; R.wid = (K3_GLOBAL(const uint32_t))h.wid;
+    R.seg_cnt = (K3_GLOBAL(const uint32_t))h.seg_cnt; R.ent = (K3_GLOBAL(const u32x4_t))h.ent; R.ent_cap = h.ent_cap;
+    R.ovf_regions = (K3_GLOBAL(const uint32_t))h.ovf_regions; R.redo = (K3_GLOBAL(const i32x2_t))h.redo;
+}
+
+struct HeavyDeal {
+    uint32_t regions, block, blocks;
+    const uint32_t *seg_n, *seg_first;
+    uint32_t first, end; bool last;
+};
+
+template <bool FUSED>
+__device__ __forceinline__ void heavy_work(const HeavyRec& heavy, const HeavyDeal& deal, const float* inv_k, HeavyLds& L,
+                                           const ClassRec* cls_tab, int lane, int wv)
+{
+    const auto means = heavy.means; const int64_t rows = heavy.rows; const int32_t G = heavy.G;
+    const auto row_of_cell = heavy.row_of_cell; const auto scal = heavy.scal; const auto ga = heavy.ga; const auto gbm1 = heavy.gbm1;
+    const uint32_t k0 = heavy.k0, k1 = heavy.k1; const uint64_t cell_offset = heavy.cell_offset;
+    const auto cell_index = heavy.cell_index; const auto out = heavy.out; const int64_t ld = heavy.ld;
     auto locate = [&](uint32_t chunk, uint32_t& seg, uint32_t& first) __attribute__((always_inline)) {
         uint32_t lo = 0u;
 #pragma unroll
         for (uint32_t step = kSegs / 2; step != 0u; step >>= 1)
-            if (seg_first[lo + step] <= chunk) lo += step;
+            if (deal.seg_first[lo + step] <= chunk) lo += step;
         seg = lo;
-        first = (chunk - seg_first[lo]) << 6;
-    };
-    const uint32_t fb1 = (uint32_t)plan.c[1].first_block, fb2 = (uint32_t)plan.c[2].first_block, fb3 = (uint32_t)plan.c[3].first_block;
+        first = (chunk - deal.seg_first[lo]) << 6;
+    };
+    const uint32_t fb1 = heavy.fb1, fb2 = heavy.fb2, fb3 = heavy.fb3;
     struct Origin { int32_t tile_g, n0, cells; };
     auto region_origin = [&](uint32_t r) __attribute__((always_inline)) -> Origin {
         const uint32_t blk = r >> 2;
@@ -373,10 +378,6 @@
         while (hg_top >= 64) gamma_pass();
     };
 
-    const uint32_t wave_id = blockIdx.x * (kHeavyBlock / 64) + (uint32_t)wv;
-    const bool walker = (blockIdx.x & 15u) < kWalkerBlocks;
-    const uint32_t walker_blocks = (gridDim.x >> 4) * kWalkerBlocks + ((gridDim.x & 15u) < kWalkerBlocks ? (gridDim.x & 15u) : kWalkerBlocks);
-    const uint32_t n_redo = heavy.seg_cnt[kSegs + 1] < (uint32_t)kRedoCap ? heavy.seg_cnt[kSegs + 1] : (uint32_t)kRedoCap;
     auto push_entries = [&](bool has, int32_t n, int32_t g, float m) __attribute__((always_inline)) {
         const unsigned long long mh = __builtin_amdgcn_ballot_w64(has);
         if (has) {
@@ -387,64 +388,71 @@
         hg_top += __popcll(mh);
         while (hg_top >= 64) gamma_pass();
     };
-    if (!walker) {
-        const uint32_t blk_rank = blockIdx.x - ((blockIdx.x >> 4) * kWalkerBlocks + ((blockIdx.x & 15u) < kWalkerBlocks ? (blockIdx.x & 15u) : kWalkerBlocks));
-        const uint32_t rank = blk_rank * (kHeavyBlock / 64) + (uint32_t)wv;
-        const uint32_t drawers = (gridDim.x - walker_blocks) * (kHeavyBlock / 64);
-        {
-            const int sub = lane >> 4, sl = lane & 15;
-            const uint4* const dense4 = reinterpret_cast<const uint4*>(heavy.dense);
-            struct Step { uint32_t cnt; uint4 d4; Origin o; };
-            auto load_step = [&](uint64_t r0) __attribute__((always_inline)) -> Step {
-                Step S;
-                S.cnt = 0u; S.d4 = make_uint4(0u, 0u, 0u, 0u);
-                const uint64_t r = r0 + (uint64_t)sub * drawers;
-                S.o = region_origin((uint32_t)r);
-                if (r < (uint64_t)regions) {
-                    S.cnt = heavy.count[r] & 0xffffu;
-                    S.d4 = dense4[r * (kDense / 2) + (uint32_t)sl];
-                }
-                return S;
-            };
-            Step nxt = load_step(rank);
-            for (uint64_t r0 = rank; r0 < (uint64_t)regions; r0 += 4ull * drawers) {
-                const Step cur = nxt;
-                nxt = load_step(r0 + 4ull * drawers);
-                const uint32_t cnt = cur.cnt > heavy.cap ? 0u : cur.cnt;
-                const int32_t tile_g = cur.o.tile_g, n0 = cur.o.n0;
-                push_entries(2u * (uint32_t)sl < cnt, n0 + (int32_t)(cur.d4.x >> 8), tile_g * kTileG + (int32_t)(cur.d4.x & 255u), __uint_as_float(cur.d4.y));
-                push_entries(2u * (uint32_t)sl + 1u < cnt, n0 + (int32_t)(cur.d4.z >> 8), tile_g * kTileG + (int32_t)(cur.d4.z & 255u), __uint_as_float(cur.d4.w));
-            }
-        }
-        {
-            const uint32_t chunks = seg_first[kSegs];
-            HeavyEntry nx;
-            nx.n = 0; nx.g = 0; nx.m = 0.0f; nx.pad = 0u;
-            bool nx_has = false;
-            auto request = [&](uint32_t chunk) __attribute__((always_inline)) {
-                uint32_t sg, first;
-                locate(chunk, sg, first);
-                nx_has = first + (uint32_t)lane < seg_n[sg];
-                if (nx_has) nx = heavy.ent[(uint64_t)sg * heavy.ent_cap + first + (uint32_t)lane];
-            };
-            if (rank < chunks) request(rank);
-            for (uint32_t chunk = rank; chunk < chunks; chunk += drawers) {
-                const HeavyEntry e = nx;
-                const bool has = nx_has;
-                if (chunk + drawers < chunks) request(chunk + drawers);
-                push_entries(has, e.n, e.g, e.m);
-            }
-        }
-    } else {
-        const uint32_t wrank = ((blockIdx.x >> 4) * kWalkerBlocks + (blockIdx.x & 15u)) * (kHeavyBlock / 64) + (uint32_t)wv;
-        const uint32_t walkers = walker_blocks * (kHeavyBlock / 64);
-        for (uint32_t i = wrank * 64u; i < n_redo; i += walkers * 64u) {
+    auto read_dense = [&](uint32_t first, uint32_t stride, uint32_t end) __attribute__((always_inline)) {
+        const int sub = lane >> 4, sl = lane & 15;
+        struct Step { uint32_t cnt; u32x4_t d4; Origin o; };
+        auto load_step = [&](uint64_t r0) __attribute__((always_inline)) -> Step {
+            Step S;
+            S.cnt = 0u; S.d4 = u32x4_t{0u, 0u, 0u, 0u};
+            const uint64_t r = r0 + (uint64_t)sub * stride;
+            S.o = region_origin((uint32_t)r);
+            if (r < (uint64_t)end) {
+                S.cnt = heavy.count[r] & 0xffffu;
+                S.d4 = heavy.dense4[r * (kDense / 2) + (uint32_t)sl];
+            }
+            return S;
+        };
+        Step nxt = load_step(first);
+        for (uint64_t r0 = first; r0 < (uint64_t)end; r0 += 4ull * stride) {
+            const Step cur = nxt;
+            nxt = load_step(r0 + 4ull * stride);
+            const uint32_t cnt = cur.cnt > heavy.cap ? 0u : cur.cnt;
+            const int32_t tile_g = cur.o.tile_g, n0 = cur.o.n0;
+            push_entries(2u * (uint32_t)sl < cnt, n0 + (int32_t)(cur.d4.x >> 8), tile_g * kTileG + (int32_t)(cur.d4.x & 255u), __uint_as_float(cur.d4.y));
+            push_entries(2u * (uint32_t)sl + 1u < cnt, n0 + (int32_t)(cur.d4.z >> 8), tile_g * kTileG + (int32_t)(cur.d4.z & 255u), __uint_as_float(cur.d4.w));
+        }
+    };
+    auto read_segments = [&](uint32_t first, uint32_t stride) __attribute__((always_inline)) {
+        const uint32_t chunks = deal.seg_first[kSegs];
+        u32x4_t nx = {0u, 0u, 0u, 0u};
+        bool nx_has = false;
+        auto request = [&](uint32_t chunk) __attribute__((always_inline)) {
+            uint32_t sg, at;
+            locate(chunk, sg, at);
+            nx_has = at + (uint32_t)lane < deal.seg_n[sg];
+            if (nx_has) nx = heavy.ent[(uint64_t)sg * heavy.ent_cap + at + (uint32_t)lane];
+        };
+        if (first < chunks) request(first);
+        for (uint32_t chunk = first; chunk < chunks; chunk += stride) {
+            const u32x4_t e = nx;
+            const bool has = nx_has;
+            if (chunk + stride < chunks) request(chunk + stride);
+            push_entries(has, (int32_t)e.x, (int32_t)e.y, __uint_as_float(e.z));
+        }
+    };
+    auto read_staged = [&](uint32_t first, uint32_t stride, uint32_t end) __attribute__((always_inline)) {
+        for (uint32_t r = first; r < end; r += stride) {
+            const uint32_t cnt = (uint32_t)__builtin_amdgcn_readfirstlane((int32_t)(heavy.count[r] & 0xffffu));
+            if (cnt <= (uint32_t)kDense || cnt > heavy.cap) continue;
+            const Origin o = region_origin(r);
+            K3_GLOBAL(const u32x2_t) const mine = heavy.list + (uint64_t)r * (heavy.cap + (uint32_t)kListTail);
+            for (uint32_t i = (uint32_t)kDense; i < cnt; i += 64u) {
+                const bool has = i + (uint32_t)lane < cnt;
+                const u32x2_t e = has ? mine[i + (uint32_t)lane] : u32x2_t{0u, 0u};
+                push_entries(has, o.n0 + (int32_t)(e.x >> 8), o.tile_g * kTileG + (int32_t)(e.x & 255u), __uint_as_float(e.y));
+            }
+        }
+    };
+    auto read_redo = [&](uint32_t first, uint32_t stride) __attribute__((always_inline)) {
+        const uint32_t listed = heavy.seg_cnt[kSegs + 1];
+        const uint32_t n_redo = listed < (uint32_t)kRedoCap ? listed : (uint32_t)kRedoCap;
+        for (uint32_t i = first; i < n_redo; i += stride) {
             const bool has = i + (uint32_t)lane < n_redo;
-            const int2 ng = has ? heavy.redo[i + (uint32_t)lane] : make_int2(0, 0);
+            const i32x2_t ng = has ? heavy.redo[i + (uint32_t)lane] : i32x2_t{0, 0};
             from_start(has, ng.x, ng.y);
         }
-        const uint32_t per_walker = ((regions + walkers - 1u) / walkers + 15u) & ~15u;
-        const uint32_t r_end = (wrank + 1u) * per_walker < regions ? (wrank + 1u) * per_walker : regions;
+    };
+    auto read_walks = [&](uint32_t first, uint32_t r_end) __attribute__((always_inline)) {
         const uint32_t rl = (uint32_t)lane >> 2, s0 = (uint32_t)lane & 3u;
         static_assert(kWalkSlots <= 12, "three slots per lane");
         struct WStep { uint32_t n_walks; f32x4_t st[3]; uint32_t id[3]; Origin o; };
@@ -468,8 +476,8 @@
             }
             return S;
         };
-        WStep wn = load_wstep(wrank * per_walker);
-        for (uint32_t rb = wrank * per_walker; rb < r_end; rb += 16u) {
+        WStep wn = load_wstep(first);
+        for (uint32_t rb = first; rb < r_end; rb += 16u) {
             const WStep cur = wn;
             wn = load_wstep(rb + 16u);
             const int32_t tile_g = cur.o.tile_g, n0 = cur.o.n0;
@@ -480,24 +488,101 @@
                           (int32_t)(cur.id[j] >> 16) - 3, cur.st[j]);
             }
         }
-    }
-    {
+    };
+    auto redo_region = [&](uint32_t r) __attribute__((always_inline)) {
+        const Origin o = region_origin(r);
+        const int32_t tg = o.tile_g;
+        const int64_t nb = o.n0;
+        for (int32_t c = 0; c < o.cells; ++c)
+            for (int j = 0; j < 4; ++j) {
+                const int32_t g = tg * kTileG + j * 64 + lane;
+                from_start(g < G, (int32_t)(nb + c), g);
+            }
+    };
+
+    if constexpr (!FUSED) {
+        const uint32_t regions = deal.regions, blk = deal.block, blocks = deal.blocks;
+        const bool walker = (blk & 15u) < kWalkerBlocks;
+        const uint32_t walker_blocks = (blocks >> 4) * kWalkerBlocks + ((blocks & 15u) < kWalkerBlocks ? (blocks & 15u) : kWalkerBlocks);
+        if (!walker) {
+            const uint32_t blk_rank = blk - ((blk >> 4) * kWalkerBlocks + ((blk & 15u) < kWalkerBlocks ? (blk & 15u) : kWalkerBlocks));
+            const uint32_t rank = blk_rank * (kHeavyBlock / 64) + (uint32_t)wv;
+            const uint32_t drawers = (blocks - walker_blocks) * (kHeavyBlock / 64);
+            read_dense(rank, drawers, regions);
+            read_segments(rank, drawers);
+        } else {
+            const uint32_t wrank = ((blk >> 4) * kWalkerBlocks + (blk & 15u)) * (kHeavyBlock / 64) + (uint32_t)wv;
+            const uint32_t walkers = walker_blocks * (kHeavyBlock / 64);
+            read_redo(wrank * 64u, walkers * 64u);
+            const uint32_t per_walker = ((regions + walkers - 1u) / walkers + 15u) & ~15u;
+            const uint32_t r_first = wrank * per_walker;
+            read_walks(r_first, r_first + per_walker < regions ? r_first + per_walker : regions);
+        }
+        const uint32_t wave_id = blk * (kHeavyBlock / 64) + (uint32_t)wv, waves = blocks * (kHeavyBlock / 64);
         const uint32_t n_ovf = heavy.seg_cnt[kSegs];
-        for (uint32_t i = wave_id; i < n_ovf; i += waves) {
-            const uint32_t r = heavy.ovf_regions[i];
-            const Origin o = region_origin(r);
-            const int32_t tg = o.tile_g;
-            const int64_t nb = o.n0;
-            for (int32_t c = 0; c < o.cells; ++c)
-                for (int j = 0; j < 4; ++j) {
-                    const int32_t g = tg * kTileG + j * 64 + lane;
-                    from_start(g < G, (int32_t)(nb + c), g);
-                }
-        }
+        for (uint32_t i = wave_id; i < n_ovf; i += waves) redo_region(heavy.ovf_regions[i]);
+    } else {
+        const uint32_t mine = deal.first + (uint32_t)wv;
+        read_dense(mine, 4u, deal.end);
+        read_staged(mine, 4u, deal.end);
+        if (deal.last) read_redo((uint32_t)wv * 64u, (kBlock / 64) * 64u);
+        const uint32_t per_wave = (deal.end - deal.first + 3u) >> 2;
+        const uint32_t w_first = deal.first + (uint32_t)wv * per_wave;
+        read_walks(w_first, w_first + per_wave < deal.end ? w_first + per_wave : deal.end);
+        for (uint32_t r = mine; r < deal.end; r += 4u)
+            if ((uint32_t)__builtin_amdgcn_readfirstlane((int32_t)(heavy.count[r] & 0xffffu)) > heavy.cap) redo_region(r);
     }
     walk_service(true);
     while (hg_top > 0) gamma_pass();
     while (hp_top > 0) poisson_pass();
+}
+
+__global__ __launch_bounds__(kHeavyBlock) void sample_counts_heavy_kernel(
+    const HeavyList* __restrict__ heavy_ptr, uint32_t regions, StripPlan plan,
+    const float* __restrict__ means, int64_t rows,
+    int32_t G, const int32_t* __restrict__ row_of_cell, const float* __restrict__ scal,
+    const float* __restrict__ ga, const float* __restrict__ gbm1, int64_t N, uint32_t k0, uint32_t k1,
+    uint64_t cell_offset, const int64_t* __restrict__ cell_index, int32_t* __restrict__ out, int64_t ld,
+    int64_t* __restrict__ check_words, uint32_t check_request, uint32_t check_bad_row, uint32_t check_verdict)
+{
+    __shared__ __attribute__((aligned(16))) float inv_k_store[prnb::kTabShift + prnb::kKTab];
+    float* const inv_k = inv_k_store + prnb::kTabShift;
+    __shared__ HeavyLds lds_all[kHeavyBlock / 64];
+    __shared__ uint32_t seg_n[kSegs], seg_first[kSegs + 1];
+    __shared__ __attribute__((aligned(16))) ClassRec cls_tab[kPlanClasses];
+    const int tid = threadIdx.x, lane = tid & 63, wv = __builtin_amdgcn_readfirstlane(tid >> 6);
+    if (regions != 0u) {
+        const HeavyList heavy = *heavy_ptr;
+        for (int k = tid - prnb::kTabShift; k < prnb::kKTab; k += kHeavyBlock) inv_k[k] = k > 0 ? 1.0f / (float)k : 0.0f;
+        if (wv == 0) {
+            uint32_t n = heavy.seg_cnt[lane];
+            n = n < heavy.ent_cap ? n : heavy.ent_cap;
+            uint32_t x = (n + 63u) >> 6;
+            const uint32_t mine = x;
+#pragma unroll
+            for (int d = 1; d < 64; d <<= 1) {
+                const uint32_t t = (uint32_t)__shfl_up((int)x, d, 64);
+                if (lane >= d) x += t;
+            }
+            seg_n[lane] = n;
+            seg_first[lane] = x - mine;
+            if (lane == 63) seg_first[kSegs] = x;
+        }
+        class_table(cls_tab, plan, tid);
+        __syncthreads();
+        HeavyRec R;
+        heavy_rec_lists(R, heavy);
+        R.means = (K3_GLOBAL(const float))means; R.rows = rows; R.G = G; R.row_of_cell = (K3_GLOBAL(const int32_t))row_of_cell;
+        R.scal = (K3_GLOBAL(const float))scal; R.ga = (K3_GLOBAL(const float))ga; R.gbm1 = (K3_GLOBAL(const float))gbm1;
+        R.k0 = k0; R.k1 = k1; R.cell_offset = cell_offset; R.cell_index = (K3_GLOBAL(const int64_t))cell_index;
+        R.out = (K3_GLOBAL(int32_t))out; R.ld = ld;
+        R.fb1 = (uint32_t)plan.c[1].first_block; R.fb2 = (uint32_t)plan.c[2].first_block; R.fb3 = (uint32_t)plan.c[3].first_block;
+        HeavyDeal deal;
+        deal.regions = regions; deal.block = blockIdx.x; deal.blocks = gridDim.x;
+        deal.seg_n = seg_n; deal.seg_first = seg_first;
+        deal.first = deal.end = 0u; deal.last = false;
+        heavy_work<false>(R, deal, inv_k, lds_all[wv], cls_tab, lane, wv);
+    }
 
     if (check_words && check_words[check_request] != 0 && check_words[check_bad_row] == 0) {
         bool bad = false;
@@ -514,4 +599,70 @@
     }
 }
 
+struct EpilogueLds {
+    __attribute__((aligned(16))) float inv_k_store[prnb::kTabShift + prnb::kKTab];
+    HeavyLds waves[kBlock / 64];
+    __attribute__((aligned(16))) ClassRec cls_tab[kPlanClasses];
+    uint32_t owner;
+};
+static_assert(sizeof(EpilogueLds) <= sizeof(StreamLds::epilogue) && sizeof(StreamLds) <= 32000, "five blocks per CU");
+static_assert(kBlock == kHeavyBlock, "the passes' stacks are per wave of either kernel");
+
+__device__ __forceinline__ void group_epilogue(StreamLds& lds, const HeavyList* heavy_ptr, uint32_t group)
+{
+    if (group == 0u) return;
+    const HeavyList* p = heavy_ptr;
+    asm volatile("" : "+s"(p));
+    const __attribute__((address_space(4))) HeavyList* h = (const __attribute__((address_space(4))) HeavyList*)p;
+    EpilogueLds& E = *reinterpret_cast<EpilogueLds*>(lds.epilogue);
+    const int tid = threadIdx.x, lane = tid & 63, wv = __builtin_amdgcn_readfirstlane(tid >> 6);
+    const uint32_t regions = h->call.regions;
+    const uint32_t my_group = blockIdx.x / group;
+    __builtin_amdgcn_s_waitcnt(0x0F70);
+    __syncthreads();
+    if (tid == 0) {
+        const uint32_t groups = h->call.groups;
+        const uint32_t size = my_group + 1u < groups ? group : (regions >> 2) - my_group * group;
+        K3_GLOBAL(uint32_t) cnt = (K3_GLOBAL(uint32_t))h->call.grp_cnt;
+        uint32_t word = 0u;
+        if (__hip_atomic_fetch_add(cnt + my_group, 1u, __ATOMIC_ACQ_REL, __HIP_MEMORY_SCOPE_AGENT) + 1u == size) {
+            word = 1u;
+            if (__hip_atomic_fetch_add(cnt + groups, 1u, __ATOMIC_ACQ_REL, __HIP_MEMORY_SCOPE_AGENT) + 1u == groups) word = 3u;
+        }
+        E.owner = word;
+    }
+    __syncthreads();
+    const uint32_t word = (uint32_t)__builtin_amdgcn_readfirstlane((int32_t)E.owner);
+    if ((word & 1u) == 0u) return;
+    float* const inv_k = E.inv_k_store + prnb::kTabShift;
+    for (int k = tid - prnb::kTabShift; k < prnb::kKTab; k += kBlock) inv_k[k] = k > 0 ? 1.0f / (float)k : 0.0f;
+    StripPlan plan;
+    plan.classes = h->call.plan.classes; plan.tiles_g = h->call.plan.tiles_g;
+#pragma unroll
+    for (int k = 0; k <= kPlanClasses; ++k) {
+        plan.c[k].first_cell = h->call.plan.c[k].first_cell;
+        plan.c[k].strip_cells = h->call.plan.c[k].strip_cells;
+        plan.c[k].first_block = h->call.plan.c[k].first_block;
+    }
+    class_table(E.cls_tab, plan, tid);
+    __syncthreads();
+    HeavyRec R;
+    R.list = (K3_GLOBAL(const u32x2_t))h->list; R.cap = h->cap; R.dense4 = (K3_GLOBAL(const u32x4_t))h->dense;
+    R.count = (K3_GLOBAL(const uint32_t))h->count; R.wst = (K3_GLOBAL(const f32x4_t))h->wst; R.wid = (K3_GLOBAL(const uint32_t))h->wid;
+    R.seg_cnt = (K3_GLOBAL(const uint32_t))h->seg_cnt; R.ent = (K3_GLOBAL(const u32x4_t))h->ent; R.ent_cap = h->ent_cap;
+    R.ovf_regions = (K3_GLOBAL(const uint32_t))h->ovf_regions; R.redo = (K3_GLOBAL(const i32x2_t))h->redo;
+    R.means = (K3_GLOBAL(const float))h->call.means; R.rows = h->call.rows; R.G = h->call.G;
+    R.row_of_cell = (K3_GLOBAL(const int32_t))h->call.row_of_cell; R.scal = (K3_GLOBAL(const float))h->call.scal;
+    R.ga = (K3_GLOBAL(const float))h->call.ga; R.gbm1 = (K3_GLOBAL(const float))h->call.gbm1;
+    R.k0 = h->call.k0; R.k1 = h->call.k1; R.cell_offset = h->call.cell_offset;
+    R.cell_index = (K3_GLOBAL(const int64_t))h->call.cell_index; R.out = (K3_GLOBAL(int32_t))h->call.out; R.ld = h->call.ld;
+    R.fb1 = (uint32_t)plan.c[1].first_block; R.fb2 = (uint32_t)plan.c[2].first_block; R.fb3 = (uint32_t)plan.c[3].first_block;
+    HeavyDeal deal;
+    deal.regions = regions; deal.block = 0u; deal.blocks = 1u; deal.seg_n = nullptr; deal.seg_first = nullptr;
+    deal.first = my_group * group * 4u;
+    deal.end = deal.first + group * 4u < regions ? deal.first + group * 4u : regions;
+    deal.last = (word & 2u) != 0u;
+    heavy_work<true>(R, deal, inv_k, E.waves[wv], E.cls_tab, lane, wv);
 }
+
+}
diff --git a/prosstt_amd/csrc/k3_stream.h b/prosstt_amd/csrc/k3_stream.h
--- a/prosstt_amd/csrc/k3_stream.h
+++ b/prosstt_amd/csrc/k3_stream.h
@@ -166,7 +166,24 @@
 constexpr int kDense = 32;
 constexpr int kWalkSlots = kBail + kLongSlots;
 struct HeavyEntry { int32_t n, g; float m; uint32_t pad; };
+constexpr int kHeavyGroup = 8;
+struct HeavyGroups { uint32_t groups, last; };
+__host__ __device__ inline HeavyGroups heavy_groups(uint32_t blocks, uint32_t group)
+{
+    HeavyGroups g;
+    g.groups = group ? (blocks + group - 1u) / group : 0u;
+    g.last = g.groups ? blocks - (g.groups - 1u) * group : 0u;
+    return g;
+}
+struct HeavyCall {
+    const float* means; int64_t rows; const int32_t* row_of_cell; const float *scal, *ga, *gbm1;
+    const int64_t* cell_index; uint64_t cell_offset; int32_t* out; int64_t ld;
+    uint32_t* grp_cnt;
+    int32_t G; uint32_t k0, k1, regions, group, groups;
+    StripPlan plan;
+};
 struct HeavyList {
+    HeavyCall call;
     uint2* list; uint32_t cap;
     uint2* dense;
     uint32_t* count;
@@ -191,8 +208,20 @@
 typedef uint32_t u32x4_t __attribute__((ext_vector_type(4)));
 typedef int32_t i32x2_t __attribute__((ext_vector_type(2)));
 static_assert(sizeof(HeavyEntry) == sizeof(u32x4_t) && sizeof(int2) == sizeof(i32x2_t), "stored as plain vectors");
+struct StripLds {
+    uint8_t ring_all[kBlock / 64][kRing * 256];
+    WaveLds lds_all[kBlock / 64];
+    __attribute__((aligned(16))) float inv_k_store[prnb::kTabShift + kInvTab + 2];
+};
+union StreamLds {
+    StripLds strip;
+    __attribute__((aligned(16))) unsigned char epilogue[30736];
+};
+__device__ __forceinline__ void group_epilogue(StreamLds& lds, const HeavyList* heavy_ptr, uint32_t group);
+
 template <bool VEC, bool BIG>
-__global__ __launch_bounds__(kBlock, 5) void sample_counts_stream_kernel(
+__device__ __forceinline__ uint32_t stream_strip(
+    StripLds& lds,
     const float* __restrict__ means, int32_t G, const CellInfo* __restrict__ cellinfo,
     const float* __restrict__ ga, const float* __restrict__ gbm1, const float* __restrict__ gphi,
     int64_t N, uint32_t k0, uint32_t k1, int32_t* __restrict__ out, int64_t ld, StripPlan plan,
@@ -202,6 +231,7 @@
     struct HeavyGlobal {
         K3_GLOBAL(uint32_t) count; K3_GLOBAL(f32x4_t) wst; K3_GLOBAL(uint32_t) wid; K3_GLOBAL(uint32_t) overflow;
         K3_GLOBAL(uint32_t) seg_cnt; K3_GLOBAL(u32x4_t) ent; uint32_t ent_cap; K3_GLOBAL(uint32_t) ovf_regions; K3_GLOBAL(i32x2_t) redo;
+        uint32_t group;
     };
     auto heavy_late = [&]() -> HeavyGlobal {
         const HeavyList* p = heavy_ptr;
@@ -211,16 +241,14 @@
         g.count = (K3_GLOBAL(uint32_t))h->count; g.wst = (K3_GLOBAL(f32x4_t))h->wst; g.wid = (K3_GLOBAL(uint32_t))h->wid;
         g.overflow = (K3_GLOBAL(uint32_t))h->overflow; g.seg_cnt = (K3_GLOBAL(uint32_t))h->seg_cnt; g.ent = (K3_GLOBAL(u32x4_t))h->ent;
         g.ent_cap = h->ent_cap; g.ovf_regions = (K3_GLOBAL(uint32_t))h->ovf_regions; g.redo = (K3_GLOBAL(i32x2_t))h->redo;
+        g.group = h->call.group;
         return g;
     };
-    __shared__ __attribute__((aligned(16))) float inv_k_store[prnb::kTabShift + kInvTab + 2];
-    float* const inv_k = inv_k_store + prnb::kTabShift;
-    __shared__ WaveLds lds_all[kBlock / 64];
-    __shared__ __attribute__((aligned(kRing * 256))) uint8_t ring_all[kBlock / 64][kRing * 256];
+    float* const inv_k = lds.inv_k_store + prnb::kTabShift;
 
     const int tid = threadIdx.x;
     const int lane = tid & 63, wv = __builtin_amdgcn_readfirstlane(tid >> 6);
-    WaveLds& L = lds_all[wv];
+    WaveLds& L = lds.lds_all[wv];
 
     for (int k = tid - prnb::kTabShift; k < kInvTab + 2; k += kBlock) inv_k[k] = k > 0 ? 1.0f / (float)k : 0.0f;
     __syncthreads();
@@ -232,8 +260,9 @@
     const int64_t n0 = (int64_t)__builtin_amdgcn_readfirstlane((int32_t)at.n0);
     const int cells = __builtin_amdgcn_readfirstlane(at.cells);
     if (cells <= 0) {
-        if (lane == 0) heavy_late().count[region] = 0u;
-        return;
+        const HeavyGlobal none = heavy_late();
+        if (lane == 0) none.count[region] = 0u;
+        return none.group;
     }
 
     float a[4], bm1[4], phi[4];
@@ -263,7 +292,7 @@
     int32_t* const strip_out = out + n0 * ld + gbase;
     const uint32_t ld32 = (uint32_t)ld;
     int32_t flushed_pos = -1;
-    uint8_t* const ring = ring_all[wv];
+    uint8_t* const ring = lds.ring_all[wv];
     for (int i = lane; i < kRing * 64; i += 64) reinterpret_cast<uint32_t*>(ring)[i] = 0u;
     if (lane < 4) reinterpret_cast<uint32_t*>(&L.s1_null)[lane] = 0u;
 
@@ -636,9 +665,9 @@
         }
     }
     const bool too_many = h_cnt > heavy_cap || n_long < 0;
-    if (lane == 0) heavy.count[region] = (h_cnt < 0xffffu ? h_cnt : 0xffffu) | ((n_still + (uint32_t)n_kept) << 16);
+    if (lane == 0) heavy.count[region] = (too_many ? 0xffffu : h_cnt) | ((n_still + (uint32_t)n_kept) << 16);
     bool spills = too_many;
-    if (!too_many && h_cnt > (uint32_t)kDense) {
+    if (heavy.group == 0u && !too_many && h_cnt > (uint32_t)kDense) {
         const uint32_t n_over = h_cnt - (uint32_t)kDense;
         const uint32_t seg = region & (uint32_t)(kSegs - 1);
         uint32_t base_e = 0u;
@@ -660,6 +689,22 @@
         heavy.ovf_regions[at] = region;
         heavy.overflow[0] = 1u;
     }
-}
-
-}
+    return heavy.group;
+}
+
+template <bool VEC, bool BIG>
+__global__ __launch_bounds__(kBlock, 5) void sample_counts_stream_kernel(
+    const float* __restrict__ means, int32_t G, const CellInfo* __restrict__ cellinfo,
+    const float* __restrict__ ga, const float* __restrict__ gbm1, const float* __restrict__ gphi,
+    int64_t N, uint32_t k0, uint32_t k1, int32_t* __restrict__ out, int64_t ld, StripPlan plan,
+    uint2* __restrict__ heavy_list, uint32_t heavy_cap, uint2* __restrict__ heavy_dense,
+    const HeavyList* __restrict__ heavy_ptr)
+{
+    __shared__ __attribute__((aligned(kRing * 256))) StreamLds lds;
+    static_assert(offsetof(StripLds, ring_all) == 0, "the rings are aligned to their size");
+    const uint32_t group = stream_strip<VEC, BIG>(lds.strip, means, G, cellinfo, ga, gbm1, gphi, N, k0, k1, out, ld, plan,
+                                                  heavy_list, heavy_cap, heavy_dense, heavy_ptr);
+    group_epilogue(lds, heavy_ptr, group);
+}
+
+}
diff --git a/prosstt_amd/csrc/prosstt_amd.hip b/prosstt_amd/csrc/prosstt_amd.hip
--- a/prosstt_amd/csrc/prosstt_amd.hip
+++ b/prosstt_amd/csrc/prosstt_amd.hip
@@ -14,6 +14,7 @@
 #include "prnb_device.h"
 #include "k3_stream.h"
 #include "k3_heavy.h"
+#include "../../include/prosstt_amd_heavy.h"
 #include "numpy_stream.h"
 
 #define PA_EXPORT extern "C" __attribute__((visibility("default")))
@@ -55,6 +56,8 @@
     k3::StripPlan list_plan{};
     const k3::CellInfo* list_info = nullptr;
     int64_t list_cells = 0;
+    int last_fused = 0, last_heavy_launches = 0;
+    int64_t last_groups = 0;
     int heavy_grid = 1280;
     int stream_resident = 1280;
     uint8_t* row_bad = nullptr;
@@ -154,6 +157,8 @@
 {
     const int64_t i = (int64_t)blockIdx.x * blockDim.x + threadIdx.x;
     if (heavy_rec && i < k3::kSegs + 2) heavy.seg_cnt[i] = 0u;
+    if (heavy_rec)
+        for (int64_t j = i; j <= (int64_t)heavy.call.groups; j += (int64_t)gridDim.x * blockDim.x) heavy.call.grp_cnt[j] = 0u;
     if (heavy_rec && i == 0) *heavy_rec = heavy;
     if (flags && i == 0) {
         flags[kListOverflow] = 0;
@@ -668,6 +673,7 @@
     uint64_t regions;
     uint32_t region_cap;
     uint32_t ent_cap;
+    uint32_t group;
 };
 
 static long env_number(const char* name)
@@ -676,9 +682,16 @@
     return v ? strtol(v, nullptr, 10) : 0;
 }
 
+static bool heavy_fused()
+{
+    const char* v = getenv("PROSSTT_AMD_HEAVY");
+    return v && !strcmp(v, "fused");
+}
+
 static StreamGeometry stream_geometry(int64_t N, int32_t G, int resident)
 {
     StreamGeometry g;
+    g.group = heavy_fused() ? (uint32_t)k3::kHeavyGroup : 0u;
     const long forced = env_number("PROSSTT_AMD_STRIP_CELLS"), taper = env_number("PROSSTT_AMD_STRIP_TAPER");
     const long most = env_number("PROSSTT_AMD_STRIP_CLASSES");
     const bool uniform = taper <= 0 && (forced == 8 || forced == 16 || forced == 32 || forced == 64);
@@ -705,6 +718,7 @@
     k3::HeavyList* heavy_rec;
     k3::CellInfo* info;
     size_t bytes;
+    size_t counters_at, counters_bytes;
 };
 
 static StreamWorkspace stream_workspace(const StreamGeometry& g, int64_t N, char* base)
@@ -728,6 +742,9 @@
     w.heavy.wid = (uint32_t*)take(g.regions * (size_t)k3::kWalkSlots * 4u);
     w.heavy.ovf_regions = (uint32_t*)take(g.regions * 4u);
     w.heavy.redo = (int2*)take((size_t)k3::kRedoCap * sizeof(int2));
+    w.counters_at = at;
+    w.counters_bytes = ((size_t)k3::heavy_groups((uint32_t)g.blocks, (uint32_t)k3::kHeavyGroup).groups + 1) * 4u;
+    w.heavy.call.grp_cnt = (uint32_t*)take(w.counters_bytes);
     w.info = (k3::CellInfo*)take(0);
     w.bytes = at + ((size_t)N + 4) * sizeof(k3::CellInfo) + 256;
     return w;
@@ -736,7 +753,8 @@
 static int sampler_setup(prosstt_amd_ctx* c, Staging& st, const float* means, int64_t rows, int32_t G,
                          const int32_t* row_of_cell, const double* scaling, const double* alpha,
                          const double* beta, int64_t N, uint32_t flags, SamplerArgs* A,
-                         const StreamGeometry* geo, uint64_t cell_offset, const int64_t* cell_index, uint64_t seed)
+                         const StreamGeometry* geo, uint64_t cell_offset, const int64_t* cell_index, uint64_t seed,
+                         int32_t* d_out = nullptr, int64_t ld_out = 0)
 {
     if (!c) return fail(PROSSTT_AMD_EINVAL, "ctx is NULL");
     if (N < 0 || G < 0 || rows < 0) return fail(PROSSTT_AMD_EINVAL, "negative size");
@@ -774,6 +792,14 @@
         A->heavy.overflow = (uint32_t*)(c->scratch + kListOverflow);
         A->heavy_rec = w.heavy_rec;
         A->cellinfo = w.info;
+        k3::HeavyCall& call = A->heavy.call;
+        call.means = means; call.rows = rows; call.row_of_cell = row_of_cell;
+        call.scal = A->scal; call.ga = A->ga; call.gbm1 = A->gbm1;
+        call.cell_index = cell_index; call.cell_offset = cell_offset; call.out = d_out; call.ld = ld_out;
+        call.G = G; call.k0 = (uint32_t)seed; call.k1 = (uint32_t)(seed >> 32);
+        call.regions = (uint32_t)geo->regions; call.group = geo->group;
+        call.groups = k3::heavy_groups((uint32_t)geo->blocks, geo->group).groups;
+        call.plan = geo->plan;
     }
     const uint8_t* row_bad = nullptr;
     if (geo && (flags & (PROSSTT_AMD_CHECK_DOMAIN | PROSSTT_AMD_CHECK_DEFERRED))) {
@@ -916,6 +942,43 @@
 }
 PA_CATCH
 
+PA_EXPORT int prosstt_amd_heavy_groups(int64_t blocks, int32_t* group, int64_t* groups, int32_t* last) try
+{
+    if (blocks < 0 || blocks > 0x1fffffffll) return fail(PROSSTT_AMD_EINVAL, "bad size");
+    if (!group || !groups || !last) return fail(PROSSTT_AMD_EINVAL, "NULL argument");
+    const k3::HeavyGroups g = k3::heavy_groups((uint32_t)blocks, (uint32_t)k3::kHeavyGroup);
+    *group = k3::kHeavyGroup;
+    *groups = g.groups;
+    *last = (int32_t)g.last;
+    return 0;
+}
+PA_CATCH
+
+PA_EXPORT int prosstt_amd_heavy_workspace(int64_t N, int32_t G, int32_t resident_blocks, int64_t* counters_offset,
+                                          int64_t* counters_bytes, int64_t* total_bytes) try
+{
+    if (N < 0 || G < 0 || N > 0x7fffffffll || resident_blocks < 0) return fail(PROSSTT_AMD_EINVAL, "bad size");
+    if (!counters_offset || !counters_bytes || !total_bytes) return fail(PROSSTT_AMD_EINVAL, "NULL argument");
+    const StreamGeometry geo = stream_geometry(N, G, resident_blocks);
+    if (geo.blocks > 0x1fffffffll) return fail(PROSSTT_AMD_EINVAL, "too many tiles; chunk the cells");
+    const StreamWorkspace w = stream_workspace(geo, N, nullptr);
+    *counters_offset = (int64_t)w.counters_at;
+    *counters_bytes = (int64_t)w.counters_bytes;
+    *total_bytes = (int64_t)w.bytes;
+    return 0;
+}
+PA_CATCH
+
+PA_EXPORT int prosstt_amd_last_heavy_mode(prosstt_amd_ctx* c, int32_t* fused, int32_t* heavy_launches, int64_t* groups) try
+{
+    if (!c || !fused || !heavy_launches || !groups) return fail(PROSSTT_AMD_EINVAL, "NULL argument");
+    *fused = c->last_fused;
+    *heavy_launches = c->last_heavy_launches;
+    *groups = c->last_groups;
+    return 0;
+}
+PA_CATCH
+
 PA_EXPORT int prosstt_amd_sample_counts(prosstt_amd_ctx* c, const float* means, int64_t rows, int32_t G,
                                         const int32_t* row_of_cell, const double* scaling,
                                         const double* alpha, const double* beta, int64_t N,
@@ -934,15 +997,19 @@
     }
     const StreamGeometry geo = stream_geometry(N, G, c ? c->stream_resident : 0);
     if (geo.blocks > 0x1fffffffll) return fail(PROSSTT_AMD_EINVAL, "too many tiles; chunk the cells");
-    int rc = sampler_setup(c, st, means, rows, G, row_of_cell, scaling, alpha, beta, N, flags, &A, &geo, cell_offset,
-                           cell_index, seed);
+    int rc;
+    int32_t* d_out = out;
+    if (c && N > 0 && G > 0) {
+        HIP_TRY(hipSetDevice(c->device));
+        if ((rc = st.out(d_out, (size_t)N * ld_out))) return rc;
+    }
+    rc = sampler_setup(c, st, means, rows, G, row_of_cell, scaling, alpha, beta, N, flags, &A, &geo, cell_offset,
+                       cell_index, seed, d_out, ld_out);
     if (rc) return rc;
     if (N == 0 || G == 0) return 0;
     const k3::HeavyList heavy = A.heavy;
     k3::CellInfo* cellinfo = A.cellinfo;
     const int64_t* d_cell_index = A.cell_index;
-    int32_t* d_out = out;
-    if ((rc = st.out(d_out, (size_t)N * ld_out))) return rc;
 
     const bool vec = (G % 4 == 0) && (ld_out % 4 == 0) && (((uintptr_t)A.means & 15) == 0) &&
                      (((uintptr_t)d_out & 15) == 0);
@@ -966,12 +1033,18 @@
     HIP_TRY(hipGetLastError());
     const uint64_t region_blocks = (geo.regions + 15u) / 16u;
     const unsigned heavy_blocks = (unsigned)(region_blocks < 256u ? 256u : (region_blocks < (uint64_t)c->heavy_grid ? region_blocks : (uint64_t)c->heavy_grid));
-    k3::sample_counts_heavy_kernel<<<dim3(heavy_blocks), dim3(k3::kHeavyBlock), 0, c->stream>>>(
-        (const k3::HeavyList*)A.heavy_rec, (uint32_t)geo.regions, geo.plan, A.means, rows, G, A.row_of_cell,
-        A.scal, A.ga, A.gbm1, N, k0, k1, cell_offset, d_cell_index, d_out, ld_out,
-        (checked && !(flags & PROSSTT_AMD_PARAMS_NONNEG)) ? c->scratch : nullptr, (uint32_t)kFullReq + c->call_parity,
-        (uint32_t)kStickyRow, (uint32_t)kStickyDomain);
-    HIP_TRY(hipGetLastError());
+    const bool fused = geo.group != 0u, full_check = checked && !(flags & PROSSTT_AMD_PARAMS_NONNEG);
+    if (!fused || full_check) {
+        k3::sample_counts_heavy_kernel<<<dim3(heavy_blocks), dim3(k3::kHeavyBlock), 0, c->stream>>>(
+            (const k3::HeavyList*)A.heavy_rec, fused ? 0u : (uint32_t)geo.regions, geo.plan, A.means, rows, G, A.row_of_cell,
+            A.scal, A.ga, A.gbm1, N, k0, k1, cell_offset, d_cell_index, d_out, ld_out,
+            full_check ? c->scratch : nullptr, (uint32_t)kFullReq + c->call_parity,
+            (uint32_t)kStickyRow, (uint32_t)kStickyDomain);
+        HIP_TRY(hipGetLastError());
+    }
+    c->last_fused = fused;
+    c->last_heavy_launches = (!fused || full_check) ? 1 : 0;
+    c->last_groups = fused ? (int64_t)heavy.call.groups : 0;
     c->list = heavy;
     c->list_regions = geo.regions;
     c->list_plan = geo.plan;
@@ -1008,19 +1081,23 @@
     int64_t written = 0;
     std::vector<uint32_t> counts(c->list_regions);
     HIP_TRY(hipMemcpy(counts.data(), c->list.count, counts.size() * 4, hipMemcpyDeviceToHost));
-    uint2 dense[k3::kDense];
+    std::vector<uint2> dense(k3::kDense);
     uint32_t wid[k3::kWalkSlots];
     for (uint64_t r = 0; r < c->list_regions; ++r) {
         const uint32_t listed = counts[r] & 0xffffu, walks = counts[r] >> 16;
-        const uint32_t nd = listed > c->list.cap ? 0u : (listed < (uint32_t)k3::kDense ? listed : (uint32_t)k3::kDense);
-        *total += nd + walks;
-        if (nd + walks == 0 || written >= cap) continue;
-        if (nd) HIP_TRY(hipMemcpy(dense, c->list.dense + r * k3::kDense, (size_t)nd * sizeof(uint2), hipMemcpyDeviceToHost));
+        const uint32_t nl = listed > c->list.cap ? 0u : listed;
+        const uint32_t nd = nl < (uint32_t)k3::kDense ? nl : (uint32_t)k3::kDense;
+        const uint32_t ns = c->last_fused ? nl - nd : 0u;
+        *total += nd + ns + walks;
+        if (nd + ns + walks == 0 || written >= cap) continue;
+        dense.resize((size_t)nd + ns);
+        if (nd) HIP_TRY(hipMemcpy(dense.data(), c->list.dense + r * k3::kDense, (size_t)nd * sizeof(uint2), hipMemcpyDeviceToHost));
+        if (ns) HIP_TRY(hipMemcpy(dense.data() + nd, c->list.list + r * ((size_t)c->list.cap + k3::kListTail) + k3::kDense, (size_t)ns * sizeof(uint2), hipMemcpyDeviceToHost));
         if (walks) HIP_TRY(hipMemcpy(wid, c->list.wid + r * k3::kWalkSlots, (size_t)walks * 4, hipMemcpyDeviceToHost));
         const k3::StripAt at = k3::strip_of_region(c->list_plan, (uint32_t)r);
         const int64_t tile_g = at.tile_g, n0 = at.n0;
-        for (uint32_t i = 0; i < nd + walks && written < cap; ++i, ++written) {
-            const uint32_t pos = i < nd ? dense[i].x : (wid[i - nd] & 0xffffu);
+        for (uint32_t i = 0; i < nd + ns + walks && written < cap; ++i, ++written) {
+            const uint32_t pos = i < nd + ns ? dense[i].x : (wid[i - nd - ns] & 0xffffu);
             cells[written] = n0 + (pos >> 8);
             genes[written] = (int32_t)(tile_g * kTileG + (pos & 255u));
         }
diff --git a/prosstt_amd/device.py b/prosstt_amd/device.py
--- a/prosstt_amd/device.py
+++ b/prosstt_amd/device.py
@@ -164,6 +164,11 @@
             self._h, classes.ctypes.data_as(ctypes.c_void_p), ctypes.byref(n), ctypes.byref(tiles), ctypes.byref(blocks)))
         return classes[:n.value].copy(), tiles.value, blocks.value
 
+    def last_heavy_mode(self):
+        fused, launches, groups = ctypes.c_int32(0), ctypes.c_int32(0), ctypes.c_int64(0)
+        _native.check(self._lib.prosstt_amd_last_heavy_mode(self._h, ctypes.byref(fused), ctypes.byref(launches), ctypes.byref(groups)))
+        return bool(fused.value), launches.value, groups.value
+
     HW_OPS = dict(rcp=0, log2=1, exp2neg=2)
 
     def hw_math(self, op, first_bits, count):
```
